# steveschwarcz/Cuda-Path-Tracer-SS

Measured on AMD Instinct MI355X. Metric: Mrays/sec at 1920x1080, 8 bounces, 2072 spp run (BASELINE configs[2] asks 2000 spp; a rate metric); ray = one live ray processed in one bounce, higher is better.
Workload: dtype f32; 1 GPU; configs[2]: 1920x1080 'mixed' preset (22 spheres, 16 triangles, Lambert/Phong/Cook-Torrance/glass/mirror), 8 bounces, 2072 spp = 74 steps x 1 pass(es) x 28 sample lanes per pixel; samples_per_pass=28, frame_lanes=1, lanes_free_run=True, seed=24301

## Files before the change

### cuda-path-tracer-ss_amd/csrc/ptss_api.hip

```cpp
#include <stdio.h>
#include <stdlib.h>
#include <string.h>

#include <new>
#include <string>
#include <vector>

#include "ptss.h"
#include "ptss_device.h"
#include <algorithm>
#include <array>
#include <cmath>
#include "ptquant.h"
#include "ptdenoise.h"
#include "ptmesh.h"
#include "pttri.h"

using namespace ptv;

#if PTSS_DIAG
namespace ptss { hipError_t readDiagCounters(unsigned long long* out8); }
#endif
namespace {

// ... 473 lines not shown
int validateScene(const ptss_scene_desc& s) {
    if ((s.numSpheres && !s.spheres) || (s.numTriangles && !s.triangles) || (s.numMaterials && !s.materials) ||
        (s.numPointLights && !s.pointLights) || (s.numAreaLights && !s.areaLights))
        return fail(PTSS_EINVAL, "scene: null array with non-zero count");
    for (size_t i = 0; i < s.numSpheres; ++i)
        if (s.spheres[i].materialIdx < 0 || (size_t)s.spheres[i].materialIdx >= s.numMaterials)
            return fail(PTSS_EINVAL, "scene: sphere materialIdx out of range");
    for (size_t i = 0; i < s.numTriangles; ++i)
        if (s.triangles[i].materialIdx < 0 || (size_t)s.triangles[i].materialIdx >= s.numMaterials)
            return fail(PTSS_EINVAL, "scene: triangle materialIdx out of range");
    for (size_t i = 0; i < s.numAreaLights; ++i)
        if (s.areaLights[i].triangleIdx < 0 || (size_t)s.areaLights[i].triangleIdx + 1 >= s.numTriangles)
            return fail(PTSS_EINVAL, "scene: area light needs triangles [triangleIdx, triangleIdx+1]");
    return PTSS_OK;
}

int localRows(const ptss_render_config& cfg) {
    int rows = 0;
    for (int y = 0; y < cfg.height; ++y)
        if ((y / cfg.bandRows) % cfg.tileWorld == cfg.tileRank) ++rows;
    return rows;
}

int createCheck(hipError_t e, const char* what) { return e == hipSuccess ? PTSS_OK : fail(e == hipErrorOutOfMemory ? PTSS_ENOMEM : PTSS_EHIP, what, e); }
#define ALLOC_TRY(expr) RC_TRY(createCheck((expr), #expr))
template <class T>
hipError_t mallocZeroed(T** p, size_t bytes) {
    const hipError_t e = hipMalloc(p, bytes);
    return e == hipSuccess ? hipMemset(*p, 0, bytes) : e;
}

int allocLane(Lane& ln, const uint32_t (&shardCount0)[ptss::kShards], bool ownStream) {
    const size_t poolBytes = (size_t)ptss::kRayPlanes * ln.regionCap * ptss::kShards * sizeof(float);
    for (float*& pool : ln.dPool) ALLOC_TRY(hipMalloc(&pool, poolBytes));
    for (uint32_t*& counts : ln.dCounts) ALLOC_TRY(mallocZeroed(&counts, ptss::kCountWords * sizeof(uint32_t)));
    ALLOC_TRY(mallocZeroed(&ln.dLastCounts, ptss::kCountWords * sizeof(uint32_t)));
    for (int s = 0; s < ptss::kShards; ++s)
        ALLOC_TRY(hipMemcpy(ln.dCounts[0] + ptss::countIndex(0, s), &shardCount0[s], sizeof(uint32_t), hipMemcpyHostToDevice));
    ALLOC_TRY(hipMalloc(&ln.dShardCount0, sizeof(shardCount0)));
    ALLOC_TRY(hipMemcpy(ln.dShardCount0, shardCount0, sizeof(shardCount0), hipMemcpyHostToDevice));
    ALLOC_TRY(mallocZeroed(&ln.dDone, (ptss::kCountWords + ptss::kCountStride) * sizeof(uint32_t)));
    if (ownStream) {
        ALLOC_TRY(hipStreamCreateWithFlags(&ln.stream, hipStreamNonBlocking));
        for (hipEvent_t& ev : ln.evDone) ALLOC_TRY(hipEventCreateWithFlags(&ev, hipEventDisableTiming));
    }
    ALLOC_TRY(hipHostMalloc(&ln.hCounts, 4 * ptss::kCountWords * sizeof(uint32_t), hipHostMallocDefault));
    for (hipEvent_t& ev : ln.hintEvent) ALLOC_TRY(hipEventCreateWithFlags(&ev, hipEventDisableTiming));
    return PTSS_OK;
}
#undef ALLOC_TRY

void releaseLane(Lane& ln) {
    for (hipEvent_t ev : ln.hintEvent)
        if (ev) (void)hipEventDestroy(ev);
    if (ln.hCounts) (void)hipHostFree(ln.hCounts);
    (void)hipFree(ln.dDone);
    for (hipEvent_t ev : ln.evDone)
        if (ev) (void)hipEventDestroy(ev);
    if (ln.stream) (void)hipStreamDestroy(ln.stream);
    for (float* pool : ln.dPool) (void)hipFree(pool);
    for (uint32_t* counts : ln.dCounts) (void)hipFree(counts);
    (void)hipFree(ln.dShardCount0);
    (void)hipFree(ln.dLastCounts);
}

ptss::FrameBuffers frameBuffers(const ptss_context* c, int laneIdx, ptss_uchar4* pixels, int sample) {
    const Lane& ln = c->lanes[(size_t)laneIdx];
    ptss::FrameBuffers fb{};
    fb.pool[0] = ln.dPool[0];
    fb.pool[1] = ln.dPool[1];
    fb.rngHome = c->dRngHome;
    fb.counts = ln.dCounts[c->countParity];
    fb.countsNext = ln.dCounts[1 - c->countParity];
    fb.shardCount0 = ln.dShardCount0;
    fb.lastCounts = ln.dLastCounts;
    fb.totalRayBounces = c->dTotal + laneIdx;
    fb.guardTimeouts = reinterpret_cast<uint32_t*>(c->dTotal + ptss::kMaxLanes + 8);
    fb.accum = c->dAccum;
    fb.fsum = c->dFsum;
    fb.staged = c->dStaged ? c->dStaged + (c->stagedTwice ? (size_t)(c->frameIndex & 1u) * c->capacity * c->samples : 0) : nullptr;
    fb.quantTable = reinterpret_cast<const float*>(c->image().dBlob + c->image().layout.offQuant);
    fb.pixels = pixels;
    fb.regionCap = ln.regionCap;
    fb.numPixels = c->numPixels;
    fb.plane = c->capacity;
    fb.samples = c->samples;
    fb.firstTiles = c->samples * (c->capacity / ptss::kBlock);
    fb.minLive = c->tile.world > 1 ? 0u : ptss::kMinLiveRays;
    fb.inverseTicks = 1.f / (float)((int)c->samples * (sample + 1));
    fb.defaultColor[0] = c->defaultColor[0];
    fb.defaultColor[1] = c->defaultColor[1];
    fb.defaultColor[2] = c->defaultColor[2];
    fb.laneIndex = (uint32_t)laneIdx;
    fb.laneCount = (uint32_t)c->lanes.size();
    fb.frameRays = c->numPixels * c->samples;
    fb.numPeers = fb.laneCount - 1;
    fb.myDone = ln.dDone;
    fb.myFrameDone = ln.dDone + ptss::kCountWords;
    fb.frameSeq = c->frameIndex;
    fb.joinsFrame = (laneIdx + 1 == (int)c->lanes.size()) ? 1u : 0u;
    uint32_t p = 0;
    for (size_t k = 0; k < c->lanes.size(); ++k) {
        if ((int)k == laneIdx) continue;
        fb.peerCounts[p] = c->lanes[k].dCounts[c->countParity];
        fb.peerDone[p] = c->lanes[k].dDone;
        fb.peerFrameDone[p] = c->lanes[k].dDone + ptss::kCountWords;
        ++p;
    }
    return fb;
}

void drainKernelEvents(ptss_context* c, bool wait) {
    size_t k = 0;
    for (size_t i = 0; i < c->evBusy.size(); ++i) {
        EventPair p = c->evBusy[i];
        hipError_t q = wait ? hipEventSynchronize(p.b) : hipEventQuery(p.b);
        if (q == hipSuccess) {
            float start = 0, ms = 0;
            if (hipEventElapsedTime(&start, c->evEpoch, p.a) == hipSuccess && hipEventElapsedTime(&ms, p.a, p.b) == hipSuccess)
            {
                if (c->kernelSpans.size() >= (1u << 20)) c->kernelSpans.clear();
                c->kernelSpans.emplace_back((double)start, (double)start + (double)ms);
            }
            c->evFree.push_back(p);
        } else {
            c->evBusy[k++] = p;
        }
    }
    c->evBusy.resize(k);
    (void)hipGetLastError();
}

int checkLaneTimeouts(ptss_context* c) {
    if (c->lanes.size() < 2 && !c->images[0].oneLaunch && !c->images[1].oneLaunch) return PTSS_OK;
    uint32_t v = 0;
    HIP_TRY(hipMemcpy(&v, c->dTotal + ptss::kMaxLanes + 8, sizeof(v), hipMemcpyDeviceToHost));
    if (v != c->timeoutsSeen) {
        c->timeoutsSeen = v;
        return fail(PTSS_ETIMEOUT, "a bounded wait on the device expired (a frame lane for a peer lane, or a workgroup of the one-launch "
                                   "frame kernel for its shard): the frame was not traced as specified");
    }
    return PTSS_OK;
}

void selectImage(ptss_context* c) {
    if (!c->images[1].dBlob) return;
    const int want = cameraInRange(c->camera) ? 0 : 1;
    if (want != c->active) {
        c->active = want;
        c->cameraDirty = true;
    }
}

ptss::EyeParams eyeParams(const ptss_context* c) {
    return {c->camera, -2 * ptm::tan(c->camera.fieldOfView * 0.5f), (float)c->tile.height / (float)c->tile.width, 1.0f / c->tile.width,
            1.0f / c->tile.height};
}

void harvestHints(ptss_context* c) {
    for (Lane& ln : c->lanes)
        for (int q = 0; q < 4; ++q) {
            if (!ln.hintPending[q] || hipEventQuery(ln.hintEvent[q]) != hipSuccess) continue;
            const uint32_t* src = ln.hCounts + (size_t)q * ptss::kCountWords;
            for (int b = 0; b <= ptss::kMaxBounces; ++b) {
                uint32_t mx = 0;
                for (int s = 0; s < ptss::kShards; ++s) mx = std::max(mx, src[ptss::countIndex(b, s)]);
                ln.hint[b] = mx;
            }
            ln.haveHint = true;
            ln.hintPending[q] = false;
        }
    (void)hipGetLastError();
}

int forkLanes(ptss_context* c, bool forkNeeded) {
    if (c->lanes.size() > 1 && (forkNeeded || c->frameIndex == 0 || !c->cfg.lanesFreeRun)) {
        HIP_TRY(hipEventRecord(c->evFork, c->stream));
        for (Lane& ln : c->lanes) HIP_TRY(hipStreamWaitEvent(ln.stream, c->evFork, 0));
    }
    if (c->stagedTwice && c->frameIndex >= 2)
        for (Lane& ln : c->lanes) HIP_TRY(hipStreamWaitEvent(ln.stream, c->evDisplay[c->frameIndex & 1u], 0));
    return PTSS_OK;
}

template <class Launch>
int timedLaunch(ptss_context* c, hipStream_t s, Launch launch) {
    if (!c->cfg.timeKernels) return launch();
    EventPair ev{nullptr, nullptr};
    if (c->evFree.empty() && c->evBusy.size() >= 4096) drainKernelEvents(c, true);
    if (c->evFree.empty()) {
        HIP_TRY(hipEventCreate(&ev.a));
        HIP_TRY(hipEventCreate(&ev.b));
    } else {
        ev = c->evFree.back();
        c->evFree.pop_back();
    }
    HIP_TRY(hipEventRecord(ev.a, s));
    RC_TRY(launch());
    HIP_TRY(hipEventRecord(ev.b, s));
    c->evBusy.push_back(ev);
    return PTSS_OK;
}

int traceOneLaunch(ptss_context* c, const ptss::FrameBuffers& fb, int numIterations, bool bounded, const ptss::EyeParams& eye) {
    const SceneImage& im = c->image();
    return timedLaunch(c, c->stream, [&] {
        HIP_TRY(ptss::launchFrame(c->stream, fb, im.dBlob, im.layout, numIterations, bounded, c->lanes[0].maxBlocks, c->tile, eye,
                                          &c->launchedKernels));
        return PTSS_OK;
    });
}

int traceBounces(ptss_context* c, ptss::FrameBuffers* fbs, int numIterations, bool bounded, const ptss::EyeParams& eye) {
    const SceneImage& im = c->image();
    const int K = (int)c->lanes.size();
    for (int i = 0; i < numIterations; ++i)
        for (int k = 0; k < K; ++k) {
            Lane& ln = c->lanes[(size_t)k];
            const hipStream_t ls = K > 1 ? ln.stream : c->stream;
            int blocks = ln.maxBlocks;
            if (i > 0 && ln.haveHint) {
                const unsigned long long tilesPerShard = ((unsigned long long)ln.hint[i] * 65 / 64 + ptss::kBlock) / ptss::kBlock + 1;
                const unsigned long long want = tilesPerShard * ptss::kShards;
                if (want < (unsigned long long)blocks) blocks = (int)want;
            }
            if (c->gridCap > 0 && c->gridCap * ptss::kShards < blocks) blocks = c->gridCap * ptss::kShards;
            if (i > 0)
                for (int j = 0, p = 0; j < K; ++j)
                    if (j != k) fbs[k].peerTarget[p++] = c->lanes[(size_t)j].doneTarget[i - 1];
            RC_TRY(timedLaunch(c, ls, [&] {
                HIP_TRY(ptss::launchBounce(ls, fbs[k], im.dBlob, im.layout, i, i == numIterations - 1, im.inLds, bounded, blocks, c->tile, eye,
                                               &c->launchedKernels));
                return PTSS_OK;
            }));
            ln.doneTarget[i] += (uint32_t)blocks;
        }
    return PTSS_OK;
}

int flushAndJoin(ptss_context* c, const ptss::FrameBuffers* fbs, int numIterations) {
    const int K = (int)c->lanes.size();
    for (int k = 0; k < K; ++k) {
        Lane& ln = c->lanes[(size_t)k];
        const hipStream_t ls = K > 1 ? ln.stream : c->stream;
        ptss::FlushTargets targets{};
        for (int j = 0, p = 0; j < K; ++j)
            if (j != k) {
                for (int b = 0; b <= ptss::kMaxBounces; ++b) targets.target[p][b] = c->lanes[(size_t)j].doneTarget[b];
                ++p;
            }
        HIP_TRY(ptss::launchFlush(ls, fbs[k], numIterations, targets));
        if (!ln.haveHint || (c->frameIndex & 7u) == 0) {
            const int q = (int)((c->frameIndex >> 3) & 3u);
            if (!ln.hintPending[q]) {
                HIP_TRY(hipMemcpyAsync(ln.hCounts + (size_t)q * ptss::kCountWords, ln.dLastCounts, ptss::kCountWords * sizeof(uint32_t),
                                       hipMemcpyDeviceToHost, ls));
                HIP_TRY(hipEventRecord(ln.hintEvent[q], ls));
                ln.hintPending[q] = true;
            }
        }
        if (K > 1 && k == K - 1) {
            HIP_TRY(hipEventRecord(ln.evDone[c->frameIndex & 1u], ls));
            HIP_TRY(hipStreamWaitEvent(c->stream, ln.evDone[c->frameIndex & 1u], 0));
        }
    }
    return PTSS_OK;
}

}

extern "C" {

int ptss_version(void) { return PTSS_VERSION; }

const char* ptss_error_string(int code) {
    switch (code) {
        case PTSS_OK: return "ok";
        case PTSS_EINVAL: return "invalid argument";
        case PTSS_EHIP: return "HIP runtime error";
        case PTSS_ENODEVICE: return "no usable HIP device";
        case PTSS_ENOMEM: return "out of memory";
        case PTSS_ERANGE: return "buffer too small or index out of range";
        case PTSS_ETIMEOUT: return "a frame lane timed out waiting for a peer lane";
        default: return "unknown error";
    }
}

const char* ptss_last_error_detail(void) { return g_detail.c_str(); }

int ptss_default_config(ptss_render_config* cfg) {
    if (!cfg) return fail(PTSS_EINVAL, "cfg is null");
    memset(cfg, 0, sizeof(*cfg));
    cfg->structSize = (unsigned int)sizeof(*cfg);
    cfg->width = 512;
    cfg->height = 512;
    cfg->seed = 0x5EEDull;
    cfg->maxIterations = 15;
    cfg->device = 0;
    cfg->tileRank = 0;
    cfg->tileWorld = 1;
    cfg->bandRows = 8;
    cfg->syncEachFrame = 1;
    cfg->floatAccumulator = 0;
    cfg->timeKernels = 0;
    cfg->samplesPerPass = 1;
    cfg->everySphereLoop = 0;
    cfg->frameLanes = 0;
    cfg->lanesFreeRun = 0;
    cfg->oneLaunchFrames = 0;
    return PTSS_OK;
}

int ptss_create(const ptss_scene_desc* scene, const ptss_render_config* cfg, ptss_context** out) {
    if (!scene || !cfg || !out) return fail(PTSS_EINVAL, "null argument");
    if (cfg->structSize != (unsigned int)sizeof(ptss_render_config))
        return fail(PTSS_EINVAL, "cfg->structSize is not this library's sizeof(ptss_render_config): the caller was built against another "
                                 "ptss.h (compare ptss_version() with PTSS_VERSION) or did not start from ptss_default_config");
    if (cfg->width <= 0 || cfg->height <= 0 || (long long)cfg->width * cfg->height > (1ll << 31) - 256)
        return fail(PTSS_EINVAL, "bad frame size");
    if (cfg->maxIterations == 0 || cfg->maxIterations > (unsigned)ptss::kMaxBounces)
        return fail(PTSS_EINVAL, "maxIterations must be in [1, 64]");
    if (cfg->tileWorld <= 0 || cfg->tileRank < 0 || cfg->tileRank >= cfg->tileWorld || cfg->bandRows <= 0)
        return fail(PTSS_EINVAL, "bad tile spec");
    const int spp = cfg->samplesPerPass == 0 ? 1 : cfg->samplesPerPass;
    if (spp < 1 || spp > 64) return fail(PTSS_EINVAL, "samplesPerPass must be in [1, 64]");
    if ((long long)cfg->width * cfg->height >= (1ll << 26)) return fail(PTSS_EINVAL, "frame too large (>= 2^26 pixels)");
    {
        const long long rows = localRows(*cfg);
        const unsigned long long rays = ((unsigned long long)cfg->width * rows + 255ull) / 256ull * 256ull * (unsigned long long)spp;
        if ((rays + (unsigned long long)ptss::kShards * ptss::kBlock) * ptss::kRayPlanes >= (1ull << 32))
            return fail(PTSS_EINVAL, "too many rays per pass: width x local rows x samplesPerPass must stay below ~226 million");
    }
    int rc = validateScene(*scene);
    if (rc != PTSS_OK) return rc;

    int ndev = 0;
    hipError_t e = hipGetDeviceCount(&ndev);
    if (e != hipSuccess || ndev <= 0) {
        (void)hipGetLastError();
        return fail(PTSS_ENODEVICE, "hipGetDeviceCount found no device (libptss has no CPU path)", e);
    }
    if (cfg->device < 0 || cfg->device >= ndev) return fail(PTSS_ENODEVICE, "device ordinal out of range");
    HIP_TRY(hipSetDevice(cfg->device));

    ptss_context* c = new (std::nothrow) ptss_context();
    if (!c) return fail(PTSS_ENOMEM, "context");
    c->cfg = *cfg;
    c->maxIterations = cfg->maxIterations;
    c->samples = (uint32_t)spp;
    c->defaultColor[0] = scene->defaultColor.x;
    c->defaultColor[1] = scene->defaultColor.y;
    c->defaultColor[2] = scene->defaultColor.z;
    c->camera.rotation = q4(1, 0, 0, 0);
    c->camera.position = v3(0, 0, 0);
    c->camera.zNear = -0.1f;
    c->camera.zFar = -100.0f;
    c->camera.fieldOfView = ptm::kPi / 2.0f;

    c->tile = ptss::TileMap{cfg->width, cfg->height, localRows(*cfg), cfg->tileRank, cfg->tileWorld, cfg->bandRows};
    c->numPixels = (uint32_t)cfg->width * (uint32_t)c->tile.localRows;
    const uint32_t gran = ptss::kBlock > 256 ? (uint32_t)ptss::kBlock : 256u;
    c->capacity = ((c->numPixels + gran - 1) / gran) * gran;
    if (c->capacity == 0) c->capacity = gran;
    int numLanes = cfg->frameLanes;
    if (numLanes < 0 || numLanes > ptss::kMaxLanes) return (delete c, fail(PTSS_EINVAL, "frameLanes must be in [0, 4]"));
    {
        const unsigned long long rays = (unsigned long long)c->numPixels * c->samples;
        if (numLanes == 0) numLanes = (cfg->lanesFreeRun && rays >= (3ull << 17) && rays <= (1ull << 24)) ? 2 : 1;
    }
    c->lanes.resize((size_t)numLanes);
    uint32_t shardCount0[ptss::kMaxLanes][ptss::kShards] = {{0}};
    {
        const uint32_t tilesPerPlane = c->capacity / ptss::kBlock;
        const uint32_t tiles = tilesPerPlane * c->samples;
        const uint32_t rounds = (tiles + ptss::kShards - 1) / ptss::kShards;
        for (int k = 0; k < numLanes; ++k) {
            const uint32_t laneRounds = (rounds + (uint32_t)numLanes - 1 - (uint32_t)k) / (uint32_t)numLanes;
            c->lanes[(size_t)k].regionCap = (laneRounds ? laneRounds : 1) * ptss::kBlock;
            c->lanes[(size_t)k].maxBlocks = (int)(c->lanes[(size_t)k].regionCap / ptss::kBlock) * ptss::kShards;
        }
        for (uint32_t t = 0; t < tiles; ++t) {
            const uint32_t first = (t % tilesPerPlane) * ptss::kBlock;
            uint32_t cnt = 0;
            if (first < c->numPixels) cnt = c->numPixels - first < (uint32_t)ptss::kBlock ? c->numPixels - first : (uint32_t)ptss::kBlock;
            shardCount0[(t / ptss::kShards) % (uint32_t)numLanes][t % ptss::kShards] += cnt;
        }
    }

    const bool wantAccel = accelEligible(*scene) && !cfg->everySphereLoop;
    const bool wantMesh = !wantAccel && meshEligible(*scene) && !cfg->everySphereLoop;
    const int numImages = wantAccel ? 2 : 1;
    std::vector<float4> blob[2];
    for (int i = 0; i < numImages; ++i) {
        SceneImage& im = c->images[i];
        packScene(*scene, im.layout, blob[i], wantAccel && i == 0, wantMesh);
        im.inLds = ptss::bounceLdsBytes(im.layout, true) <= 64 * 1024;
    }

#define CREATE_TRY(expr) do { if (int _rc = createCheck((expr), #expr)) return (ptss_destroy(c), _rc); } while (0)

    for (int i = 0; i < numImages; ++i) {
        CREATE_TRY(hipMalloc(&c->images[i].dBlob, blob[i].size() * sizeof(float4)));
        CREATE_TRY(hipMemcpy(c->images[i].dBlob, blob[i].data(), blob[i].size() * sizeof(float4), hipMemcpyHostToDevice));
    }
    CREATE_TRY(hipMalloc(&c->dRngHome, (size_t)ptss::kHomeWords * c->capacity * c->samples * sizeof(uint32_t)));
    for (int k = 0; k < numLanes; ++k)
        if (int laneRc = allocLane(c->lanes[(size_t)k], shardCount0[k], numLanes > 1)) return (ptss_destroy(c), laneRc);
    if (numLanes > 1) CREATE_TRY(hipEventCreateWithFlags(&c->evFork, hipEventDisableTiming));
    CREATE_TRY(mallocZeroed(&c->dTotal, kTotalWords * sizeof(unsigned long long)));
    CREATE_TRY(mallocZeroed(&c->dAccumOwned, (size_t)3 * c->capacity * sizeof(uint32_t)));
    c->dAccum = c->dAccumOwned;
    if (cfg->floatAccumulator) CREATE_TRY(mallocZeroed(&c->dFsum, (size_t)3 * c->capacity * c->samples * sizeof(float)));
    if (c->samples > 1) {
        c->stagedTwice = numLanes > 1 && cfg->lanesFreeRun != 0;
        const size_t words = (size_t)c->capacity * c->samples * (c->stagedTwice ? 2 : 1);
        CREATE_TRY(mallocZeroed(&c->dStaged, words * sizeof(uint32_t)));
        if (c->stagedTwice)
            for (int q = 0; q < 2; ++q) CREATE_TRY(hipEventCreateWithFlags(&c->evDisplay[q], hipEventDisableTiming));
    }
    CREATE_TRY(hipEventCreate(&c->evStart));
    CREATE_TRY(hipEventCreate(&c->evStop));
    CREATE_TRY(hipEventCreate(&c->evEpoch));

    {
        std::vector<uint32_t> table(ptrng::kJumpTableWords);
        ptrng::build_subsequence_table(table.data());
        uint32_t* dTable = nullptr;
        CREATE_TRY(hipMalloc(&dTable, table.size() * sizeof(uint32_t)));
        hipError_t e1 = hipMemcpy(dTable, table.data(), table.size() * sizeof(uint32_t), hipMemcpyHostToDevice);
        hipError_t e2 = e1;
        if (e1 == hipSuccess && c->numPixels > 0)
            e2 = ptss::launchRngInit(nullptr, c->dRngHome, c->capacity, c->samples, c->tile, cfg->seed, dTable);
        hipError_t e3 = e2 == hipSuccess ? hipEventRecord(c->evEpoch, nullptr) : e2;
        if (e3 == hipSuccess) e3 = hipDeviceSynchronize();
        (void)hipFree(dTable);
        CREATE_TRY(e3);
    }

    {
        hipDeviceProp_t prop;
        CREATE_TRY(hipGetDeviceProperties(&prop, cfg->device));
        const SceneImage& primary = c->images[0];
        const int perCU = ptss::bounceOccupancyBlocksPerCU(primary.layout, primary.inLds, primary.layout.sphereBounded != 0);
        c->gridCap = prop.multiProcessorCount * (perCU > 0 ? perCU : 4) * 16 / ptss::kShards;
        auto qualifies = [&](const SceneImage& im) {
            if (cfg->oneLaunchFrames <= 0 || numLanes != 1 || !im.inLds) return false;
            if (ptss::meshImage(im.layout)) return false;
            int perCU = ptss::frameOccupancyBlocksPerCU(im.layout, false);
            if (im.layout.sphereBounded) perCU = std::min(perCU, ptss::frameOccupancyBlocksPerCU(im.layout, true));
            const int resident = perCU - 1;
            return resident >= 1 && c->lanes[0].maxBlocks <= prop.multiProcessorCount * resident;
        };
        for (int i = 0; i < numImages; ++i) c->images[i].oneLaunch = qualifies(c->images[i]);
#ifdef PTSS_TUNING_KNOBS
        if (const char* e = getenv("PTSS_SCENE_PATH")) {
            if (!strcmp(e, "scalar"))
                for (SceneImage& im : c->images) im.inLds = false;
        }
        if (const char* e = getenv("PTSS_GRID_CAP")) c->gridCap = atoi(e);
#endif
    }
#undef CREATE_TRY

    *out = c;
    return PTSS_OK;
}

int ptss_destroy(ptss_context* c) {
    if (!c) return PTSS_OK;
    (void)hipSetDevice(c->cfg.device);
    (void)hipDeviceSynchronize();
    drainKernelEvents(c, true);
    for (EventPair& p : c->evFree) {
        (void)hipEventDestroy(p.a);
        (void)hipEventDestroy(p.b);
    }
    for (Lane& ln : c->lanes) releaseLane(ln);
    for (hipEvent_t ev : {c->evFork, c->evDisplay[0], c->evDisplay[1], c->evStart, c->evStop, c->evEpoch})
        if (ev) (void)hipEventDestroy(ev);
    for (SceneImage& im : c->images) (void)hipFree(im.dBlob);
    (void)hipFree(c->dRngHome);
    (void)hipFree(c->dTotal);
    (void)hipFree(c->dAccumOwned);
    (void)hipFree(c->dFsum);
    (void)hipFree(c->dStaged);
    for (float4* plane : c->dDenoise) (void)hipFree(plane);
    delete c;
    return PTSS_OK;
}

int ptss_generate_frame(ptss_context* c, ptss_uchar4* pixels, int ticks) {
    if (!c) return fail(PTSS_EINVAL, "ctx is null");
    hipStream_t st = c->stream;
    HIP_TRY(hipSetDevice(c->cfg.device));
    c->lastTicks = ticks;
    if (c->numPixels == 0) {
        if (c->resetTicksThisFrame) c->lastResetTick = ticks;
        c->resetTicksThisFrame = false;
        c->lastMs = 0.0f;
        return PTSS_OK;
    }

    selectImage(c);
    bool forkNeeded = false;
    if (c->resetTicksThisFrame) {
        forkNeeded = true;
        c->lastResetTick = ticks;
        HIP_TRY(ptss::launchClear(st, frameBuffers(c, 0, pixels, 0)));
        c->resetTicksThisFrame = false;
    }
    const int sample = ticks - c->lastResetTick;
    const int K = (int)c->lanes.size();
    ptss::FrameBuffers fbs[ptss::kMaxLanes];
    for (int k = 0; k < K; ++k) fbs[k] = frameBuffers(c, k, pixels, sample);

    if (c->cfg.syncEachFrame) HIP_TRY(hipEventRecord(c->evStart, st));

    const int numIterations = c->usePathTracer ? (int)c->maxIterations : 1;
    const ptss::EyeParams eye = eyeParams(c);
    if (c->cameraDirty) {
        forkNeeded = true;
        HIP_TRY(ptss::launchPrimaryPrep(st, c->image().dBlob, c->image().layout, c->camera.position));
        c->cameraDirty = false;
    }
    harvestHints(c);
    RC_TRY(forkLanes(c, forkNeeded));
    if (c->cfg.timeKernels) drainKernelEvents(c, false);
    const bool bounded = c->image().layout.sphereBounded != 0 && cameraInRange(c->camera);
    RC_TRY(c->image().oneLaunch && K == 1 ? traceOneLaunch(c, fbs[0], numIterations, bounded, eye) : traceBounces(c, fbs, numIterations, bounded, eye));
    RC_TRY(flushAndJoin(c, fbs, numIterations));
    if (c->samples > 1) {
        HIP_TRY(ptss::launchDisplay(st, fbs[0]));
        if (c->stagedTwice) HIP_TRY(hipEventRecord(c->evDisplay[c->frameIndex & 1u], st));
    }
    c->countParity ^= 1;
    c->frameIndex++;

    if (c->cfg.syncEachFrame) {
        HIP_TRY(hipEventRecord(c->evStop, st));
        HIP_TRY(hipEventSynchronize(c->evStop));
        HIP_TRY(hipEventElapsedTime(&c->lastMs, c->evStart, c->evStop));
        return c->lanes.size() > 1 ? checkLaneTimeouts(c) : PTSS_OK;
    }
    return PTSS_OK;
}

int ptss_set_camera(ptss_context* c, const ptss_camera* camera) {
    if (!c || !camera) return fail(PTSS_EINVAL, "null argument");
    c->camera = *camera;
    c->cameraDirty = true;
    c->resetTicksThisFrame = true;
    return PTSS_OK;
}

int ptss_get_camera(const ptss_context* c, ptss_camera* out) {
    if (!c || !out) return fail(PTSS_EINVAL, "null argument");
    *out = c->camera;
    return PTSS_OK;
}

int ptss_request_reset(ptss_context* c) {
    if (!c) return fail(PTSS_EINVAL, "ctx is null");
    c->resetTicksThisFrame = true;
    return PTSS_OK;
}

int ptss_set_mode(ptss_context* c, int usePathTracer) {
    if (!c) return fail(PTSS_EINVAL, "ctx is null");
    c->usePathTracer = usePathTracer != 0;
    c->resetTicksThisFrame = true;
    return PTSS_OK;
}

int ptss_set_max_iterations(ptss_context* c, unsigned int maxIterations) {
    if (!c || maxIterations == 0 || maxIterations > (unsigned)ptss::kMaxBounces)
        return fail(PTSS_EINVAL, "maxIterations must be in [1, 64]");
    c->maxIterations = maxIterations;
    return PTSS_OK;
}

int ptss_set_stream(ptss_context* c, void* hipStream) {
    if (!c) return fail(PTSS_EINVAL, "ctx is null");
    c->stream = (hipStream_t)hipStream;
    return PTSS_OK;
}

int ptss_bind_accumulator(ptss_context* c, uint32_t* dev) {
    if (!c) return fail(PTSS_EINVAL, "ctx is null");
    c->dAccum = dev ? dev : c->dAccumOwned;
    return PTSS_OK;
}

int ptss_accumulator_devptr(ptss_context* c, uint32_t** out) {
    if (!c || !out) return fail(PTSS_EINVAL, "null argument");
    *out = c->dAccum;
    return PTSS_OK;
}

int ptss_float_accumulator_devptr(ptss_context* c, float** out) {
    if (!c || !out) return fail(PTSS_EINVAL, "null argument");
    *out = c->dFsum;
    return PTSS_OK;
}

int ptss_alloc_pixels(ptss_context* c, ptss_uchar4** out) {
    if (!c || !out) return fail(PTSS_EINVAL, "null argument");
    HIP_TRY(hipSetDevice(c->cfg.device));
    HIP_TRY(hipMalloc(out, (size_t)c->capacity * sizeof(ptss_uchar4)));
    HIP_TRY(hipMemset(*out, 0, (size_t)c->capacity * sizeof(ptss_uchar4)));
    return PTSS_OK;
}

int ptss_free_pixels(ptss_context* c, ptss_uchar4* dev) {
    if (!c) return fail(PTSS_EINVAL, "ctx is null");
    HIP_TRY(hipFree(dev));
    return PTSS_OK;
}

int ptss_local_pixels(const ptss_context* c, size_t* out) {
    if (!c || !out) return fail(PTSS_EINVAL, "null argument");
    *out = c->numPixels;
    return PTSS_OK;
}

int ptss_local_rows(const ptss_context* c, int* rows, int cap, int* count) {
    if (!c || !count) return fail(PTSS_EINVAL, "null argument");
    int n = 0;
    for (int y = 0; y < c->tile.height; ++y) {
        if ((y / c->tile.bandRows) % c->tile.world != c->tile.rank) continue;
        if (rows) {
            if (n >= cap) return fail(PTSS_ERANGE, "rows[] too small");
            rows[n] = y;
        }
        ++n;
    }
    *count = n;
    return PTSS_OK;
}

int ptss_synchronize(ptss_context* c) {
    if (!c) return fail(PTSS_EINVAL, "ctx is null");
    HIP_TRY(hipStreamSynchronize(c->stream));
    return checkLaneTimeouts(c);
}

int ptss_read_accumulator(ptss_context* c, uint32_t* host, size_t count) {
    if (!c || !host) return fail(PTSS_EINVAL, "null argument");
    if (count != (size_t)3 * c->numPixels) return fail(PTSS_ERANGE, "count must be 3 * local pixels");
    HIP_TRY(hipStreamSynchronize(c->stream));
    HIP_TRY(hipMemcpy(host, c->dAccum, count * sizeof(uint32_t), hipMemcpyDeviceToHost));
    return checkLaneTimeouts(c);
}

int ptss_read_float_accumulator(ptss_context* c, float* host, size_t count) {
    if (!c || !host) return fail(PTSS_EINVAL, "null argument");
    if (!c->dFsum) return fail(PTSS_EINVAL, "context was created without floatAccumulator");
    if (count != (size_t)3 * c->numPixels) return fail(PTSS_ERANGE, "count must be 3 * local pixels");
    HIP_TRY(hipStreamSynchronize(c->stream));
    if (c->samples == 1) {
        HIP_TRY(hipMemcpy(host, c->dFsum, count * sizeof(float), hipMemcpyDeviceToHost));
    } else {
        std::vector<float> lane(count);
        for (size_t k = 0; k < count; ++k) host[k] = 0.0f;
        for (uint32_t l = 0; l < c->samples; ++l) {
            HIP_TRY(hipMemcpy(lane.data(), c->dFsum + (size_t)3 * l * c->capacity, count * sizeof(float), hipMemcpyDeviceToHost));
            for (size_t k = 0; k < count; ++k) host[k] = host[k] + lane[k];
        }
    }
    return checkLaneTimeouts(c);
}

int ptss_read_pixels(ptss_context* c, const ptss_uchar4* dev, ptss_uchar4* host, size_t count) {
    if (!c || !dev || !host) return fail(PTSS_EINVAL, "null argument");
    if (count > c->numPixels) return fail(PTSS_ERANGE, "count exceeds local pixels");
    HIP_TRY(hipStreamSynchronize(c->stream));
    HIP_TRY(hipMemcpy(host, dev, count * sizeof(ptss_uchar4), hipMemcpyDeviceToHost));
    return checkLaneTimeouts(c);
}

int ptss_read_rng_state(ptss_context* c, size_t local_pixel, uint32_t* out6) { return ptss_read_rng_state_lane(c, local_pixel, 0, out6); }

int ptss_read_rng_state_lane(ptss_context* c, size_t local_pixel, unsigned int lane, uint32_t* out6) {
    if (!c || !out6) return fail(PTSS_EINVAL, "null argument");
    if (local_pixel >= c->numPixels || lane >= c->samples) return fail(PTSS_ERANGE, "pixel or lane out of range");
    HIP_TRY(hipStreamSynchronize(c->stream));
    HIP_TRY(hipMemcpy(out6, c->dRngHome + (size_t)ptss::kHomeWords * ((size_t)lane * c->capacity + local_pixel), 6 * sizeof(uint32_t),
                      hipMemcpyDeviceToHost));
    return PTSS_OK;
}

int ptss_last_pass_ms(ptss_context* c, float* out) {
    if (!c || !out) return fail(PTSS_EINVAL, "null argument");
    *out = c->lastMs;
    return PTSS_OK;
}

int ptss_samples_since_reset(const ptss_context* c, int* out) {
    if (!c || !out) return fail(PTSS_EINVAL, "null argument");
    *out = c->resetTicksThisFrame ? 0 : (c->lastTicks - c->lastResetTick + 1) * (int)c->samples;
    return PTSS_OK;
}

int ptss_live_counts(ptss_context* c, uint32_t* out, int cap, int* n) {
    if (!c || !out || !n) return fail(PTSS_EINVAL, "null argument");
    const int numIterations = c->usePathTracer ? (int)c->maxIterations : 1;
    if (cap < numIterations) return fail(PTSS_ERANGE, "out[] too small");
    std::vector<uint32_t> raw(ptss::kCountWords), sum(ptss::kCountWords, 0u);
    HIP_TRY(hipStreamSynchronize(c->stream));
    for (const Lane& ln : c->lanes) {
        HIP_TRY(hipMemcpy(raw.data(), ln.dLastCounts, raw.size() * sizeof(uint32_t), hipMemcpyDeviceToHost));
        for (size_t k = 0; k < raw.size(); ++k) sum[k] += raw[k];
    }
    bool stopped = false;
    for (int i = 0; i < numIterations; ++i) {
        uint32_t total = 0;
        for (int s = 0; s < ptss::kShards; ++s) total += sum[ptss::countIndex(i, s)];
        if (total <= (c->tile.world > 1 ? 0u : ptss::kMinLiveRays)) stopped = true;
        out[i] = stopped ? 0u : total;
    }
    *n = numIterations;
    return checkLaneTimeouts(c);
}

int ptss_total_ray_bounces(ptss_context* c, unsigned long long* out) {
    if (!c || !out) return fail(PTSS_EINVAL, "null argument");
    HIP_TRY(hipStreamSynchronize(c->stream));
    unsigned long long perLane[ptss::kMaxLanes];
    HIP_TRY(hipMemcpy(perLane, c->dTotal, sizeof(perLane), hipMemcpyDeviceToHost));
    *out = 0;
    for (size_t k = 0; k < c->lanes.size(); ++k) *out += perLane[k];
    return checkLaneTimeouts(c);
}

int ptss_guard_timeouts(ptss_context* c, unsigned int* out) {
    if (!c || !out) return fail(PTSS_EINVAL, "null argument");
    HIP_TRY(hipStreamSynchronize(c->stream));
    uint32_t v = 0;
    HIP_TRY(hipMemcpy(&v, c->dTotal + ptss::kMaxLanes + 8, sizeof(v), hipMemcpyDeviceToHost));
    *out = v;
    return PTSS_OK;
}

int ptss_one_launch_frames(const ptss_context* c, int* out) {
    if (!c || !out) return fail(PTSS_EINVAL, "null argument");
    *out = (c->image().oneLaunch && c->lanes.size() == 1) ? 1 : 0;
    return PTSS_OK;
}

int ptss_frame_lanes(const ptss_context* c, int* out) {
    if (!c || !out) return fail(PTSS_EINVAL, "null argument");
    *out = (int)c->lanes.size();
    return PTSS_OK;
}

int ptss_launched_kernels(const ptss_context* c, unsigned long long* out) {
    if (!c || !out) return fail(PTSS_EINVAL, "null argument");
    *out = c->launchedKernels;
    return PTSS_OK;
}

static int rayQuery(ptss_context* c, bool any, const ptss_ray_query* rays, void* out, size_t n, void* hipStream) {
    if (!c) return fail(PTSS_EINVAL, "ctx is null");
    if (n == 0) return PTSS_OK;
    if (!rays || !out) return fail(PTSS_EINVAL, "null buffer with n > 0");
    if (n >= (size_t(1) << 31)) return fail(PTSS_ERANGE, "n must be below 2^31");
    if (((uintptr_t)rays | (uintptr_t)out) & (any ? 3u : 15u) || (uintptr_t)rays & 15u)
        return fail(PTSS_EINVAL, "rays and hits must be 16-byte aligned, verdicts 4-byte aligned");
    const SceneImage& im = c->images[0];
    if (!im.dBlob) return fail(PTSS_EINVAL, "context has no scene image");
    HIP_TRY(hipSetDevice(c->cfg.device));
    hipStream_t st = hipStream ? static_cast<hipStream_t>(hipStream) : c->stream;
    HIP_TRY(ptss::launchQuery(st, any, im.dBlob, im.layout, im.inLds, rays, out, (uint32_t)n, c->gridCap * ptss::kShards,
                              &c->launchedKernels));
    return PTSS_OK;
}

int ptss_intersect(ptss_context* c, const ptss_ray_query* dev_rays, ptss_ray_hit* dev_hits, size_t n, void* hipStream) {
    return rayQuery(c, false, dev_rays, dev_hits, n, hipStream);
}

int ptss_occluded(ptss_context* c, const ptss_ray_query* dev_rays, uint32_t* dev_occluded, size_t n, void* hipStream) {
    return rayQuery(c, true, dev_rays, dev_occluded, n, hipStream);
}

int ptss_render_features(ptss_context* c, ptss_pixel_feature* dev_features, void* hipStream) {
    if (!c) return fail(PTSS_EINVAL, "ctx is null");
    if (!dev_features) return fail(PTSS_EINVAL, "dev_features is null");
    if ((uintptr_t)dev_features & 15u) return fail(PTSS_EINVAL, "dev_features must be 16-byte aligned");
    if (c->numPixels == 0) return PTSS_OK;
    const SceneImage& im = c->images[0];
    if (!im.dBlob) return fail(PTSS_EINVAL, "context has no scene image");
    HIP_TRY(hipSetDevice(c->cfg.device));
    hipStream_t st = hipStream ? static_cast<hipStream_t>(hipStream) : c->stream;
    const ptss_vec3 defaultColor{c->defaultColor[0], c->defaultColor[1], c->defaultColor[2]};
    HIP_TRY(ptss::launchFeatures(st, im.dBlob, im.layout, im.inLds, c->tile, eyeParams(c), defaultColor, dev_features, c->numPixels,
                                 c->gridCap * ptss::kShards, &c->launchedKernels));
    return PTSS_OK;
}

int ptss_default_denoise_params(ptss_denoise_params* p) {
    if (!p) return fail(PTSS_EINVAL, "params is null");
    p->structSize = (unsigned int)sizeof(*p);
    p->levels = 5;
    p->sigmaColor = 64.0f;
    p->sigmaNormal = 0.1f;
    p->sigmaDepth = 4.0f;
    return PTSS_OK;
}

int ptss_denoise(ptss_context* c, const ptss_pixel_feature* dev_features, const ptss_denoise_params* params, ptss_uchar4* dev_out,
                 void* hipStream) {
    if (!c) return fail(PTSS_EINVAL, "ctx is null");
    if (!dev_features || !params || !dev_out) return fail(PTSS_EINVAL, "null argument");
    if (params->structSize != (unsigned int)sizeof(ptss_denoise_params))
        return fail(PTSS_EINVAL, "params->structSize is not this library's sizeof(ptss_denoise_params): start from ptss_default_denoise_params");
    if (params->levels < 0 || params->levels > PTSS_DENOISE_MAX_LEVELS) return fail(PTSS_EINVAL, "levels must be in [0, 6]");
    if (!(params->sigmaColor > 0.0f) || !(params->sigmaNormal > 0.0f) || !(params->sigmaDepth >= 0.0f))
        return fail(PTSS_EINVAL, "sigmaColor and sigmaNormal must be positive, sigmaDepth not negative");
    if (((uintptr_t)dev_features & 15u) || ((uintptr_t)dev_out & 3u)) return fail(PTSS_EINVAL, "dev_features must be 16-byte aligned, dev_out 4-byte aligned");
    if (c->tile.world > 1)
        return fail(PTSS_EINVAL, "ptss_denoise needs the whole frame: this context is a pixel-band shard (tileWorld > 1), whose bands of rows "
                                 "have no neighbours to filter with");
    HIP_TRY(hipSetDevice(c->cfg.device));
    hipStream_t st = hipStream ? static_cast<hipStream_t>(hipStream) : c->stream;
    const int levels = params->levels;
    if (levels >= 2)
        for (float4*& plane : c->dDenoise)
            if (!plane) {
                const hipError_t e = hipMalloc(&plane, (size_t)c->numPixels * sizeof(float4));
                if (e != hipSuccess) return fail(e == hipErrorOutOfMemory ? PTSS_ENOMEM : PTSS_EHIP, "ptss_denoise: colour planes", e);
            }
    const float inverseTicks = 1.f / (float)((int)c->samples * (c->lastTicks - c->lastResetTick + 1));
    const int width = c->tile.width, height = c->tile.height;
    c->denoiseLastPlane = levels >= 2 ? (levels - 2) & 1 : -1;
    c->denoiseLastLevel = levels - 2;
    c->denoiseStream = st;
    for (int i = 0; i < (levels > 0 ? levels : 1); ++i) {
        const bool first = i == 0, last = i + 1 >= levels;
        const void* src = first ? static_cast<const void*>(c->dAccum) : c->dDenoise[(i - 1) & 1];
        void* dst = last ? static_cast<void*>(dev_out) : c->dDenoise[i & 1];
        HIP_TRY(ptss::launchDenoise(st, first, last, src, dst, dev_features, width, height, ptdn::levelOf(*params, i), inverseTicks,
                                    &c->launchedKernels));
    }
    return PTSS_OK;
}

int ptss_read_denoise_plane(ptss_context* c, float* host_float3, size_t count, int* level) {
    if (!c || !host_float3) return fail(PTSS_EINVAL, "null argument");
    if (c->denoiseLastPlane < 0) return fail(PTSS_EINVAL, "no colour plane: the latest ptss_denoise of this context ran fewer than two levels");
    if (count != (size_t)3 * c->numPixels) return fail(PTSS_ERANGE, "count must be 3 * local pixels");
    HIP_TRY(hipSetDevice(c->cfg.device));
    HIP_TRY(hipStreamSynchronize(c->denoiseStream));
    std::vector<float4> plane(c->numPixels);
    HIP_TRY(hipMemcpy(plane.data(), c->dDenoise[c->denoiseLastPlane], plane.size() * sizeof(float4), hipMemcpyDeviceToHost));
    for (size_t p = 0; p < plane.size(); ++p) {
        host_float3[3 * p] = plane[p].x;
        host_float3[3 * p + 1] = plane[p].y;
        host_float3[3 * p + 2] = plane[p].z;
    }
    if (level) *level = c->denoiseLastLevel;
    return PTSS_OK;
}

int ptss_triangle_leaves(const ptss_context* c, int* out) {
    if (!c || !out) return fail(PTSS_EINVAL, "null argument");
    const ptss::SceneLayout& L = c->image().layout;
    *out = ptss::meshImage(L) ? L.mesh.numLeaves : 0;
    return PTSS_OK;
}

int ptss_debug_counters(ptss_context* c, unsigned long long* out8) {
    if (!c || !out8) return fail(PTSS_EINVAL, "null argument");
    HIP_TRY(hipStreamSynchronize(c->stream));
#if PTSS_DIAG
    HIP_TRY(ptss::readDiagCounters(out8));
#else
    for (int k = 0; k < 8; ++k) out8[k] = 0ull;
#endif
    return PTSS_OK;
}

int ptss_bounce_kernel_time(ptss_context* c, double* total_ms, unsigned long long* launches) {
    if (!c || !total_ms || !launches) return fail(PTSS_EINVAL, "null argument");
    HIP_TRY(hipStreamSynchronize(c->stream));
    for (const Lane& ln : c->lanes)
        if (ln.stream) HIP_TRY(hipStreamSynchronize(ln.stream));
    drainKernelEvents(c, true);
    std::sort(c->kernelSpans.begin(), c->kernelSpans.end());
    double busy = 0.0, curA = 0.0, curB = -1.0;
    for (const auto& sp : c->kernelSpans) {
        if (curB < curA || sp.first > curB) {
            if (curB >= curA) busy += curB - curA;
            curA = sp.first;
            curB = sp.second;
        } else if (sp.second > curB) {
            curB = sp.second;
        }
    }
    if (curB >= curA) busy += curB - curA;
    *total_ms = busy;
    *launches = c->kernelSpans.size();
    c->kernelSpans.clear();
    HIP_TRY(hipEventRecord(c->evEpoch, c->stream));
    HIP_TRY(hipEventSynchronize(c->evEpoch));
    return checkLaneTimeouts(c);
}

}
```

### cuda-path-tracer-ss_amd/csrc/ptss_device.h

```cpp
#pragma once
#include <hip/hip_runtime.h>
#include <stdint.h>

#include "ptmath.h"
#include "ptss_types.h"
#include "xorwow.h"

namespace ptdn { struct Level; }

namespace ptss {

enum RayPlane : int {
    kOx = 0, kOy, kOz,
    kDx, kDy, kDz,
    kL0x, kL0y, kL0z,
    kTx, kTy, kTz,
    kPix,
    kR0, kR1, kR2, kR3, kR4,
    kRd,
    kRayPlanes
};
constexpr int kHomeWords = 8;
constexpr int kMaxBounces = 64;
#ifndef PTSS_BLOCK
#define PTSS_BLOCK 256
#endif
#ifndef PTSS_SHARDS
#define PTSS_SHARDS 16
#endif
#ifndef PTSS_CHUNK
#define PTSS_CHUNK 16
#endif
#ifndef PTSS_MINWAVES
#define PTSS_MINWAVES 7
#endif
#ifndef PTSS_MINWAVES_BOUNDED
#define PTSS_MINWAVES_BOUNDED 6
#endif
#ifndef PTSS_MINWAVES_FIRST
#define PTSS_MINWAVES_FIRST 6
#endif
#ifndef PTSS_ABLATE
#define PTSS_ABLATE 0
#endif
#ifndef PTSS_DIAG
#define PTSS_DIAG 0
#endif
constexpr int kBlock = PTSS_BLOCK;
constexpr int kChunkSpheres = PTSS_CHUNK;
static_assert((kChunkSpheres & (kChunkSpheres - 1)) == 0, "chunk size must be a power of two");
constexpr int kShards = PTSS_SHARDS;
constexpr int kCountStride = 32;
constexpr int kCountWords = (kMaxBounces + 1) * kShards * kCountStride;
__host__ __device__ inline int countIndex(int bounce, int shard) { return (bounce * kShards + shard) * kCountStride; }
constexpr int kWaves = kBlock / 64;
constexpr uint32_t kMinLiveRays = 128;

struct SceneLayout {
    int numSpheres, numTriangles, numMaterials, numPointLights, numAreaLights;
    int offSphere;
    int offSphereMat;
    int offTri;
    int offTriNormal;
    int offTriVert;
    int offMaterial;
    int offPointLight;
    int offAreaLight;
    int accelSpheres;
    int numChunks;
    int offChunk;
    int offSphereOrig;
    int offSpherePos;
    int offQuant;
    int offPrimSphere;
    int offPrimTri;
    int offPrimChunk;
    int totalVec4;
    int ldsVec4;
    int neeSkipSafe;
    int sphereBounded;
    int neePairs;
    int triDetBounded;
    int triClassed;
    union {
        uint32_t triClassPack[5];
        struct {
            int numLeaves, numGroups;
            int offGroup;
            int offLeaf;
            int reserved;
        } mesh;
    };
    int offTriPos;
};

constexpr int kMeshLeaf = 16;
__host__ __device__ inline bool meshImage(const SceneLayout& L) { return !L.triClassed && L.mesh.numLeaves > 0; }

struct TileMap {
    int width, height;
    int localRows;
    int rank, world, bandRows;
};

struct EyeParams {
    ptss_camera camera;
    float s;
    float aspect;
    float invW, invH;
};

constexpr int kMaxLanes = 4;

struct FrameBuffers {
    float* pool[2];
    uint32_t* rngHome;
    uint32_t* counts;
    uint32_t* countsNext;
    const uint32_t* shardCount0;
    uint32_t* lastCounts;
    unsigned long long* totalRayBounces;
    uint32_t* accum;
    float* fsum;
    const float* quantTable;
    uint32_t* staged;
    ptss_uchar4* pixels;
    uint32_t regionCap;
    uint32_t numPixels;
    uint32_t plane;
    uint32_t samples;
    uint32_t firstTiles;
    uint32_t minLive;
    float inverseTicks;
    float defaultColor[3];
    uint32_t laneIndex, laneCount;
    uint32_t frameRays;
    uint32_t numPeers;
    const uint32_t* peerCounts[kMaxLanes - 1];
    const uint32_t* peerDone[kMaxLanes - 1];
    uint32_t peerTarget[kMaxLanes - 1];
    uint32_t* myDone;
    uint32_t* myFrameDone;
    const uint32_t* peerFrameDone[kMaxLanes - 1];
    uint32_t frameSeq;
    uint32_t joinsFrame;
    uint32_t* guardTimeouts;
};

hipError_t launchRngInit(hipStream_t st, uint32_t* rngHome, uint32_t plane, uint32_t samples, TileMap tile, uint64_t seed,
                         const uint32_t* jumpTable);
hipError_t launchDisplay(hipStream_t st, const FrameBuffers& fb);
hipError_t launchClear(hipStream_t st, const FrameBuffers& fb);
hipError_t launchPrimaryPrep(hipStream_t st, float4* sceneBlob, const SceneLayout& layout, ptss_vec3 origin);
hipError_t launchBounce(hipStream_t st, const FrameBuffers& fb, const float4* sceneBlob, SceneLayout layout, int bounce,
                        bool isLast, bool sceneInLds, bool bounded, int gridBlocks, TileMap tile, EyeParams eye, unsigned long long* launched);
size_t bounceLdsBytes(const SceneLayout& layout, bool sceneInLds);
hipError_t launchFrame(hipStream_t st, const FrameBuffers& fb, const float4* sceneBlob, SceneLayout layout, int numBounces, bool bounded, int gridBlocks,
                       TileMap tile, EyeParams eye, unsigned long long* launched);
int frameOccupancyBlocksPerCU(const SceneLayout& layout, bool bounded);
struct FlushTargets {
    uint32_t target[kMaxLanes - 1][kMaxBounces + 1];
};
hipError_t launchFlush(hipStream_t st, const FrameBuffers& fb, int numBounces, const FlushTargets& targets);
int bounceOccupancyBlocksPerCU(const SceneLayout& layout, bool sceneInLds, bool bounded);
hipError_t launchQuery(hipStream_t st, bool any, const float4* sceneBlob, SceneLayout layout, bool sceneInLds, const void* rays, void* out,
                       uint32_t n, int maxBlocks, unsigned long long* launched);
hipError_t launchFeatures(hipStream_t st, const float4* sceneBlob, SceneLayout layout, bool sceneInLds, TileMap tile, EyeParams eye,
                          ptss_vec3 defaultColor, void* out, uint32_t n, int maxBlocks, unsigned long long* launched);
hipError_t launchDenoise(hipStream_t st, bool first, bool last, const void* src, void* dst, const void* features, int width, int height,
                         const ptdn::Level& level, float inverseTicks, unsigned long long* launched);

}
```

### cuda-path-tracer-ss_amd/csrc/ptss_kernels.hip

```cpp
#include "ptss_device.h"
#include "ptquant.h"
#include "pttri.h"

#include <array>
#include <utility>

using namespace ptv;

namespace ptss {
namespace {

__device__ __forceinline__ float asF(uint32_t u) { return __builtin_bit_cast(float, u); }
__device__ __forceinline__ uint32_t asU(float f) { return __builtin_bit_cast(uint32_t, f); }
__device__ __forceinline__ vec3 xyz(float4 v) { return vec3{v.x, v.y, v.z}; }
__device__ __forceinline__ bool waveAny(bool p) { return __builtin_amdgcn_ballot_w64(p) != 0ull; }
__device__ __forceinline__ bool waveAll(bool p) { return __builtin_amdgcn_ballot_w64(p) == __builtin_amdgcn_ballot_w64(true); }
__device__ __forceinline__ void waveLdsFence() { __builtin_amdgcn_fence(__ATOMIC_ACQ_REL, "wavefront"); }

struct PixelCoord {
    int x, gy;
    uint32_t globalIndex;
};

__device__ __forceinline__ PixelCoord locate(const TileMap& t, uint32_t local) {
    const int lx = (int)(local % (uint32_t)t.width);
    const int ly = (int)(local / (uint32_t)t.width);
    const int band = ly / t.bandRows, within = ly % t.bandRows;
    PixelCoord p;
    p.x = lx;
    p.gy = (band * t.world + t.rank) * t.bandRows + within;
    p.globalIndex = (uint32_t)p.gy * (uint32_t)t.width + (uint32_t)lx;
    return p;
}

constexpr uint32_t kLaneShift = 26;
constexpr uint32_t kPixMask = (1u << kLaneShift) - 1u;
__device__ __forceinline__ uint32_t pixOf(uint32_t packed) { return packed & kPixMask; }
__device__ __forceinline__ uint32_t laneOf(uint32_t packed) { return packed >> kLaneShift; }

struct RayRegs {
    vec3 o, d, L0, T;
    uint32_t pix;
    ptrng::State rng;
    bool active;
};

__device__ __forceinline__ const float* tileBlock(const float* __restrict__ region, uint32_t firstSlot ) {
    return region + (size_t)(firstSlot / kBlock) * (kRayPlanes * kBlock);
}
__device__ __forceinline__ uint32_t slotWord(uint32_t slot) {
    return (slot / kBlock) * (uint32_t)(kRayPlanes * kBlock) + (slot % kBlock);
}

template <bool kCoherent = false>
__device__ __forceinline__ float ldPlane(const float* __restrict__ block, uint32_t laneBytes, int plane) {
    const float* p = reinterpret_cast<const float*>(reinterpret_cast<const char*>(block) + (size_t)laneBytes + (size_t)plane * (kBlock * sizeof(float)));
    if constexpr (kCoherent) return __hip_atomic_load(p, __ATOMIC_RELAXED, __HIP_MEMORY_SCOPE_AGENT);
    else return *p;
}
template <bool kCoherent = false>
__device__ __forceinline__ void stPlane(float* __restrict__ region, uint32_t wordBytes, int plane, float v) {
    float* p = reinterpret_cast<float*>(reinterpret_cast<char*>(region) + (size_t)wordBytes + (size_t)plane * (kBlock * sizeof(float)));
    if constexpr (kCoherent) __hip_atomic_store(p, v, __ATOMIC_RELAXED, __HIP_MEMORY_SCOPE_AGENT);
    else *p = v;
}

template <bool kCoherent = false>
__device__ __forceinline__ void loadRayGeometry(const float* __restrict__ block, uint32_t w, RayRegs& r) {
    const uint32_t b = w * 4u;
    r.o = vec3{ldPlane<kCoherent>(block, b, kOx), ldPlane<kCoherent>(block, b, kOy), ldPlane<kCoherent>(block, b, kOz)};
    r.d = vec3{ldPlane<kCoherent>(block, b, kDx), ldPlane<kCoherent>(block, b, kDy), ldPlane<kCoherent>(block, b, kDz)};
    r.active = true;
}
template <bool kCoherent = false>
__device__ __forceinline__ void loadRayRng(const float* __restrict__ block, uint32_t w, RayRegs& r) {
    const uint32_t b = w * 4u;
    r.rng.v[0] = asU(ldPlane<kCoherent>(block, b, kR0));
    r.rng.v[1] = asU(ldPlane<kCoherent>(block, b, kR1));
    r.rng.v[2] = asU(ldPlane<kCoherent>(block, b, kR2));
    r.rng.v[3] = asU(ldPlane<kCoherent>(block, b, kR3));
    r.rng.v[4] = asU(ldPlane<kCoherent>(block, b, kR4));
    r.rng.d = asU(ldPlane<kCoherent>(block, b, kRd));
}
template <bool kCoherent = false>
__device__ __forceinline__ void loadRayRadiance(const float* __restrict__ block, uint32_t w, RayRegs& r) {
    const uint32_t b = w * 4u;
    r.L0 = vec3{ldPlane<kCoherent>(block, b, kL0x), ldPlane<kCoherent>(block, b, kL0y), ldPlane<kCoherent>(block, b, kL0z)};
    r.T = vec3{ldPlane<kCoherent>(block, b, kTx), ldPlane<kCoherent>(block, b, kTy), ldPlane<kCoherent>(block, b, kTz)};
    r.pix = asU(ldPlane<kCoherent>(block, b, kPix));
}
template <bool kCoherent = false>
__device__ __forceinline__ void loadRay(const float* __restrict__ block, uint32_t w, RayRegs& r) {
    loadRayGeometry<kCoherent>(block, w, r);
    loadRayRng<kCoherent>(block, w, r);
    loadRayRadiance<kCoherent>(block, w, r);
}

template <bool kCoherent = false>
__device__ __forceinline__ void storeRay(float* __restrict__ region, uint32_t slot, const RayRegs& r) {
    const uint32_t b = slotWord(slot) * 4u;
    stPlane<kCoherent>(region, b, kOx, r.o.x);   stPlane<kCoherent>(region, b, kOy, r.o.y);   stPlane<kCoherent>(region, b, kOz, r.o.z);
    stPlane<kCoherent>(region, b, kDx, r.d.x);   stPlane<kCoherent>(region, b, kDy, r.d.y);   stPlane<kCoherent>(region, b, kDz, r.d.z);
    stPlane<kCoherent>(region, b, kL0x, r.L0.x); stPlane<kCoherent>(region, b, kL0y, r.L0.y); stPlane<kCoherent>(region, b, kL0z, r.L0.z);
    stPlane<kCoherent>(region, b, kTx, r.T.x);   stPlane<kCoherent>(region, b, kTy, r.T.y);   stPlane<kCoherent>(region, b, kTz, r.T.z);
    stPlane<kCoherent>(region, b, kPix, asF(r.pix));
    stPlane<kCoherent>(region, b, kR0, asF(r.rng.v[0]));
    stPlane<kCoherent>(region, b, kR1, asF(r.rng.v[1]));
    stPlane<kCoherent>(region, b, kR2, asF(r.rng.v[2]));
    stPlane<kCoherent>(region, b, kR3, asF(r.rng.v[3]));
    stPlane<kCoherent>(region, b, kR4, asF(r.rng.v[4]));
    stPlane<kCoherent>(region, b, kRd, asF(r.rng.d));
}

__device__ __forceinline__ bool sphereTest(float4 sp, vec3 o, vec3 d, float limit, float& t) {
    const vec3 v = o - xyz(sp);
    const float b = dot(d, v) * 2;
    const float c = dot(v, v) - sp.w;
    float disc = (b * b) - 4 * c;
    if (disc < 0) return false;
    disc = ptm::sqrt(disc);
    float t0 = (-b + disc) * 0.5f;
    float t1 = (-b - disc) * 0.5f;
    if (t0 < 0 && t1 < 0) return false;
    if (t0 > t1) {
        const float tmp = t0;
        t0 = t1;
        t1 = tmp;
    }
    const float cand = (t0 < 0) ? t1 : t0;
    if (cand > limit) return false;
    t = cand;
    return true;
}

struct TriHit {
    bool hit;
    unsigned long long hitMask;
    float dist, w0, w1, w2;
};

struct TriRows {
    float4 a, b, c;
};
__device__ __forceinline__ float4 loadRow16(const float4* p) { return *p; }
__device__ __forceinline__ TriRows loadTri(const float4* tr) { return TriRows{loadRow16(tr), loadRow16(tr + 1), loadRow16(tr + 2)}; }
__device__ __forceinline__ TriRows loadTriEdges(const float4* tr) { return TriRows{float4{0, 0, 0, 0}, loadRow16(tr + 1), loadRow16(tr + 2)}; }

__device__ __forceinline__ float triRcp(float det) { return ptm::rcp_if_above_1em7(det); }

__device__ __forceinline__ unsigned long long maskOf(bool directCompare) { return __builtin_amdgcn_ballot_w64(directCompare); }

__device__ __forceinline__ TriHit triangleTest(const TriRows& tr, vec3 o, vec3 d, float limit, unsigned long long liveMask) {
    const vec3 v0 = xyz(tr.a), e1 = xyz(tr.b), e2 = xyz(tr.c);
    const vec3 q = cross(d, e2);
    const float det = dot(e1, q);
// ... 56 lines not shown
        const bool hit = __builtin_amdgcn_inverse_ballot_w64(hitMask);
        best.dist = hit ? h.dist : best.dist;
        best.key = hit ? key : best.key;
        best.w1 = hit ? b1 : best.w1;
        best.w2 = hit ? b2 : best.w2;
    }
}
struct ClassBounds {
    uint32_t w[5];
};
__device__ __forceinline__ ClassBounds classBounds(const SceneLayout& L) {
    return ClassBounds{{L.triClassPack[0], L.triClassPack[1], L.triClassPack[2], L.triClassPack[3], L.triClassPack[4]}};
}
template <int kCode>
__device__ __forceinline__ int classBegin(ClassBounds& b) {
    asm volatile("" : "+s"(b.w[kCode / 4]));
    return (int)((b.w[kCode / 4] >> (8 * (kCode % 4))) & 255u);
}
#define PTSS_FOR_TRIANGLES_BY_CLASS(L, BODY)                                                                        \
    do {                                                                                                            \
        ClassBounds _cb = classBounds(L);                                                                           \
        PTSS_TRI_CLASS_LOOP(_cb, 0, 0, BODY) PTSS_TRI_CLASS_LOOP(_cb, 0, 1, BODY) PTSS_TRI_CLASS_LOOP(_cb, 0, 2, BODY) PTSS_TRI_CLASS_LOOP(_cb, 0, 3, BODY) \
        PTSS_TRI_CLASS_LOOP(_cb, 1, 0, BODY) PTSS_TRI_CLASS_LOOP(_cb, 1, 2, BODY) PTSS_TRI_CLASS_LOOP(_cb, 1, 3, BODY)      \
        PTSS_TRI_CLASS_LOOP(_cb, 2, 0, BODY) PTSS_TRI_CLASS_LOOP(_cb, 2, 1, BODY) PTSS_TRI_CLASS_LOOP(_cb, 2, 3, BODY)      \
        PTSS_TRI_CLASS_LOOP(_cb, 3, 0, BODY) PTSS_TRI_CLASS_LOOP(_cb, 3, 1, BODY) PTSS_TRI_CLASS_LOOP(_cb, 3, 2, BODY)      \
    } while (0)
#define PTSS_TRI_CLASS_LOOP(cb, c1, c2, BODY) \
    for (int t = classBegin<(c1) * 4 + (c2)>(cb), tEnd = classBegin<(c1) * 4 + (c2) + 1>(cb); t < tEnd; ++t) { BODY(c1, c2, t) }

template <int kC1, int kC2>
__device__ __forceinline__ void triangleClassedAny(const float4* rows, vec3 o, vec3 d, float limit, unsigned long long& need, unsigned long long& blocked) {
    const pttri::Head h = pttri::head<kC1, kC2, false>(xyz(loadRow16(rows)), xyz(loadRow16(rows + 1)), xyz(loadRow16(rows + 2)), v3(0, 0, 0), v3(0, 0, 0), 0.0f, o, d);
    const unsigned long long passMask = need & maskOf(!(ptm::abs(h.det) <= 1e-7f)) & maskOf(!(h.dist <= 0.0f)) & maskOf(!(h.dist > limit));
    if (passMask != 0ull) {
        float b0, b1, b2;
        pttri::weights<kC1, kC2>(h, d, b0, b1, b2);
        const unsigned long long hitMask = passMask & maskOf(!(__builtin_fminf(__builtin_fminf(b0, b1), b2) < 0));
        blocked |= hitMask;
        need &= ~hitMask;
    }
}
template <int kC1, int kC2>
__device__ __forceinline__ void triangleClassedPair(const float4* rows, vec3 o, vec3 dA, float limitA, vec3 dB, float limitB, unsigned long long& needA,
                                                    unsigned long long& needB, unsigned long long& blockedA, unsigned long long& blockedB) {
    const vec3 e1 = xyz(loadRow16(rows + 1)), e2 = xyz(loadRow16(rows + 2));
    const pttri::OriginPart p = pttri::originPart<kC1, kC2>(xyz(loadRow16(rows)), e1, e2, o);
    if (needA != 0ull) {
        const pttri::Head h = pttri::headFrom<kC1, kC2>(p, e1, e2, dA);
        const unsigned long long pass = needA & maskOf(!(ptm::abs(h.det) <= 1e-7f)) & maskOf(!(h.dist <= 0.0f)) & maskOf(!(h.dist > limitA));
        if (pass != 0ull) {
            float b0, b1, b2;
            pttri::weights<kC1, kC2>(h, dA, b0, b1, b2);
            const unsigned long long hit = pass & maskOf(!(__builtin_fminf(__builtin_fminf(b0, b1), b2) < 0));
            blockedA |= hit;
            needA &= ~hit;
        }
    }
    if (needB != 0ull) {
        const pttri::Head h = pttri::headFrom<kC1, kC2>(p, e1, e2, dB);
        const unsigned long long pass = needB & maskOf(!(ptm::abs(h.det) <= 1e-7f)) & maskOf(!(h.dist <= 0.0f)) & maskOf(!(h.dist > limitB));
        if (pass != 0ull) {
            float b0, b1, b2;
            pttri::weights<kC1, kC2>(h, dB, b0, b1, b2);
            const unsigned long long hit = pass & maskOf(!(__builtin_fminf(__builtin_fminf(b0, b1), b2) < 0));
            blockedB |= hit;
            needB &= ~hit;
        }
    }
}
__device__ __forceinline__ bool classedQueryOk(vec3 o, vec3 d) { return waveAll(dot(d, d) < 0x1p30f) && waveAll(dot(o, o) < 0x1p100f); }

__device__ __forceinline__ bool sphereTestPrimary(float4 pv, vec3 d, float limit, float& t) {
    const float b = dot(d, xyz(pv)) * 2;
    float disc = (b * b) - 4 * pv.w;
    if (disc < 0) return false;
    disc = ptm::sqrt(disc);
    float t0 = (-b + disc) * 0.5f;
    float t1 = (-b - disc) * 0.5f;
    if (t0 < 0 && t1 < 0) return false;
    if (t0 > t1) {
        const float tmp = t0;
        t0 = t1;
        t1 = tmp;
    }
    const float cand = (t0 < 0) ? t1 : t0;
    if (cand > limit) return false;
    t = cand;
    return true;
}

__device__ __forceinline__ TriHit triangleTestPrimary(const TriRows& tr, float4 ps , float4 pr ,
                                                      vec3 d, float limit, unsigned long long liveMask) {
    const vec3 e1 = xyz(tr.b), e2 = xyz(tr.c);
    const vec3 q = cross(d, e2);
    const float det = dot(e1, q);
    const float inverseDet = triRcp(det);
    const float dist = ps.w * inverseDet;
    const unsigned long long passMask = liveMask & maskOf(!(ptm::abs(det) <= 1e-7f)) & maskOf(!(dist <= 0.0f)) & maskOf(!(dist > limit));
    TriHit h;
    h.hit = false;
    h.hitMask = 0ull;
    h.dist = dist;
    h.w0 = h.w1 = h.w2 = 0;
    if (passMask != 0ull) {
        const float b1 = dot(xyz(ps), q) * inverseDet;
        const float b2 = dot(d, xyz(pr)) * inverseDet;
        const float b0 = 1.0f - (b1 + b2);
        h.hitMask = passMask & maskOf(!(b0 < 0)) & maskOf(!(b1 < 0)) & maskOf(!(b2 < 0));
        h.hit = __builtin_amdgcn_inverse_ballot_w64(h.hitMask);
        h.w0 = b0;
        h.w1 = b1;
        h.w2 = b2;
    }
    return h;
}

__device__ __forceinline__ void shiftInMayHit(uint32_t& rev, float bb, float c4) {
    asm("v_cmp_nlt_f32 vcc, %1, %2\n\tv_addc_co_u32 %0, vcc, %0, %0, vcc" : "+v"(rev) : "v"(bb), "v"(c4) : "vcc");
}
template <bool kCull>
__device__ __forceinline__ float aheadFactor(float h) {
    if constexpr (kCull) {
        const float hk = h * 0x1p-18f;
        float m;
        asm("v_min_f32 %0, %1, %2" : "=v"(m) : "v"(hk), "v"(h));
        return m;
    } else {
        return h;
    }
}
template <bool kBounded, bool kCull = false>
__device__ __forceinline__ void shiftInSphere(uint32_t& rev, float4 sp, vec3 o, vec3 d) {
    const vec3 v = o - xyz(sp);
    if constexpr (kBounded) {
        const float h = dot(d, v);
        const float c = dot(v, v) - sp.w;
        shiftInMayHit(rev, h * aheadFactor<kCull>(h), c);
    } else {
        const float b = dot(d, v) * 2;
        const float c = dot(v, v) - sp.w;
        shiftInMayHit(rev, b * b, 4 * c);
    }
}
template <bool kBounded>
__device__ __forceinline__ void shiftInSpherePrimary(uint32_t& rev, float4 pv, vec3 d) {
    if constexpr (kBounded) {
        const float h = dot(d, xyz(pv));
        shiftInMayHit(rev, h * h, pv.w);
    } else {
        const float b = dot(d, xyz(pv)) * 2;
        shiftInMayHit(rev, b * b, 4 * pv.w);
    }
}
template <bool kPrimary, bool kBounded>
__device__ __forceinline__ uint32_t sphereCandidates(const float4* rows, int cnt, vec3 o, vec3 d) {
    const int trips = (cnt + 3) >> 2;
    uint32_t rev = 0;
    for (int g = 0; g < trips; ++g) {
        const float4 r0 = rows[4 * g], r1 = rows[4 * g + 1], r2 = rows[4 * g + 2], r3 = rows[4 * g + 3];
        if constexpr (kPrimary) {
            shiftInSpherePrimary<kBounded>(rev, r0, d);
            shiftInSpherePrimary<kBounded>(rev, r1, d);
            shiftInSpherePrimary<kBounded>(rev, r2, d);
            shiftInSpherePrimary<kBounded>(rev, r3, d);
        } else {
            shiftInSphere<kBounded, true>(rev, r0, o, d);
            shiftInSphere<kBounded, true>(rev, r1, o, d);
            shiftInSphere<kBounded, true>(rev, r2, o, d);
            shiftInSphere<kBounded, true>(rev, r3, o, d);
        }
    }
    return __builtin_bitreverse32(rev) >> (32 - 4 * trips);
}
template <bool kBounded>
__device__ __forceinline__ uint32_t sphereCandidatesPairs(const float4* rows, int cnt, vec3 o, vec3 d) {
    const int trips = (cnt + 1) >> 1;
    uint32_t rev = 0;
    for (int g = 0; g < trips; ++g) {
        const float4 r0 = rows[2 * g], r1 = rows[2 * g + 1];
        shiftInSphere<kBounded>(rev, r0, o, d);
        shiftInSphere<kBounded>(rev, r1, o, d);
    }
    return __builtin_bitreverse32(rev) >> (32 - 2 * trips);
}
template <bool kBounded>
__device__ __forceinline__ uint32_t sphereCandidatesStridedPairs(const float4* first, int stride, int cnt, vec3 o, vec3 d) {
    const int trips = (cnt + 1) >> 1;
    uint32_t rev = 0;
    for (int g = 0; g < trips; ++g) {
        const float4* p = first + 2 * g * stride;
        const float4 r0 = p[0], r1 = p[stride];
        shiftInSphere<kBounded>(rev, r0, o, d);
        shiftInSphere<kBounded>(rev, r1, o, d);
    }
    return __builtin_bitreverse32(rev) >> (32 - 2 * trips);
}
__device__ __forceinline__ uint32_t lowBits(int cnt) { return (cnt >= 32) ? 0xffffffffu : ((1u << cnt) - 1u); }
__device__ __forceinline__ uint32_t lowBitsClamped(int cnt) { return (cnt <= 0) ? 0u : lowBits(cnt); }

struct Hit {
    float distance;
    int kind, idx;
    float w0, w1, w2;
};

constexpr int kQueueCapConst = 2 * 64;
constexpr float kAccelMu = 5e-3f + 5e-3f * 5e-3f;
constexpr float kAccelDirEps = 1e-5f;
constexpr float kAccelQ = 0.25f * (1.0f + 2e-5f) / (1.0f - kAccelMu) * (1.0f + 1e-6f);

__device__ __forceinline__ void shiftInChunk(uint32_t& rev, float4 b, vec3 o, vec3 d) {
    const vec3 v = o - xyz(b);
    const float dv = dot(d, v);
    const float vv = dot(v, v);
    const float t = dv - ptm::abs(dv);
    const unsigned long long may = ~maskOf(ptm::fma(-kAccelQ, t * t, vv) > b.w);
    asm("v_addc_co_u32 %0, vcc, %0, %0, %1" : "+v"(rev) : "s"(may) : "vcc");
}
__device__ __forceinline__ void shiftInChunkPrimary(uint32_t& rev, float4 pv, vec3 d) {
    const float dv = dot(d, xyz(pv));
    const float t = dv - ptm::abs(dv);
    const unsigned long long may = ~maskOf(ptm::fma(-kAccelQ, t * t, pv.w) > 0.0f);
    asm("v_addc_co_u32 %0, vcc, %0, %0, %1" : "+v"(rev) : "s"(may) : "vcc");
}
template <bool kPrimary>
__device__ __forceinline__ uint32_t chunkMask(const float4* bounds, int cnt, vec3 o, vec3 d, bool unitDir) {
    const int trips = (cnt + 3) >> 2;
    uint32_t rev = 0;
    for (int g = 0; g < trips; ++g) {
        const float4 b0 = bounds[4 * g], b1 = bounds[4 * g + 1], b2 = bounds[4 * g + 2], b3 = bounds[4 * g + 3];
        if constexpr (kPrimary) {
            shiftInChunkPrimary(rev, b0, d);
            shiftInChunkPrimary(rev, b1, d);
            shiftInChunkPrimary(rev, b2, d);
            shiftInChunkPrimary(rev, b3, d);
        } else {
            shiftInChunk(rev, b0, o, d);
            shiftInChunk(rev, b1, o, d);
            shiftInChunk(rev, b2, o, d);
            shiftInChunk(rev, b3, o, d);
        }
    }
    const uint32_t all = (cnt >= 32) ? 0xffffffffu : ((1u << cnt) - 1u);
    return unitDir ? ((__builtin_bitreverse32(rev) >> (32 - 4 * trips)) & all) : all;
}

#include "ptss_diag.h"
#include "ptmesh.h"

typedef __attribute__((address_space(3))) const float4 LdsRow;
__device__ __forceinline__ uint32_t chunkCandidates(const float4* spheres , int base, int chunk, vec3 o, vec3 d) {
    static_assert(kChunkSpheres * sizeof(float4) <= 256, "a chunk's rows must not straddle the 256-byte window the XOR walks");
    uint32_t rev = 0;
    const int twist = chunk & (kChunkSpheres - 1);
#if __HIP_DEVICE_COMPILE__
    if (__builtin_amdgcn_is_shared(spheres)) {
        const uint32_t first = (uint32_t)(uintptr_t)(LdsRow*)spheres;
        if ((first & 255u) == 0u) {
            uint32_t x = (first + (uint32_t)base * (uint32_t)sizeof(float4)) ^ ((uint32_t)twist << 4);
            asm volatile("" : "+v"(x));
#pragma unroll
            for (int i = 0; i < kChunkSpheres; ++i) shiftInSphere<true, true>(rev, *(LdsRow*)(uintptr_t)(x ^ ((uint32_t)i << 4)), o, d);
            return rev;
        }
    }
#endif
#pragma unroll 4
    for (int i = 0; i < kChunkSpheres; ++i) shiftInSphere<true, true>(rev, spheres[base + (i ^ twist)], o, d);
    return rev;
}
__device__ __forceinline__ int chunkSlot(int bit, int chunk) { return ((kChunkSpheres - 1 - bit) ^ chunk) & (kChunkSpheres - 1); }

struct ChunkBits {
    uint32_t w[4];
};
template <bool kPrimary = false>
__device__ __forceinline__ ChunkBits chunkBits128(const float4* sc, const SceneLayout& L, int g0, vec3 o, vec3 d, bool unitDir, bool live) {
    ChunkBits b;
#pragma unroll
    for (int q = 0; q < 4; ++q) {
        const int g = g0 + 32 * q;
        const int left = L.numChunks - g;
        b.w[q] = (left > 0) ? chunkMask<kPrimary>(sc + (kPrimary ? L.offPrimChunk : L.offChunk) + g, left < 32 ? left : 32, o, d, unitDir) : 0u;
        if (!live) b.w[q] = 0u;
    }
    return b;
}
__device__ __forceinline__ bool anyChunk(const ChunkBits& b) { return (b.w[0] | b.w[1] | b.w[2] | b.w[3]) != 0u; }
__device__ __forceinline__ int popChunk(ChunkBits& b) {
    const int q = b.w[0] ? 0 : (b.w[1] ? 1 : (b.w[2] ? 2 : 3));
    const uint32_t word = q == 0 ? b.w[0] : (q == 1 ? b.w[1] : (q == 2 ? b.w[2] : b.w[3]));
    const int k = __builtin_ctz(word);
    const uint32_t rest = word & (word - 1u);
    b.w[0] = q == 0 ? rest : b.w[0];
    b.w[1] = q == 1 ? rest : b.w[1];
    b.w[2] = q == 2 ? rest : b.w[2];
    b.w[3] = q == 3 ? rest : b.w[3];
    return 32 * q + k;
}


__device__ __forceinline__ bool anySphereChunked(const float4* sc, const SceneLayout& L, vec3 lo, vec3 w_i, float distance, bool live) {
    const bool unitDir = ptm::abs(dot(w_i, w_i) - 1.0f) <= kAccelDirEps;
    bool occluded = false;
    for (int g0 = 0; g0 < L.numChunks; g0 += 128) {
        ChunkBits chunks = chunkBits128(sc, L, g0, lo, w_i, unitDir, live && !occluded);
        while (anyChunk(chunks)) {
            const int chunk = g0 + popChunk(chunks);
            const int base = chunk * kChunkSpheres;
            uint32_t mask = chunkCandidates(sc + L.offSphere, base, chunk, lo, w_i);
            while (mask != 0) {
// ... 181 lines not shown
            incl += (lane >= off) ? below : 0u;
        }
        startTab[lane] = incl - cnt;
        const uint32_t total = (uint32_t)__shfl((int)incl, 63);
        waveLdsFence();
        for (uint32_t q0 = 0; q0 < total; q0 += 64) {
            const uint32_t q = q0 + lane;
            const bool valid = q < total;
            uint32_t a = 0, b = 64;
#pragma unroll
            for (int step = 0; step < 6; ++step) {
                const uint32_t mid = (a + b) >> 1;
                const bool right = startTab[mid] <= q;
                a = right ? mid : a;
                b = right ? b : mid;
            }
            const uint32_t owner = valid ? a : lane;
            uint32_t r = valid ? q - startTab[owner] : 0u;
            uint32_t word = 0, wordIdx = 0;
            bool found = false;
#pragma unroll
            for (int w = 0; w < 4; ++w) {
                const uint32_t bits = (w == 0 ? bits0 : (w == 1 ? bits1 : (w == 2 ? bits2 : bits3)))[owner];
                const uint32_t pc = (uint32_t)__builtin_popcount(bits);
                const bool here = !found && r < pc;
                word = here ? bits : word;
                wordIdx = here ? (uint32_t)w : wordIdx;
                found = found || here;
                r -= (!found) ? pc : 0u;
            }
            const bool work = valid && found && blocked[owner] == 0u;
            const int chunk = g0 + (int)(32u * wordIdx + nthSetBit(word, r));
            const int base = (work ? chunk : 0) * kChunkSpheres;
            const vec3 so = v3(seg[0 * kQueueCapConst + owner], seg[1 * kQueueCapConst + owner], seg[2 * kQueueCapConst + owner]);
            const vec3 sd = v3(seg[3 * kQueueCapConst + owner], seg[4 * kQueueCapConst + owner], seg[5 * kQueueCapConst + owner]);
            const float reach = seg[6 * kQueueCapConst + owner];
            uint32_t mask = chunkCandidates(sc + L.offSphere, base, chunk, so, sd);
            if (!work) mask = 0;
            while (mask != 0) {
                const int j = chunkSlot(__builtin_ctz(mask), chunk);
                mask &= mask - 1;
                float t;
                if (sphereTest(sc[L.offSphere + base + j], so, sd, reach, t)) {
                    blocked[owner] = 1u;
                    mask = 0;
                }
            }
        }
        waveLdsFence();
        occluded = blocked[lane] != 0u;
        waveLdsFence();
    }
    return occluded;
}

__device__ __forceinline__ bool meshQueryOk(vec3 o, vec3 d, bool live) {
    return waveAll(!live || (ptm::abs(dot(d, d) - 1.0f) <= ptmesh::kMeshDirEps && dot(o, o) < 0x1p80f));
}
__device__ __forceinline__ bool meshMay(const float4* b, vec3 o, vec3 d) {
    const float4 r0 = loadRow16(b), r1 = loadRow16(b + 1), r2 = loadRow16(b + 2);
    return ptmesh::mayTouch(xyz(r0), r0.w, xyz(r1), r1.w, r2.x, r2.y, r2.z, r2.w, o, d, 1.0f);
}
__device__ __forceinline__ uint32_t meshGroupMask(const float4* groups, int cnt, vec3 o, vec3 d) {
    const int trips = (cnt + 3) >> 2;
    uint32_t rev = 0;
    for (int g = 0; g < trips; ++g) {
#pragma unroll
        for (int k = 0; k < 4; ++k) {
            const unsigned long long may = maskOf(meshMay(groups + 3 * (4 * g + k), o, d));
            asm("v_addc_co_u32 %0, vcc, %0, %0, %1" : "+v"(rev) : "s"(may) : "vcc");
        }
    }
    return (__builtin_bitreverse32(rev) >> (32 - 4 * trips)) & lowBits(cnt);
}
__device__ __forceinline__ uint32_t meshLeafMask(const float4* leaves, int g, int numLeaves, vec3 o, vec3 d) {
    const int first = g * kMeshLeaf;
    const int cnt = numLeaves - first < kMeshLeaf ? numLeaves - first : kMeshLeaf;
    uint32_t m = 0;
    for (int j = 0; j < cnt; ++j) m |= meshMay(leaves + 3 * (first + j), o, d) ? (1u << j) : 0u;
    return m;
}
__device__ __forceinline__ const float4* meshLeaves(const float4* sc, const float4* cold, const SceneLayout& L) {
    return (L.mesh.offLeaf < L.ldsVec4 ? sc : cold) + L.mesh.offLeaf;
}
template <bool kPrimary>
__device__ __forceinline__ void closestTrianglesMesh(const float4* sc, const float4* cold, const SceneLayout& L, vec3 o, vec3 d, bool live,
                                                     TriBest& best) {
    const float4* leaves = meshLeaves(sc, cold, L);
    for (int g0 = 0; g0 < L.mesh.numGroups; g0 += 32) {
        const int left = L.mesh.numGroups - g0;
        uint32_t groups = meshGroupMask(sc + L.mesh.offGroup + 3 * g0, left < 32 ? left : 32, o, d);
        if (!live) groups = 0u;
        while (groups != 0u) {
            const int g = g0 + __builtin_ctz(groups);
            groups &= groups - 1u;
            uint32_t leafBits = meshLeafMask(leaves, g, L.mesh.numLeaves, o, d);
            while (leafBits != 0u) {
                const int t0 = (g * kMeshLeaf + __builtin_ctz(leafBits)) * kMeshLeaf;
                leafBits &= leafBits - 1u;
                const int t1 = L.numTriangles - t0 < kMeshLeaf ? L.numTriangles : t0 + kMeshLeaf;
                for (int t = t0; t < t1; ++t)
                    triangleClassed<kPrimary, 0, 0, true>(cold + L.offTri + 3 * t, cold + L.offPrimTri + 2 * t, 0u, o, d, ~0ull, best);
            }
        }
    }
}
__device__ __forceinline__ bool anyTrianglesMesh(const float4* sc, const float4* cold, const SceneLayout& L, vec3 o, vec3 d, float limit, bool live) {
    if (!meshQueryOk(o, d, live)) {
        unsigned long long need = maskOf(live), blocked = 0ull;
        for (int i = 0; i < L.numTriangles; ++i) {
            if (need == 0ull) break;
            const TriHit th = triangleTest(loadTri(cold + L.offTri + 3 * i), o, d, limit, need);
            blocked |= th.hitMask;
            need &= ~th.hitMask;
        }
        return __builtin_amdgcn_inverse_ballot_w64(blocked);
    }
    const float4* leaves = meshLeaves(sc, cold, L);
    bool blocked = false;
    for (int g0 = 0; g0 < L.mesh.numGroups; g0 += 32) {
        if (!waveAny(live && !blocked)) break;
        const int left = L.mesh.numGroups - g0;
        uint32_t groups = meshGroupMask(sc + L.mesh.offGroup + 3 * g0, left < 32 ? left : 32, o, d);
        if (!live || blocked) groups = 0u;
        while (groups != 0u) {
            const int g = g0 + __builtin_ctz(groups);
            groups &= groups - 1u;
            uint32_t leafBits = meshLeafMask(leaves, g, L.mesh.numLeaves, o, d);
            while (leafBits != 0u) {
                const int t0 = (g * kMeshLeaf + __builtin_ctz(leafBits)) * kMeshLeaf;
                leafBits &= leafBits - 1u;
                const int t1 = L.numTriangles - t0 < kMeshLeaf ? L.numTriangles : t0 + kMeshLeaf;
                for (int t = t0; t < t1; ++t) {
                    const float4* r = cold + L.offTri + 3 * t;
                    const pttri::Head hh = pttri::head<0, 0, false>(xyz(loadRow16(r)), xyz(loadRow16(r + 1)), xyz(loadRow16(r + 2)), v3(0, 0, 0),
                                                                    v3(0, 0, 0), 0.0f, o, d);
                    if (pttri::passesHead(hh, limit)) {
                        float b0, b1, b2;
                        pttri::weights<0, 0>(hh, d, b0, b1, b2);
                        if (pttri::passesWeights(b0, b1, b2)) {
                            blocked = true;
                            break;
                        }
                    }
                }
                if (blocked) leafBits = 0u;
            }
            if (blocked) groups = 0u;
        }
    }
    return blocked;
}

template <bool kPrimary, bool kAccel, bool kBounded, bool kMesh = false>
__device__ __forceinline__ Hit closestHit(const float4* sc, const float4* cold, const SceneLayout& L, vec3 o, vec3 d, bool live, uint32_t* ws) {
    Hit h;
    h.distance = ptm::inf();
    h.kind = 0;
    h.idx = 0;
    h.w0 = h.w1 = h.w2 = 0;
    if constexpr (kAccel) closestSpheresRegrouped<kPrimary>(sc, cold, L, o, d, live, h, ws);
    for (int base = 0; base < (kAccel ? 0 : L.numSpheres); base += 32) {
        const int cnt = (L.numSpheres - base < 32) ? (L.numSpheres - base) : 32;
        uint32_t mask = sphereCandidates<kPrimary, kBounded>(sc + (kPrimary ? L.offPrimSphere : L.offSphere) + base, cnt, o, d);
        mask &= live ? lowBits(cnt) : 0u;
        PTSS_DIAG_CANDIDATES(mask, live, 0);
        while (mask != 0) {
            const int j = __builtin_ctz(mask);
            mask &= mask - 1;
            float t;
            const bool acc = kPrimary ? sphereTestPrimary(sc[L.offPrimSphere + base + j], d, h.distance, t)
                                      : sphereTest(sc[L.offSphere + base + j], o, d, h.distance, t);
            if (acc) {
                h.distance = t;
                h.kind = 1;
                h.idx = base + j;
            }
        }
    }
    const unsigned long long liveMask = maskOf(live);
    if constexpr (kMesh) {
        if (meshQueryOk(o, d, live)) {
            TriBest best{h.distance, kNoTriangle, 0.0f, 0.0f};
            closestTrianglesMesh<kPrimary>(sc, cold, L, o, d, live, best);
            if (best.key != kNoTriangle) {
                h.distance = best.dist;
                h.kind = 2;
                h.idx = reinterpret_cast<const int*>(cold + L.offTriPos)[0xfffffffeu - best.key];
                h.w1 = best.w1;
                h.w2 = best.w2;
                h.w0 = 1.0f - (best.w1 + best.w2);
            }
            return h;
        }
    } else if (L.triClassed) {
        if (classedQueryOk(o, d)) {
            TriBest best{h.distance, kNoTriangle, 0.0f, 0.0f};
#define PTSS_CLOSEST_BODY(c1, c2, t) \
    triangleClassed<kPrimary, c1, c2, true>(sc + L.offTri + 3 * t, sc + L.offPrimTri + 2 * t, 0u, o, d, liveMask, best);
            PTSS_FOR_TRIANGLES_BY_CLASS(L, PTSS_CLOSEST_BODY);
#undef PTSS_CLOSEST_BODY
            if (waveAny(best.key != kNoTriangle)) {
                const int* posOf = reinterpret_cast<const int*>(sc + L.offTriPos);
                int pos = 0;
                if (best.key != kNoTriangle) pos = posOf[0xfffffffeu - best.key];
                const bool zeroWeight = best.key != kNoTriangle && (best.w1 == 0.0f || best.w2 == 0.0f);
                if (waveAny(zeroWeight)) {
                    if (zeroWeight) {
                        const float4* rows = sc + L.offTri + 3 * pos;
                        const float4* prim = sc + L.offPrimTri + 2 * pos;
                        const pttri::Head g = pttri::head<0, 0, kPrimary>(xyz(rows[0]), xyz(rows[1]), xyz(rows[2]), xyz(prim[0]), xyz(prim[1]), prim[0].w, o, d);
                        float b0;
                        pttri::weights<0, 0>(g, d, b0, best.w1, best.w2);
                    }
                }
                if (best.key != kNoTriangle) {
                    h.distance = best.dist;
                    h.kind = 2;
                    h.idx = pos;
                    h.w1 = best.w1;
                    h.w2 = best.w2;
                    h.w0 = 1.0f - (best.w1 + best.w2);
                }
            }
            return h;
        }
    } else if (L.triDetBounded && waveAll(dot(d, d) < 0x1p30f)) {
        TriBest best{h.distance, kNoTriangle, 0.0f, 0.0f};
        for (int i = 0; i < L.numTriangles; ++i)
            triangleClassed<kPrimary, 0, 0, false>(sc + L.offTri + 3 * i, sc + L.offPrimTri + 2 * i, (uint32_t)i, o, d, liveMask, best);
        if (best.key != kNoTriangle) {
            h.distance = best.dist;
            h.kind = 2;
            h.idx = (int)best.key;
            h.w1 = best.w1;
            h.w2 = best.w2;
            h.w0 = 1.0f - (best.w1 + best.w2);
        }
        return h;
    }
    const float4* td = kMesh ? cold : sc;
    const int* posOfOriginal = reinterpret_cast<const int*>(td + L.offTriPos);
    for (int k = 0; k < L.numTriangles; ++k) {
        const int i = (kMesh || L.triClassed) ? posOfOriginal[k] : k;
        const TriRows tcur = kPrimary ? loadTriEdges(td + L.offTri + 3 * i) : loadTri(td + L.offTri + 3 * i);
        const TriHit th = kPrimary ? triangleTestPrimary(tcur, td[L.offPrimTri + 2 * i], loadRow16(td + L.offPrimTri + 2 * i + 1), d,
                                                         h.distance, liveMask)
                                   : triangleTest(tcur, o, d, h.distance, liveMask);
        if (th.hit) {
            h.distance = th.dist;
            h.kind = 2;
            h.idx = i;
            h.w0 = th.w0;
            h.w1 = th.w1;
            h.w2 = th.w2;
        }
    }
    return h;
}

__device__ __forceinline__ void anyTriangleLoop(const float4* sc, const SceneLayout& L, vec3 lo, vec3 w_i, float distance, unsigned long long& need,
                                                unsigned long long& blocked) {
    if (L.triClassed && classedQueryOk(lo, w_i)) {
#define PTSS_ANY_BODY(c1, c2, t)   \
    if (need == 0ull) break;      \
    triangleClassedAny<c1, c2>(sc + L.offTri + 3 * t, lo, w_i, distance, need, blocked);
        PTSS_FOR_TRIANGLES_BY_CLASS(L, PTSS_ANY_BODY);
#undef PTSS_ANY_BODY
        return;
    }
    for (int i = 0; i < L.numTriangles; ++i) {
        if (need == 0ull) break;
        const TriRows tcur = loadTri(sc + L.offTri + 3 * i);
        const TriHit th = triangleTest(tcur, lo, w_i, distance, need);
        blocked |= th.hitMask;
        need &= ~th.hitMask;
    }
}

__device__ __forceinline__ bool anyTriangles(const float4* sc, const SceneLayout& L, vec3 lo, vec3 w_i, float distance, bool live) {
    unsigned long long need = maskOf(live), blocked = 0ull;
    anyTriangleLoop(sc, L, lo, w_i, distance, need, blocked);
    return __builtin_amdgcn_inverse_ballot_w64(blocked);
}

template <bool kAccel, bool kBounded, bool kMesh = false>
__device__ __forceinline__ bool anyHit(const float4* sc, const SceneLayout& L, vec3 lo, vec3 w_i, float distance,
                                       bool live, const float4* cold = nullptr) {
    bool occluded = false;
    if constexpr (kAccel) occluded = anySphereChunked(sc, L, lo, w_i, distance, live);
    for (int base = 0; base < (kAccel ? 0 : L.numSpheres); base += 32) {
        const int cnt = (L.numSpheres - base < 32) ? (L.numSpheres - base) : 32;
        uint32_t mask = sphereCandidatesPairs<kBounded>(sc + L.offSphere + base, cnt, lo, w_i);
        mask &= (live && !occluded) ? lowBits(cnt) : 0u;
        PTSS_DIAG_CANDIDATES(mask, live, 4);
        while (mask != 0) {
            const int j = __builtin_ctz(mask);
            mask &= mask - 1;
            float t;
            if (sphereTest(sc[L.offSphere + base + j], lo, w_i, distance, t)) {
                occluded = true;
                mask = 0;
            }
        }
    }
    if constexpr (kMesh) return anyTrianglesMesh(sc, cold, L, lo, w_i, distance, live && !occluded) || occluded;
    unsigned long long need = maskOf(live) & ~maskOf(occluded);
    unsigned long long blocked = 0ull;
    anyTriangleLoop(sc, L, lo, w_i, distance, need, blocked);
    return occluded || __builtin_amdgcn_inverse_ballot_w64(blocked);
}

template <bool kBounded>
__device__ __forceinline__ bool anyHitSplit(const float4* sc, const SceneLayout& L, vec3 lo, vec3 w_i, float distance,
                                            bool live, int shift, int sub) {
    bool occluded = false;
    const int g = 1 << shift;
    const int sphereSteps = (L.numSpheres + g - 1) >> shift;
    for (int base = 0; base < sphereSteps; base += 32) {
        const int cnt = (sphereSteps - base < 32) ? (sphereSteps - base) : 32;
        uint32_t mask = sphereCandidatesStridedPairs<kBounded>(sc + L.offSphere + (base << shift) + sub, g, cnt, lo, w_i);
        mask &= (live && !occluded) ? lowBitsClamped(((L.numSpheres - sub + g - 1) >> shift) - base) : 0u;
        while (mask != 0) {
            const int j = __builtin_ctz(mask);
            mask &= mask - 1;
            float t;
            if (sphereTest(sc[L.offSphere + ((base + j) << shift) + sub], lo, w_i, distance, t)) {
                occluded = true;
                mask = 0;
            }
        }
    }
    const int triSteps = (L.numTriangles + g - 1) >> shift;
    unsigned long long need = maskOf(live) & ~maskOf(occluded);
    unsigned long long blocked = 0ull;
    for (int k = 0; k < triSteps; ++k) {
        if (need == 0ull) break;
        const int idx = (k << shift) + sub;
        const bool in = idx < L.numTriangles;
        const TriRows tcur = loadTri(sc + L.offTri + 3 * (in ? idx : 0));
        const TriHit th = triangleTest(tcur, lo, w_i, distance, need & maskOf(in));
        blocked |= th.hitMask;
        need &= ~th.hitMask;
    }
    return occluded || __builtin_amdgcn_inverse_ballot_w64(blocked);
}

template <bool kBounded, bool kSplit>
__device__ __forceinline__ void pairAnyHit(const float4* sc, const SceneLayout& L, vec3 lo, vec3 wA, float dA, bool liveA, vec3 wB, float dB,
                                           bool liveB, int shift, int sub, bool& occA, bool& occB) {
    occA = false;
    occB = false;
    const int g = kSplit ? (1 << shift) : 1;
    const int sphereSteps = kSplit ? ((L.numSpheres + g - 1) >> shift) : L.numSpheres;
// ... 266 lines not shown
    uint32_t x, y, z;
};

__device__ __forceinline__ void finishPath(const FrameBuffers& fb, const RayRegs& r, const float* quantT) {
    const uint32_t p = pixOf(r.pix), lane = laneOf(r.pix);
    const uint32_t stream = lane * fb.plane + p;
    const uint32_t qx = quantizeSample(r.L0.x, quantT), qy = quantizeSample(r.L0.y, quantT), qz = quantizeSample(r.L0.z, quantT);
    if (fb.samples == 1) {
        U3* acc = reinterpret_cast<U3*>(fb.accum) + p;
        U3 t = *acc;
        t.x += qx;
        t.y += qy;
        t.z += qz;
        *acc = t;
        if (fb.pixels) {
            const uint32_t px = (uint32_t)(unsigned char)(t.x * fb.inverseTicks + 0.5f) |
                                ((uint32_t)(unsigned char)(t.y * fb.inverseTicks + 0.5f) << 8) |
                                ((uint32_t)(unsigned char)(t.z * fb.inverseTicks + 0.5f) << 16) | (255u << 24);
            reinterpret_cast<uint32_t*>(fb.pixels)[p] = px;
        }
    } else {
        fb.staged[stream] = qx | (qy << 8) | (qz << 16);
    }
    if (fb.fsum) {
        float* fs = fb.fsum + 3u * stream;
        fs[0] += r.L0.x;
        fs[1] += r.L0.y;
        fs[2] += r.L0.z;
    }
    storeHome(fb.rngHome, stream, r.rng);
}

constexpr unsigned long long kPeerWaitTicks = 200000000ull;
__device__ __forceinline__ bool peerWaitExpired(unsigned long long& since) {
    const unsigned long long now = wall_clock64();
    if (since == 0ull) {
        since = now | 1ull;
        return false;
    }
    return now > since && now - since > kPeerWaitTicks;
}

__device__ __forceinline__ uint32_t frameLiveCount(const FrameBuffers& fb, int bounce, uint32_t own, const uint32_t* target) {
    uint32_t total = own;
    for (uint32_t p = 0; p < fb.numPeers; ++p) {
        unsigned long long since = 0ull;
        for (;;) {
            uint32_t ended = 0;
            for (int s = 0; s < kShards; ++s)
                ended += __hip_atomic_load(fb.peerDone[p] + countIndex(bounce - 1, s), __ATOMIC_ACQUIRE, __HIP_MEMORY_SCOPE_AGENT);
            if ((int32_t)(ended - target[p]) >= 0) break;
            __builtin_amdgcn_s_sleep(64);
            if (peerWaitExpired(since)) {
                if (threadIdx.x == 0) atomicAdd(fb.guardTimeouts, 1u);
                break;
            }
        }
        for (int s = 0; s < kShards; ++s)
            total += __hip_atomic_load(fb.peerCounts[p] + countIndex(bounce, s), __ATOMIC_RELAXED, __HIP_MEMORY_SCOPE_AGENT);
    }
    return total;
}

constexpr int kNeeLights = 2;
constexpr int kQueueCap = kNeeLights * 64;
static_assert(kQueueCap == kQueueCapConst, "anySpheresHybrid's plane stride");
constexpr int kWaveLdsWords = 8 * kQueueCap + kNeeLights * 64 / 4;
constexpr int kBlockScratchVec4 = 4;
constexpr int kBlockLdsVec4 = kBlockScratchVec4 + (kWaves * kWaveLdsWords + 3) / 4;

}

__global__ void rngInitKernel(uint32_t* __restrict__ rngHome, uint32_t plane, uint32_t samples, TileMap tile, uint64_t seed,
                              const uint32_t* __restrict__ jumpTable) {
    const uint32_t i = blockIdx.x * blockDim.x + threadIdx.x;
    const uint32_t n = (uint32_t)tile.width * (uint32_t)tile.localRows;
    const uint32_t lane = i / plane, p = i - lane * plane;
    if (lane >= samples || p >= n) return;
    const PixelCoord pc = locate(tile, p);
    ptrng::State s = ptrng::seeded(seed);
    ptrng::skip_subsequences(s, pc.globalIndex * samples + lane, jumpTable);
    storeHome(rngHome, i, s);
}

__global__ void clearKernel(FrameBuffers fb) {
    const uint32_t i = blockIdx.x * blockDim.x + threadIdx.x;
    if (i >= fb.numPixels) return;
    fb.accum[3 * i] = 0;
    fb.accum[3 * i + 1] = 0;
    fb.accum[3 * i + 2] = 0;
    if (fb.fsum)
        for (uint32_t l = 0; l < fb.samples; ++l) {
            float* fs = fb.fsum + 3u * (l * fb.plane + i);
            fs[0] = 0;
            fs[1] = 0;
            fs[2] = 0;
        }
    if (fb.pixels) fb.pixels[i] = ptss_uchar4{0, 0, 0, 0};
}

__global__ void displayKernel(FrameBuffers fb) {
    const uint32_t p = blockIdx.x * blockDim.x + threadIdx.x;
    if (p >= fb.numPixels) return;
    U3 t = reinterpret_cast<const U3*>(fb.accum)[p];
    uint32_t l = 0;
    for (; l + 8 <= fb.samples; l += 8) {
        uint32_t q[8];
#pragma unroll
        for (int k = 0; k < 8; ++k) q[k] = fb.staged[(l + k) * fb.plane + p];
#pragma unroll
        for (int k = 0; k < 8; ++k) {
            t.x += q[k] & 255u;
            t.y += (q[k] >> 8) & 255u;
            t.z += (q[k] >> 16) & 255u;
        }
    }
    for (; l < fb.samples; ++l) {
        const uint32_t q = fb.staged[l * fb.plane + p];
        t.x += q & 255u;
        t.y += (q >> 8) & 255u;
        t.z += (q >> 16) & 255u;
    }
    reinterpret_cast<U3*>(fb.accum)[p] = t;
    if (fb.pixels) {
        const uint32_t px = (uint32_t)(unsigned char)(t.x * fb.inverseTicks + 0.5f) |
                            ((uint32_t)(unsigned char)(t.y * fb.inverseTicks + 0.5f) << 8) |
                            ((uint32_t)(unsigned char)(t.z * fb.inverseTicks + 0.5f) << 16) | (255u << 24);
        reinterpret_cast<uint32_t*>(fb.pixels)[p] = px;
    }
}

__global__ void primaryPrepKernel(float4* __restrict__ blob, SceneLayout L, vec3 origin) {
    const int i = blockIdx.x * blockDim.x + threadIdx.x;
    if (i < L.numSpheres && !L.accelSpheres) {
        const float4 sp = blob[L.offSphere + i];
        const vec3 v = origin - xyz(sp);
        blob[L.offPrimSphere + i] = float4{v.x, v.y, v.z, dot(v, v) - sp.w};
    }
    if (L.accelSpheres && i < L.numChunks) {
        const float4 b = blob[L.offChunk + i];
        const vec3 v = origin - xyz(b);
        const float x = dot(v, v) - b.w;
        blob[L.offPrimChunk + i] = float4{v.x, v.y, v.z, x - ptm::abs(x) * 2.4e-7f};
    }
    if (i < L.numTriangles) {
        const vec3 v0 = xyz(blob[L.offTri + 3 * i]), e1 = xyz(blob[L.offTri + 3 * i + 1]), e2 = xyz(blob[L.offTri + 3 * i + 2]);
        const vec3 s = origin - v0;
        const vec3 r = cross(s, e1);
        blob[L.offPrimTri + 2 * i] = float4{s.x, s.y, s.z, dot(e2, r)};
        blob[L.offPrimTri + 2 * i + 1] = float4{r.x, r.y, r.z, 0.0f};
    }
}

struct TileEnv {
    const float4* sc;
    const float4* sceneBlob;
    const float* quantT;
    const float* in;
    float* out;
    float* wq;
    uint32_t* wqOwner;
    unsigned char* wqAnswer;
    uint32_t shard, lane, n;
    int numLights, bounce;
};

template <bool kLast, bool kFirst, bool kAccel, bool kBounded, bool kPairs, bool kCoherentIo, bool kMesh = false>
__device__ __forceinline__ void bounceTile(const FrameBuffers& fb, const SceneLayout& L, const TileMap& tile, const EyeParams& eye, const TileEnv& env,
                                           uint32_t base) {
    const float4* sc = env.sc;
    const float4* sceneBlob = env.sceneBlob;
    const float* quantT = env.quantT;
    const float* __restrict__ in = env.in;
    float* __restrict__ out = env.out;
    float* wq = env.wq;
    uint32_t* wqOwner = env.wqOwner;
    unsigned char* wqAnswer = env.wqAnswer;
    const uint32_t shard = env.shard, lane = env.lane, n = env.n;
    const int numLights = env.numLights, bounce = env.bounce;
    {
        const uint32_t i = base + threadIdx.x;
        uint32_t firstPixel = 0, firstLane = 0;
        bool valid = i < n;
        if constexpr (kFirst) {
            const uint32_t start = (((base / kBlock) * fb.laneCount + fb.laneIndex) * kShards + shard) * kBlock;
            firstLane = start / fb.plane;
            firstPixel = start - firstLane * fb.plane + threadIdx.x;
            valid = firstPixel < fb.numPixels;
        }

        RayRegs ray;
        ray.o = ray.d = ray.L0 = ray.T = v3(0, 0, 0);
        ray.pix = 0;
        ray.active = false;
        if constexpr (kFirst) {
            if (valid) {
                const uint32_t pixel = firstPixel;
                const PixelCoord pc = locate(tile, pixel);
                loadHome(fb.rngHome, firstLane * fb.plane + pixel, ray.rng);
                const float jitteredX = pc.x + ptrng::uniform(ray.rng);
                const float jitteredY = pc.gy + ptrng::uniform(ray.rng);
                const vec3 start = v3(((jitteredX * eye.invW) - 0.5f) * eye.s,
                                      1 * ((jitteredY * eye.invH) - 0.5f) * eye.s * eye.aspect, 1.0f) *
                                   eye.camera.zNear;
                ray.o = eye.camera.position;
                ray.d = normalize(rotate(eye.camera.rotation, start));
                ray.L0 = v3(0, 0, 0);
                ray.T = v3(1, 1, 1);
                ray.pix = pixel | (firstLane << kLaneShift);
                ray.active = true;
            }
        } else {
            if (valid) loadRayGeometry<kCoherentIo>(tileBlock(in, base), threadIdx.x, ray);
        }
#if PTSS_ABLATE & 2
        Hit h;
        h.kind = 2; h.idx = (int)(pixOf(ray.pix) % (uint32_t)L.numTriangles); h.distance = 1.0f + ray.d.x;
        h.w0 = 0.3f; h.w1 = 0.3f; h.w2 = 0.4f;
#else
        const Hit h = closestHit<kFirst, kAccel, kBounded, kMesh>(sc, sceneBlob, L, ray.o, ray.d, valid, reinterpret_cast<uint32_t*>(wq));
#endif
        const bool hit = valid && h.kind != 0;
        if constexpr (!kFirst) {
            if (valid) loadRayRng<kCoherentIo>(tileBlock(in, base), threadIdx.x, ray);
        }
        const float4* td = kMesh ? sceneBlob : sc;
        vec3 point = v3(0, 0, 0), normal = v3(0, 0, 0);
        float cosI = 0;
        int materialIdx = 0;
        if (hit) {
            point = ray.o + ray.d * h.distance;
            if (h.kind == 1) {
                normal = normalize(point - xyz(loadRow16(sc + L.offSphere + h.idx)));
                materialIdx = reinterpret_cast<const int*>((kAccel ? sceneBlob : sc) + L.offSphereMat)[h.idx];
            } else {
                const float4* nn = td + L.offTriNormal + 3 * h.idx;
                normal = (xyz(loadRow16(nn)) * h.w0 + xyz(loadRow16(nn + 1)) * h.w1) + xyz(loadRow16(nn + 2)) * h.w2;
                materialIdx = (int)asU(td[L.offTri + 3 * h.idx].w);
            }
            cosI = dot(-ray.d, normal);
        }
        const bool inside = cosI <= 0.0f;
        const bool lit = hit && !inside && !(PTSS_ABLATE & 1);
        const float4* mat = sc + L.offMaterial + 5 * materialIdx;

        vec3 radiance = v3(0, 0, 0);
        for (int l0 = 0; l0 < numLights; l0 += kNeeLights) {
            uint32_t queued = 0;
            bool need[kNeeLights];
            float cosL[kNeeLights], distance2[kNeeLights];
            [[maybe_unused]] vec3 pairW[kNeeLights];
            [[maybe_unused]] float pairReach[kNeeLights];
#pragma unroll
            for (int k = 0; k < kNeeLights; ++k) {
                need[k] = false;
                cosL[k] = 0;
                distance2[k] = 0;
                pairW[k] = v3(0, 0, 0);
                pairReach[k] = 0;
                const int li = l0 + k;
                if (li >= numLights) continue;
                vec3 lo = v3(0, 0, 0), w_i = v3(0, 0, 0);
                float distance = 0;
                if (lit) {
                    vec3 lightPoint;
                    if (li < L.numPointLights) {
                        lightPoint = xyz(loadRow16(sc + L.offPointLight + 2 * li));
                    } else {
                        const float4 light = sc[L.offAreaLight + 2 * (li - L.numPointLights)];
                        const float u1 = ptrng::uniform(ray.rng);
                        const float u2 = ptrng::uniform(ray.rng);
                        const float u3 = ptrng::uniform(ray.rng);
                        const float inverseTotal = ptm::rcp(u1 + u2 + u3);
                        const float weight0 = u1 * inverseTotal, weight1 = u2 * inverseTotal, weight2 = u3 * inverseTotal;
                        const int tri = (ptrng::uniform(ray.rng) > .5f) ? (int)asU(light.w) : (int)asU(sc[L.offAreaLight + 2 * (li - L.numPointLights) + 1].x);
                        const vec3 a = xyz(loadRow16(td + L.offTri + 3 * tri));
                        const vec3 b = xyz(loadRow16(td + L.offTriVert + 2 * tri));
                        const vec3 c = xyz(loadRow16(td + L.offTriVert + 2 * tri + 1));
                        lightPoint = (a * weight0 + b * weight1) + c * weight2;
                    }
                    const vec3 offset = lightPoint - point;
                    distance2[k] = dot(offset, offset);
                    distance = ptm::sqrt(distance2[k]);
                    w_i = offset / distance;
                    cosL[k] = ptm::max(0.0f, dot(normal, w_i));
                    const bool zeroTerm = L.neeSkipSafe && (distance2[k] > 0.0f) && (distance2[k] < ptm::inf()) &&
                                          (cosL[k] == 0.0f || mat[0].w == 0.0f);
                    need[k] = !zeroTerm;
                    lo = point + (ptm::kRayBump * normal);
                    distance -= 2 * ptm::kRayBump;
                }
                if constexpr (kPairs) {
                    pairW[k] = w_i;
                    pairReach[k] = distance;
                    continue;
                }
                const unsigned long long m = __ballot(need[k]);
                if (need[k]) {
                    const uint32_t slot = queued + __popcll(m & ((1ull << lane) - 1ull));
                    wq[0 * kQueueCap + slot] = lo.x;
                    wq[1 * kQueueCap + slot] = lo.y;
                    wq[2 * kQueueCap + slot] = lo.z;
                    wq[3 * kQueueCap + slot] = w_i.x;
                    wq[4 * kQueueCap + slot] = w_i.y;
                    wq[5 * kQueueCap + slot] = w_i.z;
                    wq[6 * kQueueCap + slot] = distance;
                    wqOwner[slot] = lane | ((uint32_t)k << 8);
                    wqAnswer[k * 64 + lane] = 0;
                }
                queued += (uint32_t)__popcll(m);
            }
            PTSS_DIAG_PAIRS(need[0], need[1], lit);
            waveLdsFence();
            PTSS_DIAG_QUEUE(queued);
            if constexpr (kPairs) {
                constexpr int kPairCap = 64;
                const bool needAny = need[0] || need[1];
                const unsigned long long m = __ballot(needAny);
                const uint32_t pairs = (uint32_t)__popcll(m);
                uint32_t* pairOwner = reinterpret_cast<uint32_t*>(wq + 11 * kPairCap);
                if (needAny) {
                    const uint32_t slot = __popcll(m & ((1ull << lane) - 1ull));
                    const vec3 lo = point + (ptm::kRayBump * normal);
                    wq[0 * kPairCap + slot] = lo.x;
                    wq[1 * kPairCap + slot] = lo.y;
                    wq[2 * kPairCap + slot] = lo.z;
                    wq[3 * kPairCap + slot] = pairW[0].x;
                    wq[4 * kPairCap + slot] = pairW[0].y;
                    wq[5 * kPairCap + slot] = pairW[0].z;
                    wq[6 * kPairCap + slot] = pairReach[0];
                    wq[7 * kPairCap + slot] = pairW[1].x;
                    wq[8 * kPairCap + slot] = pairW[1].y;
                    wq[9 * kPairCap + slot] = pairW[1].z;
                    wq[10 * kPairCap + slot] = pairReach[1];
                    pairOwner[slot] = lane | ((need[0] ? 1u : 0u) << 8) | ((need[1] ? 1u : 0u) << 9);
                    wqAnswer[0 * 64 + lane] = 0;
                    wqAnswer[1 * 64 + lane] = 0;
                }
                waveLdsFence();
                for (uint32_t e0 = 0; e0 < pairs;) {
                    const uint32_t rem = pairs - e0;
                    const uint32_t units = (rem + 7u) >> 3;
                    const int chunkLog = (units >= 7u) ? 6 : (units >= 4u ? 5 : (units >= 2u ? 4 : 3));
                    const int shift = 6 - chunkLog;
                    const uint32_t mine = lane >> shift;
                    const uint32_t sub = lane & ((1u << shift) - 1u);
                    const bool have = mine < rem;
                    const uint32_t es = have ? e0 + mine : 0u;
                    const vec3 lo = v3(wq[0 * kPairCap + es], wq[1 * kPairCap + es], wq[2 * kPairCap + es]);
                    const vec3 wA = v3(wq[3 * kPairCap + es], wq[4 * kPairCap + es], wq[5 * kPairCap + es]);
                    const float dA = wq[6 * kPairCap + es];
                    const vec3 wB = v3(wq[7 * kPairCap + es], wq[8 * kPairCap + es], wq[9 * kPairCap + es]);
                    const float dB = wq[10 * kPairCap + es];
                    const uint32_t ow = pairOwner[es];
                    const bool liveA = have && ((ow >> 8) & 1u) != 0u, liveB = have && ((ow >> 9) & 1u) != 0u;
                    bool occA, occB;
                    if (shift == 0) pairAnyHit<kBounded, false>(sc, L, lo, wA, dA, liveA, wB, dB, liveB, 0, 0, occA, occB);
                    else pairAnyHit<kBounded, true>(sc, L, lo, wA, dA, liveA, wB, dB, liveB, shift, (int)sub, occA, occB);
                    const unsigned long long verdictsA = __ballot(occA), verdictsB = __ballot(occB);
                    const unsigned long long group = ((1ull << (1u << shift)) - 1ull) << (mine << shift);
                    if (have && sub == 0u) {
                        if ((verdictsA & group) != 0ull) wqAnswer[0 * 64 + (ow & 63u)] = 1;
                        if ((verdictsB & group) != 0ull) wqAnswer[1 * 64 + (ow & 63u)] = 1;
                    }
                    e0 += 1u << chunkLog;
                }
            } else {
            for (uint32_t e0 = 0; e0 < queued;) {
                const uint32_t rem = queued - e0;
                const uint32_t units = (rem + 7u) >> 3;
                const int chunkLog = (units >= 7u || kAccel || kMesh) ? 6 : (units >= 4u ? 5 : (units >= 2u ? 4 : 3));
                const int shift = 6 - chunkLog;
                const uint32_t mine = lane >> shift;
// ... 383 lines not shown
        closestTrianglesMesh<false>(sc, sceneBlob, L, o, d, live, best);
        if (best.key != kNoTriangle) {
            dist = best.dist;
            kind = 2;
            prim = (int)(0xfffffffeu - best.key);
            pos = triPos[prim];
            w1 = best.w1;
            w2 = best.w2;
            w0 = 1.0f - (w1 + w2);
        }
    } else {
        for (int k = 0; k < L.numTriangles; ++k) {
            const int p = triStoredElsewhere ? triPos[k] : k;
            const TriHit th = triangleTest(loadTri(td + L.offTri + 3 * p), o, d, dist, liveMask);
            if (th.hit) {
                dist = th.dist;
                kind = 2;
                prim = k;
                pos = p;
                w0 = th.w0;
                w1 = th.w1;
                w2 = th.w2;
            }
        }
    }
    vec3 point = v3(0, 0, 0), normal = v3(0, 0, 0);
    int materialIdx = -1;
    if (kind != 0) {
        point = o + d * dist;
        if (kind == 1) {
            normal = normalize(point - xyz(loadRow16(sc + L.offSphere + pos)));
            materialIdx = reinterpret_cast<const int*>(sceneBlob + L.offSphereMat)[pos];
        } else {
            const float4* nn = td + L.offTriNormal + 3 * pos;
            normal = (xyz(loadRow16(nn)) * w0 + xyz(loadRow16(nn + 1)) * w1) + xyz(loadRow16(nn + 2)) * w2;
            materialIdx = (int)asU(td[L.offTri + 3 * pos].w);
        }
    } else {
        w1 = w2 = 0.0f;
    }
    if (kind == 1) w1 = w2 = 0.0f;
    return QueryHit{point, normal, dist, materialIdx, kind, prim, w1, w2};
}

template <bool kAny, bool kSceneInLds>
__global__ __launch_bounds__(kBlock) void queryKernel(const float4* __restrict__ sceneBlob, SceneLayout L, const float4* __restrict__ rays,
                                                       float4* __restrict__ out, uint32_t n) {
    extern __shared__ __attribute__((aligned(256))) float4 lds[];
    const float4* sc;
    if constexpr (kSceneInLds) {
        for (int k = threadIdx.x; k < L.ldsVec4; k += kBlock) lds[k] = sceneBlob[k];
        __syncthreads();
        sc = lds;
    } else {
        sc = sceneBlob;
    }
    const bool mesh = meshImage(L);
    for (uint32_t base = blockIdx.x * kBlock; base < n; base += gridDim.x * kBlock) {
        const uint32_t i = base + threadIdx.x;
        const bool live = i < n;
        float4 r0 = float4{0, 0, 0, 0}, r1 = float4{0, 0, 0, 0};
        if (live) {
            r0 = rays[2 * (size_t)i];
            r1 = rays[2 * (size_t)i + 1];
        }
        const vec3 o = xyz(r0), d = xyz(r1);
        const float tmax = r0.w;
        if constexpr (kAny) {
            bool blocked;
            if (L.accelSpheres) {
                SceneLayout Ls = L;
                Ls.numSpheres = L.numChunks * kChunkSpheres;
                blocked = anyHit<false, false, false>(sc, Ls, o, d, tmax, live);
            } else if (mesh) {
                blocked = anyHit<false, false, true>(sc, L, o, d, tmax, live, sceneBlob);
            } else {
                blocked = anyHit<false, false, false>(sc, L, o, d, tmax, live);
            }
            if (live) reinterpret_cast<uint32_t*>(out)[i] = blocked ? 1u : 0u;
        } else {
            const QueryHit q = closestQuery(sc, sceneBlob, L, o, d, tmax, live);
            if (live) {
                float4* h = out + 3 * (size_t)i;
                h[0] = float4{q.point.x, q.point.y, q.point.z, q.dist};
                h[1] = float4{q.normal.x, q.normal.y, q.normal.z, asF((uint32_t)q.materialIdx)};
                h[2] = float4{asF((uint32_t)q.kind), asF((uint32_t)q.prim), q.w1, q.w2};
            }
        }
    }
}

template <bool kSceneInLds>
__global__ __launch_bounds__(kBlock) void featureKernel(const float4* __restrict__ sceneBlob, SceneLayout L, TileMap tile, EyeParams eye,
                                                         vec3 defaultColor, float4* __restrict__ out, uint32_t n) {
    extern __shared__ __attribute__((aligned(256))) float4 lds[];
    const float4* sc;
    if constexpr (kSceneInLds) {
        for (int k = threadIdx.x; k < L.ldsVec4; k += kBlock) lds[k] = sceneBlob[k];
        __syncthreads();
        sc = lds;
    } else {
        sc = sceneBlob;
    }
    for (uint32_t base = blockIdx.x * kBlock; base < n; base += gridDim.x * kBlock) {
        const uint32_t i = base + threadIdx.x;
        const bool live = i < n;
        vec3 d = v3(0, 0, 0);
        if (live) {
            const PixelCoord pc = locate(tile, i);
            const float jitteredX = pc.x + 0.5f;
            const float jitteredY = pc.gy + 0.5f;
            const vec3 start = v3(((jitteredX * eye.invW) - 0.5f) * eye.s,
                                  1 * ((jitteredY * eye.invH) - 0.5f) * eye.s * eye.aspect, 1.0f) *
                               eye.camera.zNear;
            d = normalize(rotate(eye.camera.rotation, start));
        }
        const QueryHit q = closestQuery(sc, sceneBlob, L, eye.camera.position, d, ptm::inf(), live);
        if (live) {
            vec3 albedo = defaultColor;
            if (q.kind != 0) albedo = xyz(loadRow16(sc + L.offMaterial + 5 * q.materialIdx));
            float4* f = out + 2 * (size_t)i;
            f[0] = float4{q.normal.x, q.normal.y, q.normal.z, q.dist};
            f[1] = float4{albedo.x, albedo.y, albedo.z, asF((uint32_t)q.materialIdx)};
        }
    }
}

static inline unsigned blocksFor(uint32_t n, unsigned block) { return (n + block - 1) / block; }

hipError_t launchRngInit(hipStream_t st, uint32_t* rngHome, uint32_t plane, uint32_t samples, TileMap tile, uint64_t seed,
                         const uint32_t* jumpTable) {
    hipLaunchKernelGGL(rngInitKernel, dim3(blocksFor(plane * samples, 256)), dim3(256), 0, st, rngHome, plane, samples, tile, seed,
                       jumpTable);
    return hipGetLastError();
}

hipError_t launchDisplay(hipStream_t st, const FrameBuffers& fb) {
    hipLaunchKernelGGL(displayKernel, dim3(blocksFor(fb.numPixels, 256)), dim3(256), 0, st, fb);
    return hipGetLastError();
}

hipError_t launchClear(hipStream_t st, const FrameBuffers& fb) {
    hipLaunchKernelGGL(clearKernel, dim3(blocksFor(fb.numPixels, 256)), dim3(256), 0, st, fb);
    return hipGetLastError();
}

hipError_t launchPrimaryPrep(hipStream_t st, float4* sceneBlob, const SceneLayout& layout, ptss_vec3 origin) {
    const int n = layout.numSpheres > layout.numTriangles ? layout.numSpheres : layout.numTriangles;
    if (n <= 0) return hipSuccess;
    hipLaunchKernelGGL(primaryPrepKernel, dim3(blocksFor((uint32_t)n, 64)), dim3(64), 0, st, sceneBlob, layout, origin);
    return hipGetLastError();
}

#if PTSS_DIAG
hipError_t readDiagCounters(unsigned long long* out8) { return hipMemcpyFromSymbol(out8, HIP_SYMBOL(g_diag), 64); }
#endif
size_t bounceLdsBytes(const SceneLayout& layout, bool sceneInLds) {
    return ((sceneInLds ? (size_t)layout.ldsVec4 : 0) + kBlockLdsVec4) * sizeof(float4);
}

enum SceneVariant : int { kVariantAccel, kVariantBoundedPairs, kVariantBounded, kVariantPlain, kVariantMesh, kNumVariants };
constexpr int kNumFrameVariants = kVariantMesh;
constexpr bool kVariantArgs[kNumVariants][4] = {{true, false, false, false}, {false, true, true, false}, {false, true, false, false},
                                                {false, false, false, false}, {false, false, false, true}};

static SceneVariant sceneVariant(const SceneLayout& layout, bool bounded) {
    if (meshImage(layout)) return kVariantMesh;
    if (layout.accelSpheres) return kVariantAccel;
    if (bounded && layout.neePairs) return kVariantBoundedPairs;
    return bounded ? kVariantBounded : kVariantPlain;
}

using KernelFn = void (*)(FrameBuffers, const float4*, SceneLayout, int, TileMap, EyeParams);

template <size_t... I>
constexpr std::array<KernelFn, sizeof...(I)> bounceTable(std::index_sequence<I...>) {
    return {{bounceKernel<(I & 4) != 0, (I & 2) != 0, (I & 1) != 0, kVariantArgs[I / 8][0], kVariantArgs[I / 8][1], kVariantArgs[I / 8][2],
                          kVariantArgs[I / 8][3]>...}};
}
template <size_t... V>
constexpr std::array<KernelFn, sizeof...(V)> frameTable(std::index_sequence<V...>) {
    return {{frameKernel<kVariantArgs[V][0], kVariantArgs[V][1], kVariantArgs[V][2]>...}};
}
static int bounceIndex(SceneVariant v, bool last, bool sceneInLds, bool first) { return v * 8 + last * 4 + sceneInLds * 2 + first; }
static KernelFn bounceKernelFor(int index) {
    static constexpr auto table = bounceTable(std::make_index_sequence<kNumVariants * 8>{});
    return table[index];
}
static KernelFn frameKernelFor(SceneVariant v) {
    static constexpr auto table = frameTable(std::make_index_sequence<kNumFrameVariants>{});
    return v < kNumFrameVariants ? table[v] : nullptr;
}
static int blocksPerCU(KernelFn k, size_t lds) {
    int a = 0;
    return hipOccupancyMaxActiveBlocksPerMultiprocessor(&a, k, kBlock, lds) == hipSuccess ? a : 0;
}

hipError_t launchBounce(hipStream_t st, const FrameBuffers& fb, const float4* sceneBlob, SceneLayout layout, int bounce,
                        bool isLast, bool sceneInLds, bool bounded, int gridBlocks, TileMap tile, EyeParams eye, unsigned long long* launched) {
    const int index = bounceIndex(sceneVariant(layout, bounded), isLast, sceneInLds, bounce == 0);
    hipLaunchKernelGGL(bounceKernelFor(index), dim3(gridBlocks), dim3(kBlock), bounceLdsBytes(layout, sceneInLds), st, fb, sceneBlob, layout, bounce,
                       tile, eye);
    const hipError_t e = hipGetLastError();
    if (e == hipSuccess) *launched |= 1ull << (index < kVariantMesh * 8 ? index : index + 8);
    return e;
}

hipError_t launchFrame(hipStream_t st, const FrameBuffers& fb, const float4* sceneBlob, SceneLayout layout, int numBounces, bool bounded, int gridBlocks,
                       TileMap tile, EyeParams eye, unsigned long long* launched) {
    const SceneVariant v = sceneVariant(layout, bounded);
    if (!frameKernelFor(v)) return hipErrorInvalidValue;
    hipLaunchKernelGGL(frameKernelFor(v), dim3(gridBlocks), dim3(kBlock), bounceLdsBytes(layout, true), st, fb, sceneBlob, layout, numBounces, tile, eye);
    const hipError_t e = hipGetLastError();
    if (e == hipSuccess) *launched |= 1ull << (kVariantMesh * 8 + v);
    return e;
}
int frameOccupancyBlocksPerCU(const SceneLayout& layout, bool bounded) {
    const KernelFn k = frameKernelFor(sceneVariant(layout, bounded));
    return k ? blocksPerCU(k, bounceLdsBytes(layout, true)) : 0;
}

hipError_t launchQuery(hipStream_t st, bool any, const float4* sceneBlob, SceneLayout layout, bool sceneInLds, const void* rays, void* out,
                       uint32_t n, int maxBlocks, unsigned long long* launched) {
    using QueryFn = void (*)(const float4*, SceneLayout, const float4*, float4*, uint32_t);
    static constexpr QueryFn table[4] = {queryKernel<false, false>, queryKernel<false, true>, queryKernel<true, false>, queryKernel<true, true>};
    const int index = (any ? 2 : 0) + (sceneInLds ? 1 : 0);
    unsigned blocks = blocksFor(n, kBlock);
    if (maxBlocks > 0 && blocks > (unsigned)maxBlocks) blocks = (unsigned)maxBlocks;
    const size_t lds = sceneInLds ? (size_t)layout.ldsVec4 * sizeof(float4) : 0;
    hipLaunchKernelGGL(table[index], dim3(blocks), dim3(kBlock), lds, st, sceneBlob, layout, static_cast<const float4*>(rays),
                       static_cast<float4*>(out), n);
    const hipError_t e = hipGetLastError();
    if (e == hipSuccess) *launched |= 1ull << (48 + index);
    return e;
}

hipError_t launchFeatures(hipStream_t st, const float4* sceneBlob, SceneLayout layout, bool sceneInLds, TileMap tile, EyeParams eye,
                          ptss_vec3 defaultColor, void* out, uint32_t n, int maxBlocks, unsigned long long* launched) {
    unsigned blocks = blocksFor(n, kBlock);
    if (maxBlocks > 0 && blocks > (unsigned)maxBlocks) blocks = (unsigned)maxBlocks;
    const size_t lds = sceneInLds ? (size_t)layout.ldsVec4 * sizeof(float4) : 0;
    hipLaunchKernelGGL(sceneInLds ? featureKernel<true> : featureKernel<false>, dim3(blocks), dim3(kBlock), lds, st, sceneBlob, layout, tile, eye,
                       defaultColor, static_cast<float4*>(out), n);
    const hipError_t e = hipGetLastError();
    if (e == hipSuccess) *launched |= 1ull << (52 + (sceneInLds ? 1 : 0));
    return e;
}

hipError_t launchFlush(hipStream_t st, const FrameBuffers& fb, int numBounces, const FlushTargets& targets) {
    hipLaunchKernelGGL(flushKernel, dim3(1), dim3(kMinLiveRays), 0, st, fb, numBounces, targets);
    return hipGetLastError();
}

int bounceOccupancyBlocksPerCU(const SceneLayout& layout, bool sceneInLds, bool bounded) {
    return blocksPerCU(bounceKernelFor(bounceIndex(sceneVariant(layout, bounded), false, sceneInLds, false)), bounceLdsBytes(layout, sceneInLds));
}

}
```

### cuda-path-tracer-ss_amd/host/host_capi.cpp

```cpp
#include "ptss_host.h"

#include <cstdio>
#include <cstring>
#include <new>
#include <vector>

#include "HostOps.h"
#include "Scene.h"
#include "ptdenoise.h"
#include "ptquant.h"
#include "ptmesh.h"
#include "pttri.h"
#include "xorwow.h"

struct ptss_scene {
    Scene scene;
};

namespace {
using namespace ptv;
template <int kC1, int kC2>
void triangleForm(const float* t, const float* o3, const float* d3, float limit, bool primary, float* out) {
    const vec3 v0 = v3(t[0], t[1], t[2]), e1 = v3(t[3], t[4], t[5]), e2 = v3(t[6], t[7], t[8]);
    const vec3 o = v3(o3[0], o3[1], o3[2]), d = v3(d3[0], d3[1], d3[2]);
    pttri::Head h;
    if (primary) {
        const vec3 s = o - v0, r = cross(s, e1);
        h = pttri::head<kC1, kC2, true>(v0, e1, e2, s, r, dot(e2, r), o, d);
    } else {
        h = pttri::head<kC1, kC2, false>(v0, e1, e2, v3(0, 0, 0), v3(0, 0, 0), 0.0f, o, d);
    }
    float b0 = 0, b1 = 0, b2 = 0;
    const bool pass = pttri::passesHead(h, limit);
    if (pass) pttri::weights<kC1, kC2>(h, d, b0, b1, b2);
    out[0] = (pass && pttri::passesWeights(b0, b1, b2)) ? 1.0f : 0.0f;
    out[1] = h.dist;
    out[2] = b0;
    out[3] = b1;
    out[4] = b2;
    out[5] = h.det;
}
}

extern "C" {

int ptss_scene_create(const char* preset, ptss_scene** out) {
    if (!preset || !out) return PTSS_HOST_EINVAL;
    ptss_scene* s = new (std::nothrow) ptss_scene();
    if (!s) return PTSS_HOST_EINVAL;
    if (!s->scene.buildPreset(preset)) {
        delete s;
        return PTSS_HOST_EINVAL;
    }
    *out = s;
    return PTSS_HOST_OK;
}

void ptss_scene_destroy(ptss_scene* s) { delete s; }

int ptss_scene_describe(const ptss_scene* s, ptss_scene_desc* out) {
    if (!s || !out) return PTSS_HOST_EINVAL;
    *out = s->scene.desc();
    return PTSS_HOST_OK;
}

int ptss_scene_add_obj(ptss_scene* s, const char* path, const float* m, int materialIdx, size_t* added) {
    if (!s || !path || materialIdx < 0 || (size_t)materialIdx >= s->scene.materialsVec.size()) return PTSS_HOST_EINVAL;
    mat4 t = mat4::identity();
    if (m)
        for (int r = 0; r < 4; ++r)
            for (int c = 0; c < 4; ++c) t.c[c][r] = m[4 * r + c];
    const long n = s->scene.addObjModel(path, t, materialIdx);
    if (n < 0) return n == -2 ? PTSS_HOST_EIO : PTSS_HOST_EINVAL;
    if (added) *added = (size_t)n;
    return PTSS_HOST_OK;
}

int ptss_camera_default(ptss_camera* out) {
    if (!out) return PTSS_HOST_EINVAL;
    *out = Camera();
    return PTSS_HOST_OK;
}

int ptss_camera_ray(const ptss_camera* cam, int width, int height, int x, int y, float jx, float jy, ptss_ray_query* out) {
    if (!cam || !out || width <= 0 || height <= 0) return PTSS_HOST_EINVAL;
    *out = cameraRay(*cam, width, height, x, y, jx, jy);
    return PTSS_HOST_OK;
}

int ptss_camera_move(ptss_camera* cam, unsigned char key, int* moved) {
    if (!cam) return PTSS_HOST_EINVAL;
    Camera c;
    static_cast<ptss_camera&>(c) = *cam;
    const bool m = moveCamera(c, key);
    *cam = c;
    if (moved) *moved = m ? 1 : 0;
    return PTSS_HOST_OK;
}

int ptss_write_tga(const char* filename, const ptss_uchar4* rgba, int width, int height) {
    if (!filename || !rgba || width <= 0 || height <= 0) return PTSS_HOST_EINVAL;
    return writeTga(filename, rgba, width, height) ? PTSS_HOST_OK : PTSS_HOST_EIO;
}

int ptss_tile_rows(int height, int band_rows, int rank, int world, int* rows, int cap) {
    if (height < 0 || band_rows <= 0 || world <= 0 || rank < 0 || rank >= world) return PTSS_HOST_EINVAL;
    int n = 0;
    for (int y = 0; y < height; ++y) {
        if ((y / band_rows) % world != rank) continue;
        if (rows && n < cap) rows[n] = y;
        ++n;
    }
    return n;
}

int ptss_probe_math(int op, const float* x, const float* y, float* out, size_t n) {
    if (!x || !out) return PTSS_HOST_EINVAL;
    for (size_t i = 0; i < n; ++i) {
        float s, c;
        switch (op) {
            case 0: ptm::sincos(x[i], s, c); out[i] = s; break;
            case 1: ptm::sincos(x[i], s, c); out[i] = c; break;
            case 2: out[i] = ptm::tan(x[i]); break;
            case 3: out[i] = ptm::atan(x[i]); break;
            case 4: out[i] = ptm::log(x[i]); break;
            case 5: out[i] = ptm::exp(x[i]); break;
            case 6: if (!y) return PTSS_HOST_EINVAL; out[i] = ptm::pow(x[i], y[i]); break;
            case 7: out[i] = ptm::sqrt(x[i]); break;
            default: return PTSS_HOST_EINVAL;
        }
    }
    return PTSS_HOST_OK;
}

int ptss_probe_triangle_forms(const float* tri9, const float* o3, const float* d3, const float* limit, int primary, size_t n, int* cls,
                              float* general6, float* classed6) {
    if (!tri9 || !o3 || !d3 || !limit || !cls || !general6 || !classed6) return PTSS_HOST_EINVAL;
    for (size_t i = 0; i < n; ++i) {
        const float* t = tri9 + 9 * i;
        const int c = pttri::triangleClass(v3(t[3], t[4], t[5]), v3(t[6], t[7], t[8]));
        cls[i] = c;
        triangleForm<0, 0>(t, o3 + 3 * i, d3 + 3 * i, limit[i], primary != 0, general6 + 6 * i);
        float* out = classed6 + 6 * i;
        switch (c) {
#define PTSS_TRI_CASE(c1, c2) \
    case (c1) * 4 + (c2): triangleForm<c1, c2>(t, o3 + 3 * i, d3 + 3 * i, limit[i], primary != 0, out); break;
            PTSS_TRI_CASE(0, 1) PTSS_TRI_CASE(0, 2) PTSS_TRI_CASE(0, 3)
            PTSS_TRI_CASE(1, 0) PTSS_TRI_CASE(1, 2) PTSS_TRI_CASE(1, 3)
            PTSS_TRI_CASE(2, 0) PTSS_TRI_CASE(2, 1) PTSS_TRI_CASE(2, 3)
            PTSS_TRI_CASE(3, 0) PTSS_TRI_CASE(3, 1) PTSS_TRI_CASE(3, 2)
#undef PTSS_TRI_CASE
            default: triangleForm<0, 0>(t, o3 + 3 * i, d3 + 3 * i, limit[i], primary != 0, out); break;
        }
    }
    return PTSS_HOST_OK;
}

int ptss_probe_quantize(const float* x, unsigned int* out, size_t n) {
    if (!x || !out) return PTSS_HOST_EINVAL;
    for (size_t i = 0; i < n; ++i) out[i] = ptq::quantize_literal(x[i]);
    return PTSS_HOST_OK;
}

int ptss_probe_quant_table(float* out257) {
    if (!out257) return PTSS_HOST_EINVAL;
    float T[ptq::kTableFloats];
    if (!ptq::build_thresholds(T)) return PTSS_HOST_EINVAL;
    for (int k = 0; k <= 256; ++k) out257[k] = T[k];
    return PTSS_HOST_OK;
}

static const uint32_t* jumpTable() {
    static std::vector<uint32_t> table;
    if (table.empty()) {
        table.resize(ptrng::kJumpTableWords);
        ptrng::build_subsequence_table(table.data());
    }
    return table.data();
}

int ptss_probe_mesh_bound(const float* tri9, size_t ntri, const float* o3, const float* d3, size_t n, float margin, int* out, float* bound12) {
    if (!tri9 || ntri == 0 || ntri > (1u << 20) || (n && (!o3 || !d3 || !out))) return PTSS_HOST_EINVAL;
    float b[12];
    ptmesh::buildBound(tri9, (int)ntri, b);
    if (bound12)
        for (int k = 0; k < 12; ++k) bound12[k] = b[k];
    for (size_t i = 0; i < n; ++i) {
        const vec3 o = v3(o3[3 * i], o3[3 * i + 1], o3[3 * i + 2]), d = v3(d3[3 * i], d3[3 * i + 1], d3[3 * i + 2]);
        out[i] = ptmesh::mayTouch(v3(b[0], b[1], b[2]), b[3], v3(b[4], b[5], b[6]), b[7], b[8], b[9], b[10], b[11], o, d, margin) ? 1 : 0;
    }
    return PTSS_HOST_OK;
}

int ptss_probe_denoise(const uint32_t* accum, float inverseTicks, const ptss_pixel_feature* features, int width, int height,
                       const ptss_denoise_params* params, unsigned char* out_rgba, float* out_float) {
    if (!accum || !features || !params || width <= 0 || height <= 0) return PTSS_HOST_EINVAL;
    if (params->structSize != (unsigned int)sizeof(ptss_denoise_params) || params->levels < 0 || params->levels > PTSS_DENOISE_MAX_LEVELS)
        return PTSS_HOST_EINVAL;
    if (!(params->sigmaColor > 0.0f) || !(params->sigmaNormal > 0.0f) || !(params->sigmaDepth >= 0.0f)) return PTSS_HOST_EINVAL;
    const size_t n = (size_t)width * (size_t)height;
    std::vector<vec3> plane[2];
    plane[0].resize(n);
    for (size_t p = 0; p < n; ++p) plane[0][p] = ptdn::displayValue(accum[3 * p], accum[3 * p + 1], accum[3 * p + 2], inverseTicks);
    auto featureAt = [&](int q) { return ptdn::Feature{features[q].normal, features[q].depth, features[q].materialIdx}; };
    auto depthAt = [&](int q) { return features[q].depth; };
    int cur = 0;
    for (int i = 0; i < params->levels; ++i) {
        const ptdn::Level lv = ptdn::levelOf(*params, i);
        const std::vector<vec3>& src = plane[cur];
        std::vector<vec3>& dst = plane[1 - cur];
        dst.resize(n);
        auto colourAt = [&](int q) { return src[(size_t)q]; };
        for (int y = 0; y < height; ++y)
            for (int x = 0; x < width; ++x) dst[(size_t)y * width + x] = ptdn::filterPixel(x, y, width, height, lv, colourAt, featureAt, depthAt);
        cur = 1 - cur;
    }
    for (size_t p = 0; p < n; ++p) {
        const vec3 v = plane[cur][p];
        if (out_float) { out_float[3 * p] = v.x; out_float[3 * p + 1] = v.y; out_float[3 * p + 2] = v.z; }
        if (out_rgba) { out_rgba[4 * p] = ptdn::toByte(v.x); out_rgba[4 * p + 1] = ptdn::toByte(v.y); out_rgba[4 * p + 2] = ptdn::toByte(v.z); out_rgba[4 * p + 3] = 255; }
    }
    return PTSS_HOST_OK;
}

int ptss_probe_rng_init(unsigned long long seed, unsigned int subsequence, unsigned int* out6) {
    if (!out6) return PTSS_HOST_EINVAL;
    ptrng::State s = ptrng::seeded(seed);
    ptrng::skip_subsequences(s, subsequence, jumpTable());
    for (int i = 0; i < 5; ++i) out6[i] = s.v[i];
    out6[5] = s.d;
    return PTSS_HOST_OK;
}

int ptss_probe_rng_draw(unsigned int* state6, unsigned int* raw, float* uni, size_t n) {
    if (!state6) return PTSS_HOST_EINVAL;
    ptrng::State s;
    for (int i = 0; i < 5; ++i) s.v[i] = state6[i];
    s.d = state6[5];
    for (size_t i = 0; i < n; ++i) {
        ptrng::State before = s;
        const uint32_t r = ptrng::next(s);
        if (raw) raw[i] = r;
        if (uni) uni[i] = ptrng::uniform(before);
    }
    for (int i = 0; i < 5; ++i) state6[i] = s.v[i];
    state6[5] = s.d;
    return PTSS_HOST_OK;
}

int ptss_probe_rng_jump_table(unsigned int* out, size_t words) {
    if (!out || words != (size_t)ptrng::kJumpTableWords) return PTSS_HOST_EINVAL;
    std::memcpy(out, jumpTable(), words * sizeof(uint32_t));
    return PTSS_HOST_OK;
}

}
```

### cuda-path-tracer-ss_amd/ptss.py

```python
import ctypes as C
import os

import numpy as np

from ptss_types import (AreaLight, Camera, DenoiseParams, Material, PixelFeature, PointLight, RayHit, RayQuery, SceneDesc, Sphere,
                        Triangle, UChar4, Vec3, struct_to_dict)

_HERE = os.path.dirname(os.path.abspath(__file__))
LIBDIR = os.path.join(_HERE, "lib")
HOST_LIB = os.path.join(LIBDIR, "libptss_host.so")
DEVICE_LIB = os.path.join(LIBDIR, os.environ.get("PTSS_LIBNAME", "libptss.so"))

_u32p = C.POINTER(C.c_uint32)
_f32p = C.POINTER(C.c_float)


class PtssError(RuntimeError):
    pass


class RenderConfig(C.Structure):
    _fields_ = [("structSize", C.c_uint), ("width", C.c_int), ("height", C.c_int), ("seed", C.c_ulonglong), ("maxIterations", C.c_uint),
                ("device", C.c_int), ("tileRank", C.c_int), ("tileWorld", C.c_int), ("bandRows", C.c_int),
                ("syncEachFrame", C.c_int), ("floatAccumulator", C.c_int), ("timeKernels", C.c_int),
                ("samplesPerPass", C.c_int), ("everySphereLoop", C.c_int), ("frameLanes", C.c_int),
                ("lanesFreeRun", C.c_int), ("oneLaunchFrames", C.c_int)]


KERNEL_VARIANTS = ("accel", "bounded+pairs", "bounded", "plain")


def all_kernels():
    out = {("frame", v) for v in KERNEL_VARIANTS}
    for v in KERNEL_VARIANTS:
        out |= {("bounce", v, last, lds, first) for last in (False, True) for lds in (False, True) for first in (False, True)}
    return out


def mesh_kernels():
    return {("bounce", "mesh", last, lds, first) for last in (False, True) for lds in (False, True) for first in (False, True)}


def query_kernels():
    return {("query", kind, lds) for kind in ("closest", "any") for lds in (False, True)}


def feature_kernels():
    return {("features", lds) for lds in (False, True)}


_host = None
_dev = None
_hip = None


def _hip_lib():
    global _hip
    if _hip is None:
        device_lib()
        L = C.CDLL("libamdhip64.so.7", mode=C.RTLD_GLOBAL)
        L.hipMalloc.argtypes = [C.POINTER(C.c_void_p), C.c_size_t]
        L.hipFree.argtypes = [C.c_void_p]
        L.hipMemcpy.argtypes = [C.c_void_p, C.c_void_p, C.c_size_t, C.c_int]
        L.hipSetDevice.argtypes = [C.c_int]
        L.hipDeviceSynchronize.argtypes = []
        _hip = L
    return _hip


def _hip_check(rc, what):
    if rc != 0:
        raise PtssError(f"{what} failed (hipError {rc})")


def host_lib():
    global _host
    if _host is None:
        if not os.path.exists(HOST_LIB):
            raise PtssError(f"{HOST_LIB} missing: run `python __graft_entry__.py build` first")
        L = C.CDLL(HOST_LIB)
        L.ptss_scene_create.argtypes = [C.c_char_p, C.POINTER(C.c_void_p)]
        L.ptss_scene_destroy.argtypes = [C.c_void_p]
        L.ptss_scene_destroy.restype = None
        L.ptss_scene_describe.argtypes = [C.c_void_p, C.POINTER(SceneDesc)]
        L.ptss_camera_default.argtypes = [C.POINTER(Camera)]
        L.ptss_camera_move.argtypes = [C.POINTER(Camera), C.c_ubyte, C.POINTER(C.c_int)]
        L.ptss_write_tga.argtypes = [C.c_char_p, C.c_void_p, C.c_int, C.c_int]
        L.ptss_tile_rows.argtypes = [C.c_int, C.c_int, C.c_int, C.c_int, C.POINTER(C.c_int), C.c_int]
        L.ptss_probe_math.argtypes = [C.c_int, _f32p, _f32p, _f32p, C.c_size_t]
        L.ptss_probe_quantize.argtypes = [_f32p, C.POINTER(C.c_uint), C.c_size_t]
        L.ptss_probe_triangle_forms.argtypes = [_f32p, _f32p, _f32p, _f32p, C.c_int, C.c_size_t, C.POINTER(C.c_int), _f32p, _f32p]
        L.ptss_probe_quant_table.argtypes = [_f32p]
        L.ptss_probe_rng_init.argtypes = [C.c_ulonglong, C.c_uint, _u32p]
        L.ptss_scene_add_obj.argtypes = [C.c_void_p, C.c_char_p, _f32p, C.c_int, C.POINTER(C.c_size_t)]
        L.ptss_probe_mesh_bound.argtypes = [_f32p, C.c_size_t, _f32p, _f32p, C.c_size_t, C.c_float, C.POINTER(C.c_int), _f32p]
        L.ptss_probe_rng_draw.argtypes = [_u32p, _u32p, _f32p, C.c_size_t]
        L.ptss_probe_rng_jump_table.argtypes = [_u32p, C.c_size_t]
        L.ptss_camera_ray.argtypes = [C.POINTER(Camera), C.c_int, C.c_int, C.c_int, C.c_int, C.c_float, C.c_float, C.POINTER(RayQuery)]
        L.ptss_probe_denoise.argtypes = [_u32p, C.c_float, C.c_void_p, C.c_int, C.c_int, C.POINTER(DenoiseParams), C.c_void_p, _f32p]
        _host = L
    return _host


def _torch_first():
    import sys
    torch = sys.modules.get("torch")
    if torch is None:
        return
    try:
        if torch.cuda.is_available() and not torch.cuda.is_initialized():
            torch.cuda.init()
    except Exception as e:
        raise PtssError("torch is imported but torch.cuda could not be initialised before libptss.so's HIP runtime "
                        f"(INTEGRATION.md §5, two HIP runtimes in one process): {e}")


def device_lib():
    global _dev
    _torch_first()
    if _dev is None:
        if not os.path.exists(DEVICE_LIB):
            raise PtssError(f"{DEVICE_LIB} missing: the HIP extension was not built (no CPU fallback exists)")
        L = C.CDLL(DEVICE_LIB)
        vp = C.c_void_p
        L.ptss_default_config.argtypes = [C.POINTER(RenderConfig)]
        L.ptss_create.argtypes = [C.POINTER(SceneDesc), C.POINTER(RenderConfig), C.POINTER(vp)]
        L.ptss_destroy.argtypes = [vp]
        L.ptss_generate_frame.argtypes = [vp, vp, C.c_int]
        L.ptss_set_camera.argtypes = [vp, C.POINTER(Camera)]
        L.ptss_get_camera.argtypes = [vp, C.POINTER(Camera)]
        L.ptss_request_reset.argtypes = [vp]
        L.ptss_set_mode.argtypes = [vp, C.c_int]
        L.ptss_set_max_iterations.argtypes = [vp, C.c_uint]
        L.ptss_set_stream.argtypes = [vp, vp]
        L.ptss_bind_accumulator.argtypes = [vp, vp]
        L.ptss_accumulator_devptr.argtypes = [vp, C.POINTER(vp)]
        L.ptss_float_accumulator_devptr.argtypes = [vp, C.POINTER(vp)]
        L.ptss_alloc_pixels.argtypes = [vp, C.POINTER(vp)]
        L.ptss_free_pixels.argtypes = [vp, vp]
        L.ptss_local_pixels.argtypes = [vp, C.POINTER(C.c_size_t)]
        L.ptss_local_rows.argtypes = [vp, C.POINTER(C.c_int), C.c_int, C.POINTER(C.c_int)]
        L.ptss_read_accumulator.argtypes = [vp, _u32p, C.c_size_t]
        L.ptss_read_float_accumulator.argtypes = [vp, _f32p, C.c_size_t]
        L.ptss_read_pixels.argtypes = [vp, vp, vp, C.c_size_t]
        L.ptss_read_rng_state.argtypes = [vp, C.c_size_t, _u32p]
        L.ptss_read_rng_state_lane.argtypes = [vp, C.c_size_t, C.c_uint, _u32p]
        L.ptss_synchronize.argtypes = [vp]
        L.ptss_last_pass_ms.argtypes = [vp, _f32p]
        L.ptss_samples_since_reset.argtypes = [vp, C.POINTER(C.c_int)]
        L.ptss_live_counts.argtypes = [vp, _u32p, C.c_int, C.POINTER(C.c_int)]
        L.ptss_total_ray_bounces.argtypes = [vp, C.POINTER(C.c_ulonglong)]
        L.ptss_frame_lanes.argtypes = [vp, C.POINTER(C.c_int)]
        L.ptss_one_launch_frames.argtypes = [vp, C.POINTER(C.c_int)]
        L.ptss_guard_timeouts.argtypes = [vp, C.POINTER(C.c_uint)]
        L.ptss_bounce_kernel_time.argtypes = [vp, C.POINTER(C.c_double), C.POINTER(C.c_ulonglong)]
        L.ptss_launched_kernels.argtypes = [vp, C.POINTER(C.c_ulonglong)]
        L.ptss_debug_counters.argtypes = [vp, C.POINTER(C.c_ulonglong)]
        L.ptss_triangle_leaves.argtypes = [vp, C.POINTER(C.c_int)]
        L.ptss_intersect.argtypes = [vp, vp, vp, C.c_size_t, vp]
        L.ptss_occluded.argtypes = [vp, vp, vp, C.c_size_t, vp]
        L.ptss_render_features.argtypes = [vp, vp, vp]
        L.ptss_default_denoise_params.argtypes = [C.POINTER(DenoiseParams)]
        L.ptss_denoise.argtypes = [vp, vp, C.POINTER(DenoiseParams), vp, vp]
        L.ptss_read_denoise_plane.argtypes = [vp, _f32p, C.c_size_t, C.POINTER(C.c_int)]
        L.ptss_error_string.argtypes = [C.c_int]
        L.ptss_error_string.restype = C.c_char_p
        L.ptss_last_error_detail.restype = C.c_char_p
        _dev = L
    return _dev


def _check(rc):
    if rc != 0:
        L = device_lib()
        raise PtssError(f"ptss error {rc} ({L.ptss_error_string(rc).decode()}): {L.ptss_last_error_detail().decode()}")


class Scene:

    def __init__(self, preset="default"):
        self._h = C.c_void_p()
        rc = host_lib().ptss_scene_create(preset.encode(), C.byref(self._h))
        if rc != 0:
            raise PtssError(f"unknown scene preset {preset!r}")
        self.preset = preset
        self.desc = SceneDesc()
        host_lib().ptss_scene_describe(self._h, C.byref(self.desc))
        self.desc._owner = self

    def add_obj(self, path, transform=None, material=0):
        m = None
        if transform is not None:
            t = np.ascontiguousarray(np.asarray(transform, dtype=np.float32).reshape(4, 4))
            m = t.ctypes.data_as(_f32p)
        added = C.c_size_t()
        rc = host_lib().ptss_scene_add_obj(self._h, os.fsencode(path), m, int(material), C.byref(added))
        if rc != 0:
            raise PtssError(f"add_obj({path!r}) failed: {'cannot read the file' if rc == -2 else 'malformed OBJ or bad argument'} ({rc})")
        owner = self
        self.desc = SceneDesc()
        host_lib().ptss_scene_describe(self._h, C.byref(self.desc))
        self.desc._owner = owner
        return added.value

    def __del__(self):
        if getattr(self, "_h", None) and self._h.value and host_lib is not None:
            host_lib().ptss_scene_destroy(self._h)
            self._h = C.c_void_p()

    def _arr(self, ptr, n):
        return [ptr[i] for i in range(n)]

    @property
    def spheres(self):
        return self._arr(self.desc.spheres, self.desc.numSpheres)

    @property
    def triangles(self):
        return self._arr(self.desc.triangles, self.desc.numTriangles)

    @property
    def materials(self):
        return self._arr(self.desc.materials, self.desc.numMaterials)

    @property
    def area_lights(self):
        return self._arr(self.desc.areaLights, self.desc.numAreaLights)

    @property
    def point_lights(self):
        return self._arr(self.desc.pointLights, self.desc.numPointLights)

    def table(self):
        return {
            "spheres": [struct_to_dict(s) for s in self.spheres],
            "triangles": [struct_to_dict(s) for s in self.triangles],
            "materials": [struct_to_dict(s) for s in self.materials],
            "pointLights": [struct_to_dict(s) for s in self.point_lights],
            "areaLights": [struct_to_dict(s) for s in self.area_lights],
        }


def probe_mesh_bound(tris, origins, directions, margin=1.0):
    t = np.ascontiguousarray(np.asarray(tris, dtype=np.float32).reshape(-1, 9))
    o = np.ascontiguousarray(np.asarray(origins, dtype=np.float32).reshape(-1, 3))
    d = np.ascontiguousarray(np.asarray(directions, dtype=np.float32).reshape(-1, 3))
    out = np.zeros(len(o), dtype=np.int32)
    bound = np.zeros(12, dtype=np.float32)
    rc = host_lib().ptss_probe_mesh_bound(t.ctypes.data_as(_f32p), len(t), o.ctypes.data_as(_f32p), d.ctypes.data_as(_f32p), len(o),
                                          float(margin), out.ctypes.data_as(C.POINTER(C.c_int)), bound.ctypes.data_as(_f32p))
    if rc != 0:
        raise PtssError(f"ptss_probe_mesh_bound: {rc}")
    return out, bound


def default_camera():
    cam = Camera()
    host_lib().ptss_camera_default(C.byref(cam))
    return cam


def move_camera(cam, key):
    moved = C.c_int(0)
    host_lib().ptss_camera_move(C.byref(cam), ord(key), C.byref(moved))
    return bool(moved.value)


RAY_DTYPE = np.dtype([("origin", np.float32, 3), ("tmax", np.float32), ("direction", np.float32, 3), ("pad", np.float32)])
HIT_DTYPE = np.dtype([("point", np.float32, 3), ("distance", np.float32), ("normal", np.float32, 3), ("materialIdx", np.int32),
                      ("kind", np.int32), ("primitive", np.int32), ("w1", np.float32), ("w2", np.float32)])
FEATURE_DTYPE = np.dtype([("normal", np.float32, 3), ("depth", np.float32), ("albedo", np.float32, 3), ("materialIdx", np.int32)])
assert RAY_DTYPE.itemsize == C.sizeof(RayQuery) and HIT_DTYPE.itemsize == C.sizeof(RayHit)
assert FEATURE_DTYPE.itemsize == C.sizeof(PixelFeature)


def default_denoise_params(**overrides):
    p = DenoiseParams()
    _check(device_lib().ptss_default_denoise_params(C.byref(p)))
    for k, v in overrides.items():
        if v is not None:
            setattr(p, k, v)
    return p


def probe_denoise(accum, inverse_ticks, features, width, height, params):
    a = np.ascontiguousarray(accum, dtype=np.uint32).reshape(-1, 3)
    f = np.ascontiguousarray(features, dtype=FEATURE_DTYPE).reshape(-1)
    if len(a) != width * height or len(f) != width * height:
        raise ValueError("accum and features must hold width * height pixels")
    rgba = np.empty((len(a), 4), dtype=np.uint8)
    flt = np.empty((len(a), 3), dtype=np.float32)
    rc = host_lib().ptss_probe_denoise(a.ctypes.data_as(_u32p), float(inverse_ticks), f.ctypes.data_as(C.c_void_p), width, height,
                                       C.byref(params), rgba.ctypes.data_as(C.c_void_p), flt.ctypes.data_as(_f32p))
    if rc != 0:
        raise PtssError(f"ptss_probe_denoise: {rc}")
    return rgba, flt


def make_rays(origins, directions, tmax=float("inf")):
    o = np.asarray(origins, dtype=np.float32).reshape(-1, 3)
    d = np.asarray(directions, dtype=np.float32).reshape(-1, 3)
    if o.shape != d.shape:
        raise ValueError("origins and directions differ in shape")
    out = np.zeros((o.shape[0], 8), dtype=np.float32)
    out[:, 0:3], out[:, 4:7] = o, d
    out[:, 3] = np.broadcast_to(np.asarray(tmax, dtype=np.float32), (o.shape[0],))
    return out


def camera_ray(cam, width, height, x, y, jitter=(0.5, 0.5)):
    q = RayQuery()
    rc = host_lib().ptss_camera_ray(C.byref(cam), width, height, x, y, jitter[0], jitter[1], C.byref(q))
    if rc != 0:
        raise PtssError(f"ptss_camera_ray: {rc}")
    return np.frombuffer(bytes(q), dtype=np.float32).copy()


def camera_rays(cam, width, height, jitter=(0.5, 0.5)):
    out = np.empty((width * height, 8), dtype=np.float32)
    q = RayQuery()
    fn, jx, jy, ref_cam, ref_q = host_lib().ptss_camera_ray, C.c_float(jitter[0]), C.c_float(jitter[1]), C.byref(cam), C.byref(q)
    buf = (C.c_float * 8).from_buffer(q)
    for y in range(height):
        for x in range(width):
            if fn(ref_cam, width, height, x, y, jx, jy, ref_q) != 0:
                raise PtssError("ptss_camera_ray failed")
            out[y * width + x] = buf
    return out


def tile_rows(height, band_rows, rank, world):
    n = host_lib().ptss_tile_rows(height, band_rows, rank, world, None, 0)
    if n < 0:
        raise PtssError("bad tile spec")
    rows = (C.c_int * max(n, 1))()
    host_lib().ptss_tile_rows(height, band_rows, rank, world, rows, n)
    return np.array(rows[:n], dtype=np.int64)


def write_tga(path, rgba_hw4):
    a = np.ascontiguousarray(rgba_hw4, dtype=np.uint8)
    h, w = a.shape[:2]
    rc = host_lib().ptss_write_tga(path.encode(), a.ctypes.data_as(C.c_void_p), w, h)
    if rc != 0:
        raise PtssError(f"write_tga failed ({rc})")


class Renderer:

    def __init__(self, scene, width, height, max_iterations=15, seed=0x5EED, device=0, tile_rank=0, tile_world=1,
                 band_rows=8, sync_each_frame=True, float_accumulator=False, time_kernels=False, samples_per_pass=1,
                 every_sphere_loop=False, frame_lanes=0, lanes_free_run=False, one_launch_frames=0):
        L = device_lib()
        cfg = RenderConfig()
        _check(L.ptss_default_config(C.byref(cfg)))
        cfg.width, cfg.height = width, height
        cfg.seed = seed
        cfg.maxIterations = max_iterations
        cfg.device = device
        cfg.tileRank, cfg.tileWorld, cfg.bandRows = tile_rank, tile_world, band_rows
        cfg.syncEachFrame = 1 if sync_each_frame else 0
        cfg.floatAccumulator = 1 if float_accumulator else 0
        cfg.timeKernels = 1 if time_kernels else 0
        cfg.samplesPerPass = samples_per_pass
        cfg.everySphereLoop = 1 if every_sphere_loop else 0
        cfg.frameLanes = frame_lanes
        cfg.lanesFreeRun = 1 if lanes_free_run else 0
        cfg.oneLaunchFrames = one_launch_frames
        self.cfg = cfg
        self._scene = scene
        self._ctx = C.c_void_p()
        _check(L.ptss_create(C.byref(scene.desc), C.byref(cfg), C.byref(self._ctx)))
        n = C.c_size_t()
        _check(L.ptss_local_pixels(self._ctx, C.byref(n)))
        self.local_pixels = n.value
        self.width, self.height = width, height
        self.local_rows = self.local_pixels // width
        self._own_pixels = None
        self._buffers = {}
        self._have_features = False
        self.ticks = 1

    def close(self):
        if self._ctx:
            L = device_lib()
            if self._own_pixels:
                L.ptss_free_pixels(self._ctx, self._own_pixels)
                self._own_pixels = None
            for p in self._buffers.values():
                _hip_lib().hipFree(p)
            self._buffers = {}
            L.ptss_destroy(self._ctx)
            self._ctx = C.c_void_p()

    def __del__(self):
        try:
            self.close()
        except Exception:
            pass

    def pixels_devptr(self):
        if self._own_pixels is None:
            p = C.c_void_p()
            _check(device_lib().ptss_alloc_pixels(self._ctx, C.byref(p)))
            self._own_pixels = p
        return self._own_pixels

    def set_stream(self, raw_stream):
        _check(device_lib().ptss_set_stream(self._ctx, C.c_void_p(raw_stream)))

    def bind_accumulator(self, devptr):
        _check(device_lib().ptss_bind_accumulator(self._ctx, C.c_void_p(devptr)))

    def rows(self):
        cnt = C.c_int()
        rows = (C.c_int * max(self.local_rows, 1))()
        _check(device_lib().ptss_local_rows(self._ctx, rows, self.local_rows, C.byref(cnt)))
        return np.array(rows[:cnt.value], dtype=np.int64)

    def generate_frame(self, dev_pixels=None, ticks=None):
        if ticks is None:
            ticks = self.ticks
            self.ticks += 1
        if dev_pixels is None:
            dev_pixels = self.pixels_devptr()
        elif isinstance(dev_pixels, int):
            dev_pixels = C.c_void_p(dev_pixels)
        _check(device_lib().ptss_generate_frame(self._ctx, dev_pixels, ticks))

    def set_camera(self, cam):
        _check(device_lib().ptss_set_camera(self._ctx, C.byref(cam)))
        self._have_features = False

    def get_camera(self):
        cam = Camera()
        _check(device_lib().ptss_get_camera(self._ctx, C.byref(cam)))
        return cam

    def request_reset(self):
        _check(device_lib().ptss_request_reset(self._ctx))

    def set_mode(self, use_path_tracer):
        _check(device_lib().ptss_set_mode(self._ctx, 1 if use_path_tracer else 0))

    def set_max_iterations(self, n):
        _check(device_lib().ptss_set_max_iterations(self._ctx, n))

    def synchronize(self):
        _check(device_lib().ptss_synchronize(self._ctx))

    def accumulator(self):
        out = np.empty((self.local_pixels, 3), dtype=np.uint32)
        _check(device_lib().ptss_read_accumulator(self._ctx, out.ctypes.data_as(_u32p), out.size))
        return out

    def float_accumulator(self):
        out = np.empty((self.local_pixels, 3), dtype=np.float32)
        _check(device_lib().ptss_read_float_accumulator(self._ctx, out.ctypes.data_as(_f32p), out.size))
        return out

    def pixels(self, dev_pixels=None):
        if dev_pixels is None:
            dev_pixels = self.pixels_devptr()
        elif isinstance(dev_pixels, int):
            dev_pixels = C.c_void_p(dev_pixels)
        out = np.empty((self.local_pixels, 4), dtype=np.uint8)
        _check(device_lib().ptss_read_pixels(self._ctx, dev_pixels, out.ctypes.data_as(C.c_void_p), self.local_pixels))
        return out

    def rng_state(self, local_pixel, lane=0):
        out = np.empty(6, dtype=np.uint32)
        _check(device_lib().ptss_read_rng_state_lane(self._ctx, local_pixel, lane, out.ctypes.data_as(_u32p)))
        return out

    def last_pass_ms(self):
        v = C.c_float()
        _check(device_lib().ptss_last_pass_ms(self._ctx, C.byref(v)))
        return v.value

    def live_counts(self):
        out = (C.c_uint32 * 65)()
        n = C.c_int()
        _check(device_lib().ptss_live_counts(self._ctx, out, 65, C.byref(n)))
        return np.array(out[:n.value], dtype=np.uint32)

    def total_ray_bounces(self):
        v = C.c_ulonglong()
        _check(device_lib().ptss_total_ray_bounces(self._ctx, C.byref(v)))
        return v.value

    @property
    def one_launch_frames(self):
        v = C.c_int()
        _check(device_lib().ptss_one_launch_frames(self._ctx, C.byref(v)))
        return bool(v.value)

    @property
    def frame_lanes(self):
        v = C.c_int()
        _check(device_lib().ptss_frame_lanes(self._ctx, C.byref(v)))
        return v.value

    def guard_timeouts(self):
        v = C.c_uint()
        _check(device_lib().ptss_guard_timeouts(self._ctx, C.byref(v)))
        return v.value

    def launched_kernels(self):
        v = C.c_ulonglong()
        _check(device_lib().ptss_launched_kernels(self._ctx, C.byref(v)))
        out = set()
        for i, name in enumerate(KERNEL_VARIANTS):
            for j in range(8):
                if v.value >> (i * 8 + j) & 1:
                    out.add(("bounce", name, bool(j & 4), bool(j & 2), bool(j & 1)))
            if v.value >> (32 + i) & 1:
                out.add(("frame", name))
        for j in range(8):
            if v.value >> (40 + j) & 1:
                out.add(("bounce", "mesh", bool(j & 4), bool(j & 2), bool(j & 1)))
        for j in range(4):
            if v.value >> (48 + j) & 1:
                out.add(("query", "any" if j & 2 else "closest", bool(j & 1)))
        for j in range(2):
            if v.value >> (52 + j) & 1:
                out.add(("features", bool(j)))
        if v.value >> 54 & 1:
            out.add(("denoise",))
        return out

    def intersect(self, rays):
        return self._query(rays, any_hit=False)

    def occluded(self, rays):
        return self._query(rays, any_hit=True)

    def _query(self, rays, any_hit):
        L = device_lib()
        fn = L.ptss_occluded if any_hit else L.ptss_intersect
        if type(rays).__module__.split(".")[0] == "torch":
            import sys
            torch = sys.modules["torch"]
            if rays.dtype != torch.float32 or rays.dim() != 2 or rays.shape[1] != 8 or not rays.is_contiguous() or not rays.is_cuda:
                raise ValueError("rays: a contiguous (N, 8) float32 device tensor")
            n = rays.shape[0]
            out = (torch.empty(n, dtype=torch.int32, device=rays.device) if any_hit
                   else torch.empty((n, 12), dtype=torch.float32, device=rays.device))
            stream = torch.cuda.current_stream(rays.device).cuda_stream
            _check(fn(self._ctx, C.c_void_p(rays.data_ptr()), C.c_void_p(out.data_ptr()), n, C.c_void_p(stream)))
            return out
        a = np.asarray(rays)
        if a.dtype == RAY_DTYPE:
            a = np.ascontiguousarray(a).view(np.float32).reshape(-1, 8)
        a = np.ascontiguousarray(a, dtype=np.float32)
        if a.ndim != 2 or a.shape[1] != 8:
            raise ValueError("rays: (N, 8) float32 or (N,) RAY_DTYPE")
        n = a.shape[0]
        out = np.empty(n, dtype=np.uint32) if any_hit else np.empty(n, dtype=HIT_DTYPE)
        if n == 0:
            return out
        H = _hip_lib()
        _hip_check(H.hipSetDevice(self.cfg.device), "hipSetDevice")
        d_rays, d_out = C.c_void_p(), C.c_void_p()
        _hip_check(H.hipMalloc(C.byref(d_rays), a.nbytes), "hipMalloc")
        try:
            _hip_check(H.hipMalloc(C.byref(d_out), out.nbytes), "hipMalloc")
            _hip_check(H.hipMemcpy(d_rays, a.ctypes.data, a.nbytes, 1), "hipMemcpy")
            _check(fn(self._ctx, d_rays, d_out, n, None))
            self.synchronize()
            _hip_check(H.hipMemcpy(out.ctypes.data, d_out, out.nbytes, 2), "hipMemcpy")
        finally:
            H.hipFree(d_rays)
            if d_out:
                H.hipFree(d_out)
        return out

    def _device_buffer(self, name, nbytes):
        bufs = self._buffers
        if name not in bufs:
            H = _hip_lib()
            _hip_check(H.hipSetDevice(self.cfg.device), "hipSetDevice")
            p = C.c_void_p()
            _hip_check(H.hipMalloc(C.byref(p), max(nbytes, 16)), "hipMalloc")
            bufs[name] = p
        return bufs[name]

    def features_devptr(self):
        return self._device_buffer("features", self.local_pixels * FEATURE_DTYPE.itemsize)

    def features(self, stream=None):
        d = self.features_devptr()
        _check(device_lib().ptss_render_features(self._ctx, d, C.c_void_p(stream) if stream else None))
        out = np.empty(self.local_pixels, dtype=FEATURE_DTYPE)
        if self.local_pixels:
            if stream:
                _hip_check(_hip_lib().hipDeviceSynchronize(), "hipDeviceSynchronize")
            self.synchronize()
            _hip_check(_hip_lib().hipMemcpy(out.ctypes.data, d, out.nbytes, 2), "hipMemcpy")
        self._have_features = True
        return out

    def denoise(self, features=None, levels=None, sigma_color=None, sigma_normal=None, sigma_depth=None, dev_out=None, stream=None):
        L = device_lib()
        if features is None:
            if not self._have_features:
                self.features()
            d_feat = self.features_devptr()
        elif isinstance(features, int):
            d_feat = C.c_void_p(features)
        else:
            f = np.ascontiguousarray(features, dtype=FEATURE_DTYPE).reshape(-1)
            if len(f) != self.local_pixels:
                raise ValueError("features: one entry per local pixel")
            d_feat = self._device_buffer("features_upload", f.nbytes)
            _hip_check(_hip_lib().hipMemcpy(d_feat, f.ctypes.data, f.nbytes, 1), "hipMemcpy")
        params = default_denoise_params(levels=levels, sigmaColor=sigma_color, sigmaNormal=sigma_normal, sigmaDepth=sigma_depth)
        if dev_out is None:
            dev_out = self._device_buffer("denoised", self.local_pixels * 4)
        elif isinstance(dev_out, int):
            dev_out = C.c_void_p(dev_out)
        _check(L.ptss_denoise(self._ctx, d_feat, C.byref(params), dev_out, C.c_void_p(stream) if stream else None))
        if stream:
            _hip_check(_hip_lib().hipDeviceSynchronize(), "hipDeviceSynchronize")
        return self.pixels(dev_out)

    def denoise_plane(self):
        out = np.empty((self.local_pixels, 3), dtype=np.float32)
        level = C.c_int(-1)
        _check(device_lib().ptss_read_denoise_plane(self._ctx, out.ctypes.data_as(_f32p), out.size, C.byref(level)))
        return out, level.value

    def triangle_leaves(self):
        v = C.c_int()
        _check(device_lib().ptss_triangle_leaves(self._ctx, C.byref(v)))
        return v.value

    def debug_counters(self):
        out = (C.c_ulonglong * 8)()
        _check(device_lib().ptss_debug_counters(self._ctx, out))
        return [int(x) for x in out]

    def bounce_kernel_time(self):
        ms = C.c_double()
        n = C.c_ulonglong()
        _check(device_lib().ptss_bounce_kernel_time(self._ctx, C.byref(ms), C.byref(n)))
        return ms.value, n.value
```

### include/ptss.h

```cpp
#ifndef PTSS_H
#define PTSS_H

#include "ptss_types.h"

#ifdef __cplusplus
extern "C" {
#endif

#define PTSS_OK 0
#define PTSS_EINVAL (-1)
#define PTSS_EHIP (-2)
#define PTSS_ENODEVICE (-3)
#define PTSS_ENOMEM (-4)
#define PTSS_ERANGE (-5)
#define PTSS_ETIMEOUT (-6)
#define PTSS_VERSION 300

typedef struct ptss_context ptss_context;

typedef struct ptss_render_config {
    unsigned int structSize;
    int width, height;
    unsigned long long seed;
    unsigned int maxIterations;
    int device;
    int tileRank, tileWorld, bandRows;
    int syncEachFrame;
    int floatAccumulator;
    int timeKernels;
    int samplesPerPass;
    int everySphereLoop;
    int frameLanes;
    int lanesFreeRun;
    int oneLaunchFrames;
} ptss_render_config;

int ptss_default_config(ptss_render_config* cfg);

int ptss_create(const ptss_scene_desc* scene, const ptss_render_config* cfg, ptss_context** out);

int ptss_destroy(ptss_context* ctx);

int ptss_generate_frame(ptss_context* ctx, ptss_uchar4* dev_pixels, int ticks);

int ptss_set_camera(ptss_context* ctx, const ptss_camera* camera);
int ptss_get_camera(const ptss_context* ctx, ptss_camera* out);
int ptss_request_reset(ptss_context* ctx);
int ptss_set_mode(ptss_context* ctx, int usePathTracer);
int ptss_set_max_iterations(ptss_context* ctx, unsigned int maxIterations);

int ptss_set_stream(ptss_context* ctx, void* hipStream);
int ptss_bind_accumulator(ptss_context* ctx, uint32_t* dev_uint3);
int ptss_accumulator_devptr(ptss_context* ctx, uint32_t** out);
int ptss_float_accumulator_devptr(ptss_context* ctx, float** out);
int ptss_alloc_pixels(ptss_context* ctx, ptss_uchar4** out_dev);
int ptss_free_pixels(ptss_context* ctx, ptss_uchar4* dev);
int ptss_local_pixels(const ptss_context* ctx, size_t* out);
int ptss_local_rows(const ptss_context* ctx, int* rows, int cap, int* count);

int ptss_read_accumulator(ptss_context* ctx, uint32_t* host_uint3, size_t count);
int ptss_read_float_accumulator(ptss_context* ctx, float* host_float3, size_t count);
int ptss_read_pixels(ptss_context* ctx, const ptss_uchar4* dev_pixels, ptss_uchar4* host, size_t count);
int ptss_read_rng_state(ptss_context* ctx, size_t local_pixel, uint32_t* out6);
int ptss_read_rng_state_lane(ptss_context* ctx, size_t local_pixel, unsigned int lane, uint32_t* out6);
int ptss_synchronize(ptss_context* ctx);

int ptss_last_pass_ms(ptss_context* ctx, float* out_ms);
int ptss_samples_since_reset(const ptss_context* ctx, int* out);
int ptss_live_counts(ptss_context* ctx, uint32_t* out, int cap, int* n);
int ptss_total_ray_bounces(ptss_context* ctx, unsigned long long* out);
int ptss_bounce_kernel_time(ptss_context* ctx, double* total_ms, unsigned long long* launches);

int ptss_one_launch_frames(const ptss_context* ctx, int* out);
int ptss_frame_lanes(const ptss_context* ctx, int* out);
int ptss_guard_timeouts(ptss_context* ctx, unsigned int* out);

int ptss_launched_kernels(const ptss_context* ctx, unsigned long long* out);

int ptss_intersect(ptss_context* ctx, const ptss_ray_query* dev_rays, ptss_ray_hit* dev_hits, size_t n, void* hipStream);
int ptss_occluded(ptss_context* ctx, const ptss_ray_query* dev_rays, uint32_t* dev_occluded, size_t n, void* hipStream);

int ptss_render_features(ptss_context* ctx, ptss_pixel_feature* dev_features, void* hipStream);

int ptss_default_denoise_params(ptss_denoise_params* p);

int ptss_denoise(ptss_context* ctx, const ptss_pixel_feature* dev_features, const ptss_denoise_params* params, ptss_uchar4* dev_out,
                 void* hipStream);

int ptss_read_denoise_plane(ptss_context* ctx, float* host_float3, size_t count, int* level);

int ptss_triangle_leaves(const ptss_context* ctx, int* out);

int ptss_debug_counters(ptss_context* ctx, unsigned long long* out8);

const char* ptss_error_string(int code);
const char* ptss_last_error_detail(void);
int ptss_version(void);

#ifdef __cplusplus
}
#endif
#endif
```

### include/ptss_host.h

```cpp
#ifndef PTSS_HOST_H
#define PTSS_HOST_H

#include "ptss_types.h"

#ifdef __cplusplus
extern "C" {
#endif

#define PTSS_HOST_OK 0
#define PTSS_HOST_EINVAL (-1)
#define PTSS_HOST_EIO (-2)

typedef struct ptss_scene ptss_scene;

int ptss_scene_create(const char* preset, ptss_scene** out);
void ptss_scene_destroy(ptss_scene* s);
int ptss_scene_describe(const ptss_scene* s, ptss_scene_desc* out);

int ptss_scene_add_obj(ptss_scene* s, const char* path, const float* mat4x4, int materialIdx, size_t* added);

int ptss_camera_default(ptss_camera* out);
int ptss_camera_move(ptss_camera* cam, unsigned char key, int* moved);
int ptss_camera_ray(const ptss_camera* cam, int width, int height, int x, int y, float jx, float jy, ptss_ray_query* out);

int ptss_write_tga(const char* filename, const ptss_uchar4* rgba, int width, int height);

int ptss_tile_rows(int height, int band_rows, int rank, int world, int* rows, int cap);

int ptss_probe_math(int op, const float* x, const float* y, float* out, size_t n);
int ptss_probe_quantize(const float* x, unsigned int* out, size_t n);
int ptss_probe_quant_table(float* out257);
int ptss_probe_triangle_forms(const float* tri9, const float* o3, const float* d3, const float* limit, int primary, size_t n, int* cls,
                              float* general6, float* classed6);
int ptss_probe_mesh_bound(const float* tri9, size_t ntri, const float* o3, const float* d3, size_t n, float margin, int* out, float* bound12);
int ptss_probe_denoise(const uint32_t* accum, float inverseTicks, const ptss_pixel_feature* features, int width, int height,
                       const ptss_denoise_params* params, unsigned char* out_rgba, float* out_float);
int ptss_probe_rng_init(unsigned long long seed, unsigned int subsequence, unsigned int* out6);
int ptss_probe_rng_draw(unsigned int* state6, unsigned int* raw, float* uni, size_t n);
int ptss_probe_rng_jump_table(unsigned int* out, size_t words);

#ifdef __cplusplus
}
#endif
#endif
```

Before: 18260 Mrays/s.

## Cull primary-ray primitives per 64-pixel strip with camera frustum masks

Adds a kernel that runs when the camera changes. For each 64-pixel strip it builds a conservative frustum pyramid and computes a bitmask of the spheres and triangles that could be hit. The first-bounce closest-hit path reads this wave-uniform mask and skips sphere groups and triangles outside the strip's frustum. This removes intersection work only for primary rays, which are one of eight bounces. In exchange it adds a small per-camera-change kernel, extra blob storage and a risk of wrongly culling a primitive if the margins are too tight.

```diff
diff --git a/cuda-path-tracer-ss_amd/csrc/ptss_api.hip b/cuda-path-tracer-ss_amd/csrc/ptss_api.hip
--- a/cuda-path-tracer-ss_amd/csrc/ptss_api.hip
+++ b/cuda-path-tracer-ss_amd/csrc/ptss_api.hip
@@ -649,6 +649,14 @@
     }
 }
 
+uint32_t stripCount(const ptss_context* c) { return c->capacity / 64u; }
+size_t stripBytes(const ptss_context* c) { return (((size_t)stripCount(c) * 8u + 15u) / 16u) * 16u; }
+bool stripMasksOn(const ptss_context* c) {
+    const ptss::SceneLayout& L = c->image().layout;
+    return L.sphereBounded && cameraInRange(c->camera) && !L.accelSpheres && !ptss::meshImage(L) && (L.triClassed || L.numTriangles == 0) &&
+           L.numSpheres <= 32 && L.numSpheres + L.numTriangles <= 64 && c->usePathTracer && !c->cfg.everySphereLoop;
+}
+
 ptss::EyeParams eyeParams(const ptss_context* c) {
     return {c->camera, -2 * ptm::tan(c->camera.fieldOfView * 0.5f), (float)c->tile.height / (float)c->tile.width, 1.0f / c->tile.width,
             1.0f / c->tile.height};
@@ -897,8 +905,9 @@
 #define CREATE_TRY(expr) do { if (int _rc = createCheck((expr), #expr)) return (ptss_destroy(c), _rc); } while (0)
 
     for (int i = 0; i < numImages; ++i) {
-        CREATE_TRY(hipMalloc(&c->images[i].dBlob, blob[i].size() * sizeof(float4)));
+        CREATE_TRY(hipMalloc(&c->images[i].dBlob, (size_t)ptss::stripMaskRow(c->images[i].layout) * sizeof(float4) + stripBytes(c)));
         CREATE_TRY(hipMemcpy(c->images[i].dBlob, blob[i].data(), blob[i].size() * sizeof(float4), hipMemcpyHostToDevice));
+        CREATE_TRY(hipMemset(c->images[i].dBlob + ptss::stripMaskRow(c->images[i].layout), 0xff, stripBytes(c)));
     }
     CREATE_TRY(hipMalloc(&c->dRngHome, (size_t)ptss::kHomeWords * c->capacity * c->samples * sizeof(uint32_t)));
     for (int k = 0; k < numLanes; ++k)
@@ -1018,6 +1027,7 @@
     if (c->cameraDirty) {
         forkNeeded = true;
         HIP_TRY(ptss::launchPrimaryPrep(st, c->image().dBlob, c->image().layout, c->camera.position));
+        HIP_TRY(ptss::launchStripMasks(st, c->image().dBlob, c->image().layout, c->tile, eye, c->numPixels, stripCount(c), stripMasksOn(c)));
         c->cameraDirty = false;
     }
     harvestHints(c);
@@ -1065,6 +1075,7 @@
 int ptss_set_mode(ptss_context* c, int usePathTracer) {
     if (!c) return fail(PTSS_EINVAL, "ctx is null");
     c->usePathTracer = usePathTracer != 0;
+    c->cameraDirty = true;
     c->resetTicksThisFrame = true;
     return PTSS_OK;
 }
@@ -1359,6 +1370,26 @@
     return PTSS_OK;
 }
 
+int ptss_read_strip_masks(ptss_context* c, unsigned long long* out, size_t count) {
+    if (!c || !out) return fail(PTSS_EINVAL, "null argument");
+    if (count != (size_t)stripCount(c)) return fail(PTSS_ERANGE, "count must be the number of strips, local pixels rounded up to 256, / 64");
+    HIP_TRY(hipSetDevice(c->cfg.device));
+    HIP_TRY(hipStreamSynchronize(c->stream));
+    const ptss::SceneLayout& L = c->image().layout;
+    HIP_TRY(hipMemcpy(out, c->image().dBlob + ptss::stripMaskRow(L), count * sizeof(unsigned long long), hipMemcpyDeviceToHost));
+    if (L.triClassed && L.numTriangles > 0 && L.numSpheres + L.numTriangles <= 64) {
+        std::vector<int> posOf((size_t)L.numTriangles);
+        HIP_TRY(hipMemcpy(posOf.data(), c->image().dBlob + L.offTriPos, posOf.size() * sizeof(int), hipMemcpyDeviceToHost));
+        const unsigned long long low = L.numSpheres ? (~0ull >> (64 - L.numSpheres)) : 0ull, all = ~0ull >> (64 - (L.numSpheres + L.numTriangles));
+        for (size_t k = 0; k < count; ++k) {
+            unsigned long long w = (out[k] & low) | (out[k] & ~all);
+            for (int t = 0; t < L.numTriangles; ++t) w |= ((out[k] >> (L.numSpheres + posOf[(size_t)t])) & 1ull) << (L.numSpheres + t);
+            out[k] = w;
+        }
+    }
+    return PTSS_OK;
+}
+
 int ptss_triangle_leaves(const ptss_context* c, int* out) {
     if (!c || !out) return fail(PTSS_EINVAL, "null argument");
     const ptss::SceneLayout& L = c->image().layout;
diff --git a/cuda-path-tracer-ss_amd/csrc/ptss_device.h b/cuda-path-tracer-ss_amd/csrc/ptss_device.h
--- a/cuda-path-tracer-ss_amd/csrc/ptss_device.h
+++ b/cuda-path-tracer-ss_amd/csrc/ptss_device.h
@@ -94,6 +94,7 @@
     int offTriPos;
 };
 
+__host__ __device__ inline int stripMaskRow(const SceneLayout& L) { return L.totalVec4 + 1; }
 constexpr int kMeshLeaf = 16;
 __host__ __device__ inline bool meshImage(const SceneLayout& L) { return !L.triClassed && L.mesh.numLeaves > 0; }
 
@@ -152,6 +153,8 @@
 hipError_t launchDisplay(hipStream_t st, const FrameBuffers& fb);
 hipError_t launchClear(hipStream_t st, const FrameBuffers& fb);
 hipError_t launchPrimaryPrep(hipStream_t st, float4* sceneBlob, const SceneLayout& layout, ptss_vec3 origin);
+hipError_t launchStripMasks(hipStream_t st, float4* sceneBlob, const SceneLayout& layout, TileMap tile, EyeParams eye, uint32_t numPixels, uint32_t strips,
+                            bool on);
 hipError_t launchBounce(hipStream_t st, const FrameBuffers& fb, const float4* sceneBlob, SceneLayout layout, int bounce,
                         bool isLast, bool sceneInLds, bool bounded, int gridBlocks, TileMap tile, EyeParams eye, unsigned long long* launched);
 size_t bounceLdsBytes(const SceneLayout& layout, bool sceneInLds);
diff --git a/cuda-path-tracer-ss_amd/csrc/ptss_kernels.hip b/cuda-path-tracer-ss_amd/csrc/ptss_kernels.hip
--- a/cuda-path-tracer-ss_amd/csrc/ptss_kernels.hip
+++ b/cuda-path-tracer-ss_amd/csrc/ptss_kernels.hip
@@ -1,6 +1,7 @@
 #include "ptss_device.h"
 #include "ptquant.h"
 #include "pttri.h"
+#include "ptstrip.h"
 
 #include <array>
 #include <utility>
@@ -363,11 +364,17 @@
         shiftInMayHit(rev, b * b, 4 * pv.w);
     }
 }
-template <bool kPrimary, bool kBounded>
-__device__ __forceinline__ uint32_t sphereCandidates(const float4* rows, int cnt, vec3 o, vec3 d) {
+template <bool kPrimary, bool kBounded, bool kStrip = false>
+__device__ __forceinline__ uint32_t sphereCandidates(const float4* rows, int cnt, vec3 o, vec3 d, uint32_t keep = 0xffffffffu) {
     const int trips = (cnt + 3) >> 2;
     uint32_t rev = 0;
     for (int g = 0; g < trips; ++g) {
+        if constexpr (kStrip) {
+            if (((keep >> (4 * g)) & 15u) == 0u) {
+                rev <<= 4;
+                continue;
+            }
+        }
         const float4 r0 = rows[4 * g], r1 = rows[4 * g + 1], r2 = rows[4 * g + 2], r3 = rows[4 * g + 3];
         if constexpr (kPrimary) {
             shiftInSpherePrimary<kBounded>(rev, r0, d);
@@ -855,8 +862,9 @@
     return blocked;
 }
 
-template <bool kPrimary, bool kAccel, bool kBounded, bool kMesh = false>
-__device__ __forceinline__ Hit closestHit(const float4* sc, const float4* cold, const SceneLayout& L, vec3 o, vec3 d, bool live, uint32_t* ws) {
+template <bool kPrimary, bool kAccel, bool kBounded, bool kMesh = false, bool kStrip = false>
+__device__ __forceinline__ Hit closestHit(const float4* sc, const float4* cold, const SceneLayout& L, vec3 o, vec3 d, bool live, uint32_t* ws,
+                                          unsigned long long stripBits = ~0ull) {
     Hit h;
     h.distance = ptm::inf();
     h.kind = 0;
@@ -865,8 +873,9 @@
     if constexpr (kAccel) closestSpheresRegrouped<kPrimary>(sc, cold, L, o, d, live, h, ws);
     for (int base = 0; base < (kAccel ? 0 : L.numSpheres); base += 32) {
         const int cnt = (L.numSpheres - base < 32) ? (L.numSpheres - base) : 32;
-        uint32_t mask = sphereCandidates<kPrimary, kBounded>(sc + (kPrimary ? L.offPrimSphere : L.offSphere) + base, cnt, o, d);
-        mask &= live ? lowBits(cnt) : 0u;
+        const uint32_t keep = (kStrip && base == 0) ? (uint32_t)stripBits : 0xffffffffu;
+        uint32_t mask = sphereCandidates<kPrimary, kBounded, kStrip>(sc + (kPrimary ? L.offPrimSphere : L.offSphere) + base, cnt, o, d, keep);
+        mask &= live ? (lowBits(cnt) & keep) : 0u;
         PTSS_DIAG_CANDIDATES(mask, live, 0);
         while (mask != 0) {
             const int j = __builtin_ctz(mask);
@@ -899,10 +908,19 @@
     } else if (L.triClassed) {
         if (classedQueryOk(o, d)) {
             TriBest best{h.distance, kNoTriangle, 0.0f, 0.0f};
+            if (kStrip && stripBits != ~0ull) {
+                const unsigned long long triBits = stripBits >> (L.numSpheres & 63);
+#define PTSS_CLOSEST_BODY(c1, c2, t)              \
+    if (((triBits >> t) & 1ull) == 0ull) continue; \
+    triangleClassed<kPrimary, c1, c2, true>(sc + L.offTri + 3 * t, sc + L.offPrimTri + 2 * t, 0u, o, d, liveMask, best);
+                PTSS_FOR_TRIANGLES_BY_CLASS(L, PTSS_CLOSEST_BODY);
+#undef PTSS_CLOSEST_BODY
+            } else {
 #define PTSS_CLOSEST_BODY(c1, c2, t) \
     triangleClassed<kPrimary, c1, c2, true>(sc + L.offTri + 3 * t, sc + L.offPrimTri + 2 * t, 0u, o, d, liveMask, best);
             PTSS_FOR_TRIANGLES_BY_CLASS(L, PTSS_CLOSEST_BODY);
 #undef PTSS_CLOSEST_BODY
+            }
             if (waveAny(best.key != kNoTriangle)) {
                 const int* posOf = reinterpret_cast<const int*>(sc + L.offTriPos);
                 int pos = 0;
@@ -1475,6 +1493,21 @@
     }
 }
 
+__global__ void stripMaskKernel(float4* __restrict__ blob, SceneLayout L, TileMap tile, EyeParams eye, uint32_t numPixels, uint32_t strips, int on) {
+    const uint32_t k = blockIdx.x * blockDim.x + threadIdx.x;
+    if (k >= strips) return;
+    unsigned long long bits = ptstrip::kAllBits;
+    if (on) {
+        const float q[4] = {eye.camera.rotation.x, eye.camera.rotation.y, eye.camera.rotation.z, eye.camera.rotation.w};
+        const float pos[3] = {eye.camera.position.x, eye.camera.position.y, eye.camera.position.z};
+        const ptstrip::View v = ptstrip::makeView(q, pos, eye.camera.zNear, eye.s, eye.aspect, eye.invW, eye.invH, tile.width, tile.bandRows, tile.rank,
+                                                  tile.world, numPixels);
+        bits = ptstrip::stripMask(v, k, reinterpret_cast<const float*>(blob + L.offSphere), L.numSpheres, reinterpret_cast<const float*>(blob + L.offTri),
+                                  L.numTriangles, 1.0);
+    }
+    reinterpret_cast<unsigned long long*>(blob + stripMaskRow(L))[k] = bits;
+}
+
 struct TileEnv {
     const float4* sc;
     const float4* sceneBlob;
@@ -1541,7 +1574,15 @@
         h.kind = 2; h.idx = (int)(pixOf(ray.pix) % (uint32_t)L.numTriangles); h.distance = 1.0f + ray.d.x;
         h.w0 = 0.3f; h.w1 = 0.3f; h.w2 = 0.4f;
 #else
-        const Hit h = closestHit<kFirst, kAccel, kBounded, kMesh>(sc, sceneBlob, L, ray.o, ray.d, valid, reinterpret_cast<uint32_t*>(wq));
+        constexpr bool kStrip = kFirst && !kCoherentIo && !kAccel && !kMesh;
+        unsigned long long stripBits = ~0ull;
+        if constexpr (kStrip) {
+            const uint32_t strip = __builtin_amdgcn_readfirstlane((firstPixel - threadIdx.x + (threadIdx.x & ~63u)) >> 6);
+            const uint32_t* words = reinterpret_cast<const uint32_t*>(sceneBlob + stripMaskRow(L)) + 2 * (size_t)strip;
+            const uint32_t lo = __builtin_amdgcn_readfirstlane(words[0]), hi = __builtin_amdgcn_readfirstlane(words[1]);
+            stripBits = ((unsigned long long)hi << 32) | lo;
+        }
+        const Hit h = closestHit<kFirst, kAccel, kBounded, kMesh, kStrip>(sc, sceneBlob, L, ray.o, ray.d, valid, reinterpret_cast<uint32_t*>(wq), stripBits);
 #endif
         const bool hit = valid && h.kind != 0;
         if constexpr (!kFirst) {
@@ -2231,6 +2272,13 @@
     return hipGetLastError();
 }
 
+hipError_t launchStripMasks(hipStream_t st, float4* sceneBlob, const SceneLayout& layout, TileMap tile, EyeParams eye, uint32_t numPixels, uint32_t strips,
+                            bool on) {
+    if (strips == 0) return hipSuccess;
+    hipLaunchKernelGGL(stripMaskKernel, dim3(blocksFor(strips, 64)), dim3(64), 0, st, sceneBlob, layout, tile, eye, numPixels, strips, on ? 1 : 0);
+    return hipGetLastError();
+}
+
 #if PTSS_DIAG
 hipError_t readDiagCounters(unsigned long long* out8) { return hipMemcpyFromSymbol(out8, HIP_SYMBOL(g_diag), 64); }
 #endif
diff --git a/cuda-path-tracer-ss_amd/csrc/ptstrip.h b/cuda-path-tracer-ss_amd/csrc/ptstrip.h
--- /dev/null
+++ b/cuda-path-tracer-ss_amd/csrc/ptstrip.h
@@ -0,0 +1,202 @@
+#pragma once
+#include <stdint.h>
+
+#include "ptmath.h"
+#include "ptmesh.h"
+
+namespace ptstrip {
+
+constexpr double kTanSlack = 1e-4;
+constexpr double kSphereRel = 1e-2;
+constexpr int kMaxSpheres = 32, kMaxPrimitives = 64;
+constexpr unsigned long long kAllBits = ~0ull;
+
+struct View {
+    double o[3];
+    double cof[9];
+    double m[9];
+    double sx, sy;
+    double invW, invH;
+    int width, bandRows, rank, world;
+    uint32_t numPixels;
+    double side;
+    int valid;
+};
+
+PTM_HD bool finiteD(double x) { return x - x == 0.0; }
+
+PTM_HD View makeView(const float q[4], const float pos[3], float zNear, float s, float aspect, float invW, float invH, int width, int bandRows, int rank,
+                     int world, uint32_t numPixels) {
+    View v;
+    const double x = q[0], y = q[1], z = q[2], w = q[3];
+    const double M[9] = {1 - 2 * (y * y + z * z), 2 * (x * y - w * z),     2 * (x * z + w * y),
+                         2 * (x * y + w * z),     1 - 2 * (x * x + z * z), 2 * (y * z - w * x),
+                         2 * (x * z - w * y),     2 * (y * z + w * x),     1 - 2 * (x * x + y * y)};
+    for (int k = 0; k < 9; ++k) v.m[k] = M[k];
+    const int a[3] = {1, 2, 0}, b[3] = {2, 0, 1};
+    for (int r = 0; r < 3; ++r) {
+        const double* p = M + 3 * a[r];
+        const double* t = M + 3 * b[r];
+        v.cof[3 * r] = p[1] * t[2] - p[2] * t[1];
+        v.cof[3 * r + 1] = p[2] * t[0] - p[0] * t[2];
+        v.cof[3 * r + 2] = p[0] * t[1] - p[1] * t[0];
+    }
+    const double det = M[0] * v.cof[0] + M[1] * v.cof[1] + M[2] * v.cof[2];
+    for (int k = 0; k < 3; ++k) v.o[k] = pos[k];
+    v.sx = s;
+    v.sy = (double)s * (double)aspect;
+    v.invW = invW;
+    v.invH = invH;
+    v.width = width;
+    v.bandRows = bandRows;
+    v.rank = rank;
+    v.world = world;
+    v.numPixels = numPixels;
+    v.side = zNear < 0 ? -1.0 : 1.0;
+    const float az = zNear < 0 ? -zNear : zNear;
+    bool ok = det > 0.5 && det < 2.0 && az >= 1e-6f && az <= 1e6f && width > 0 && bandRows > 0 && world > 0 && rank >= 0;
+    ok = ok && finiteD(v.sx) && finiteD(v.sy) && finiteD(v.invW) && finiteD(v.invH);
+    ok = ok && (v.sx < 0 ? -v.sx : v.sx) <= 1e3 && (v.sy < 0 ? -v.sy : v.sy) <= 1e3 && v.invW > 0 && v.invW <= 1 && v.invH > 0 && v.invH <= 1;
+    for (int k = 0; k < 3; ++k) ok = ok && finiteD(v.o[k]);
+    v.valid = ok ? 1 : 0;
+    return v;
+}
+
+struct Pyramid {
+    double n[5][3];
+    double c[4][3];
+    int valid;
+};
+
+PTM_HD void mulUnit(const double A[9], double x, double y, double z, double out[3], int& ok) {
+    const double r0 = A[0] * x + A[1] * y + A[2] * z, r1 = A[3] * x + A[4] * y + A[5] * z, r2 = A[6] * x + A[7] * y + A[8] * z;
+    const double len = __builtin_sqrt(r0 * r0 + r1 * r1 + r2 * r2);
+    if (!(len > 1e-12) || !finiteD(len)) ok = 0;
+    out[0] = r0 / len;
+    out[1] = r1 / len;
+    out[2] = r2 / len;
+}
+
+PTM_HD Pyramid pyramidOf(const View& v, uint32_t strip, double margin) {
+    Pyramid p;
+    p.valid = 0;
+    const uint32_t p0 = strip * 64u;
+    if (!v.valid || p0 >= v.numPixels) return p;
+    const uint32_t p1 = (p0 + 63u < v.numPixels) ? p0 + 63u : v.numPixels - 1u;
+    const uint32_t W = (uint32_t)v.width;
+    const uint32_t ly0 = p0 / W, ly1 = p1 / W;
+    double xa, xb;
+    if (ly0 == ly1) {
+        xa = (double)(p0 % W);
+        xb = (double)(p1 % W);
+    } else {
+        xa = 0.0;
+        xb = (double)(W - 1u);
+    }
+    auto globalRow = [&](uint32_t ly) {
+        const uint32_t band = ly / (uint32_t)v.bandRows, within = ly % (uint32_t)v.bandRows;
+        return (double)((band * (uint32_t)v.world + (uint32_t)v.rank) * (uint32_t)v.bandRows + within);
+    };
+    const double ya = globalRow(ly0), yb = globalRow(ly1);
+    const double X0 = ((xa - margin) * v.invW - 0.5) * v.sx, X1 = ((xb + 2.0 * margin) * v.invW - 0.5) * v.sx;
+    const double Y0 = ((ya - margin) * v.invH - 0.5) * v.sy, Y1 = ((yb + 2.0 * margin) * v.invH - 0.5) * v.sy;
+    double Xmin = X0 < X1 ? X0 : X1, Xmax = X0 < X1 ? X1 : X0, Ymin = Y0 < Y1 ? Y0 : Y1, Ymax = Y0 < Y1 ? Y1 : Y0;
+    double big = -Xmin > Xmax ? -Xmin : Xmax;
+    big = -Ymin > big ? -Ymin : big;
+    big = Ymax > big ? Ymax : big;
+    const double slack = margin * kTanSlack * (1.0 + big);
+    Xmin -= slack;
+    Xmax += slack;
+    Ymin -= slack;
+    Ymax += slack;
+    int ok = (finiteD(Xmin) && finiteD(Xmax) && finiteD(Ymin) && finiteD(Ymax)) ? 1 : 0;
+    const double g = v.side;
+    mulUnit(v.cof, g, 0, -g * Xmin, p.n[0], ok);
+    mulUnit(v.cof, -g, 0, g * Xmax, p.n[1], ok);
+    mulUnit(v.cof, 0, g, -g * Ymin, p.n[2], ok);
+    mulUnit(v.cof, 0, -g, g * Ymax, p.n[3], ok);
+    mulUnit(v.cof, 0, 0, g, p.n[4], ok);
+    mulUnit(v.m, Xmin, Ymin, 1, p.c[0], ok);
+    mulUnit(v.m, Xmax, Ymin, 1, p.c[1], ok);
+    mulUnit(v.m, Xmin, Ymax, 1, p.c[2], ok);
+    mulUnit(v.m, Xmax, Ymax, 1, p.c[3], ok);
+    p.valid = ok;
+    return p;
+}
+
+PTM_HD bool sphereOutside(const View& v, const Pyramid& p, const float* row, double margin) {
+    const double w[3] = {(double)row[0] - v.o[0], (double)row[1] - v.o[1], (double)row[2] - v.o[2]};
+    const double r = __builtin_sqrt((double)row[3]);
+    const double len = __builtin_sqrt(w[0] * w[0] + w[1] * w[1] + w[2] * w[2]);
+    const double reach = r + margin * kSphereRel * (r + len);
+    if (!finiteD(reach)) return false;
+    for (int i = 0; i < 5; ++i)
+        if (p.n[i][0] * w[0] + p.n[i][1] * w[1] + p.n[i][2] * w[2] < -reach) return true;
+    return false;
+}
+
+PTM_HD bool triangleOutside(const View& v, const Pyramid& p, const float* v0, const float* e1, const float* e2, double margin) {
+    double vert[3][3], E[3][3];
+    for (int k = 0; k < 3; ++k) {
+        E[0][k] = e1[k];
+        E[1][k] = e2[k];
+        E[2][k] = (double)e2[k] - (double)e1[k];
+        vert[0][k] = (double)v0[k] - v.o[k];
+        vert[1][k] = vert[0][k] + E[0][k];
+        vert[2][k] = vert[0][k] + E[1][k];
+    }
+    double lmax = 0, sigma = 0;
+    for (int j = 0; j < 3; ++j) {
+        const double l = __builtin_sqrt(E[j][0] * E[j][0] + E[j][1] * E[j][1] + E[j][2] * E[j][2]);
+        const double d = __builtin_sqrt(vert[j][0] * vert[j][0] + vert[j][1] * vert[j][1] + vert[j][2] * vert[j][2]);
+        lmax = l > lmax ? l : lmax;
+        sigma = d > sigma ? d : sigma;
+    }
+    const double N[3] = {E[0][1] * E[1][2] - E[0][2] * E[1][1], E[0][2] * E[1][0] - E[0][0] * E[1][2], E[0][0] * E[1][1] - E[0][1] * E[1][0]};
+    double dmin = __builtin_inf();
+    int pos = 0, neg = 0;
+    for (int j = 0; j < 4; ++j) {
+        const double t = p.c[j][0] * N[0] + p.c[j][1] * N[1] + p.c[j][2] * N[2];
+        pos += t > 0;
+        neg += t < 0;
+        const double a = t < 0 ? -t : t;
+        dmin = a < dmin ? a : dmin;
+    }
+    const double coneD = (pos == 4 || neg == 4) ? dmin * (1.0 - 1e-5) : 0.0;
+    const double B = ptmesh::kBPerL2 * lmax * lmax * margin;
+    const double eta = (double)ptmesh::kEtaOfB * B;
+    const double floorD = (double)ptmesh::kDetFloor - eta;
+    const double D = coneD > floorD ? coneD : floorD;
+    if (!(D >= 4.0 * eta) || !(D > 0.0)) return false;
+    const double infl = (double)ptmesh::kInflRel * (lmax * (4.0 * (double)ptmesh::kU * margin + 1.02 * eta / D) + B * (sigma * (1.0 + 1e-6)) / D + 1e-30 * margin);
+    if (!finiteD(infl) || !finiteD(sigma)) return false;
+    for (int i = 0; i < 5; ++i) {
+        bool out = true;
+        for (int j = 0; j < 3; ++j) out = out && (p.n[i][0] * vert[j][0] + p.n[i][1] * vert[j][1] + p.n[i][2] * vert[j][2] < -infl);
+        if (out) return true;
+    }
+    return false;
+}
+
+PTM_HD bool geometryInDomain(const float* spheres, int numSpheres, const float* triRows, int numTriangles) {
+    bool ok = true;
+    for (int i = 0; i < 4 * numSpheres; ++i) ok = ok && (i % 4 == 3 ? spheres[i] <= 1e30f && spheres[i] >= 1e-24f : (spheres[i] <= 1e15f && spheres[i] >= -1e15f));
+    for (int i = 0; i < 12 * numTriangles; ++i) ok = ok && (i % 4 == 3 || (triRows[i] <= 2e15f && triRows[i] >= -2e15f));
+    return ok;
+}
+
+PTM_HD unsigned long long stripMask(const View& v, uint32_t strip, const float* spheres, int numSpheres, const float* triRows, int numTriangles, double margin) {
+    if (numSpheres < 0 || numTriangles < 0 || numSpheres > kMaxSpheres || numSpheres + numTriangles > kMaxPrimitives) return kAllBits;
+    const Pyramid p = pyramidOf(v, strip, margin);
+    if (!p.valid) return kAllBits;
+    unsigned long long bits = kAllBits;
+    for (int i = 0; i < numSpheres; ++i)
+        if (sphereOutside(v, p, spheres + 4 * i, margin)) bits &= ~(1ull << i);
+    for (int t = 0; t < numTriangles; ++t) {
+        const float* r = triRows + 12 * t;
+        if (triangleOutside(v, p, r, r + 4, r + 8, margin)) bits &= ~(1ull << (numSpheres + t));
+    }
+    return bits;
+}
+
+}
diff --git a/cuda-path-tracer-ss_amd/host/host_capi.cpp b/cuda-path-tracer-ss_amd/host/host_capi.cpp
--- a/cuda-path-tracer-ss_amd/host/host_capi.cpp
+++ b/cuda-path-tracer-ss_amd/host/host_capi.cpp
@@ -1,5 +1,6 @@
 #include "ptss_host.h"
 
+#include <cmath>
 #include <cstdio>
 #include <cstring>
 #include <new>
@@ -10,6 +11,7 @@
 #include "ptdenoise.h"
 #include "ptquant.h"
 #include "ptmesh.h"
+#include "ptstrip.h"
 #include "pttri.h"
 #include "xorwow.h"
 
@@ -85,6 +87,13 @@
 int ptss_camera_ray(const ptss_camera* cam, int width, int height, int x, int y, float jx, float jy, ptss_ray_query* out) {
     if (!cam || !out || width <= 0 || height <= 0) return PTSS_HOST_EINVAL;
     *out = cameraRay(*cam, width, height, x, y, jx, jy);
+    return PTSS_HOST_OK;
+}
+
+int ptss_camera_rays(const ptss_camera* cam, int width, int height, const int* x, const int* y, const float* jx, const float* jy, size_t n,
+                     ptss_ray_query* out) {
+    if (!cam || width <= 0 || height <= 0 || (n && (!x || !y || !jx || !jy || !out))) return PTSS_HOST_EINVAL;
+    for (size_t i = 0; i < n; ++i) out[i] = cameraRay(*cam, width, height, x[i], y[i], jx[i], jy[i]);
     return PTSS_HOST_OK;
 }
 
@@ -188,6 +197,69 @@
     for (size_t i = 0; i < n; ++i) {
         const vec3 o = v3(o3[3 * i], o3[3 * i + 1], o3[3 * i + 2]), d = v3(d3[3 * i], d3[3 * i + 1], d3[3 * i + 2]);
         out[i] = ptmesh::mayTouch(v3(b[0], b[1], b[2]), b[3], v3(b[4], b[5], b[6]), b[7], b[8], b[9], b[10], b[11], o, d, margin) ? 1 : 0;
+    }
+    return PTSS_HOST_OK;
+}
+
+int ptss_probe_strip_masks(const ptss_camera* cam, int width, int height, int band_rows, int rank, int world, const float* spheres4, size_t numSpheres,
+                           const float* tri9, size_t numTriangles, double margin, unsigned long long* out, size_t cap) {
+    if (!cam || width <= 0 || height <= 0 || band_rows <= 0 || world <= 0 || rank < 0 || rank >= world || (numSpheres && !spheres4) ||
+        (numTriangles && !tri9) || (cap && !out) || numSpheres > (1u << 20) || numTriangles > (1u << 20))
+        return PTSS_HOST_EINVAL;
+    const int rows = ptss_tile_rows(height, band_rows, rank, world, nullptr, 0);
+    const uint32_t numPixels = (uint32_t)rows * (uint32_t)width;
+    const float s = -2 * ptm::tan(cam->fieldOfView * 0.5f);
+    const float q[4] = {cam->rotation.x, cam->rotation.y, cam->rotation.z, cam->rotation.w};
+    const float pos[3] = {cam->position.x, cam->position.y, cam->position.z};
+    const ptstrip::View v = ptstrip::makeView(q, pos, cam->zNear, s, (float)height / (float)width, 1.0f / width, 1.0f / height, width, band_rows, rank, world, numPixels);
+    std::vector<float> sph(4 * numSpheres), tri(12 * numTriangles);
+    for (size_t i = 0; i < numSpheres; ++i) {
+        for (int k = 0; k < 3; ++k) sph[4 * i + k] = spheres4[4 * i + k];
+        sph[4 * i + 3] = spheres4[4 * i + 3] * spheres4[4 * i + 3];
+    }
+    for (size_t i = 0; i < numTriangles; ++i)
+        for (int r = 0; r < 3; ++r) {
+            for (int k = 0; k < 3; ++k) tri[12 * i + 4 * r + k] = tri9[9 * i + 3 * r + k];
+            tri[12 * i + 4 * r + 3] = 0.0f;
+        }
+    const uint32_t strips = (numPixels + 63u) / 64u;
+    const bool inDomain = ptstrip::geometryInDomain(sph.data(), (int)numSpheres, tri.data(), (int)numTriangles) && std::fabs(pos[0]) <= 1e15f &&
+                          std::fabs(pos[1]) <= 1e15f && std::fabs(pos[2]) <= 1e15f;
+    for (uint32_t k = 0; k < strips && k < cap; ++k)
+        out[k] = !inDomain ? ptstrip::kAllBits : ptstrip::stripMask(v, k, sph.data(), (int)numSpheres, tri.data(), (int)numTriangles, margin);
+    return (int)strips;
+}
+
+static bool sphereAcceptsPrimary(const float* sp4, vec3 o, vec3 d) {
+    const vec3 v = o - v3(sp4[0], sp4[1], sp4[2]);
+    const float c = dot(v, v) - sp4[3] * sp4[3];
+    const float b = dot(d, v) * 2;
+    float disc = (b * b) - 4 * c;
+    if (disc < 0) return false;
+    disc = ptm::sqrt(disc);
+    const float t0 = (-b + disc) * 0.5f, t1 = (-b - disc) * 0.5f;
+    if (t0 < 0 && t1 < 0) return false;
+    const float lo = t0 > t1 ? t1 : t0, hi = t0 > t1 ? t0 : t1;
+    const float cand = (lo < 0) ? hi : lo;
+    return !(cand > ptm::inf());
+}
+
+int ptss_probe_primary_hits(const float* spheres4, size_t numSpheres, const float* tri9, size_t numTriangles, const float* o3, const float* d3, size_t n,
+                            unsigned long long* out) {
+    if (numSpheres + numTriangles > 64 || (numSpheres && !spheres4) || (numTriangles && !tri9) || (n && (!o3 || !d3 || !out))) return PTSS_HOST_EINVAL;
+    const float inf = ptm::inf();
+    for (size_t i = 0; i < n; ++i) {
+        const vec3 o = v3(o3[3 * i], o3[3 * i + 1], o3[3 * i + 2]), d = v3(d3[3 * i], d3[3 * i + 1], d3[3 * i + 2]);
+        unsigned long long bits = 0;
+        for (size_t k = 0; k < numSpheres; ++k)
+            if (sphereAcceptsPrimary(spheres4 + 4 * k, o, d)) bits |= 1ull << k;
+        for (size_t t = 0; t < numTriangles; ++t) {
+            float g[6], c[6];
+            int cl;
+            ptss_probe_triangle_forms(tri9 + 9 * t, o3 + 3 * i, d3 + 3 * i, &inf, 1, 1, &cl, g, c);
+            if (g[0] != 0.0f || c[0] != 0.0f) bits |= 1ull << (numSpheres + t);
+        }
+        out[i] = bits;
     }
     return PTSS_HOST_OK;
 }
diff --git a/cuda-path-tracer-ss_amd/ptss.py b/cuda-path-tracer-ss_amd/ptss.py
--- a/cuda-path-tracer-ss_amd/ptss.py
+++ b/cuda-path-tracer-ss_amd/ptss.py
@@ -98,6 +98,10 @@
         L.ptss_probe_rng_jump_table.argtypes = [_u32p, C.c_size_t]
         L.ptss_camera_ray.argtypes = [C.POINTER(Camera), C.c_int, C.c_int, C.c_int, C.c_int, C.c_float, C.c_float, C.POINTER(RayQuery)]
         L.ptss_probe_denoise.argtypes = [_u32p, C.c_float, C.c_void_p, C.c_int, C.c_int, C.POINTER(DenoiseParams), C.c_void_p, _f32p]
+        L.ptss_camera_rays.argtypes = [C.POINTER(Camera), C.c_int, C.c_int, C.POINTER(C.c_int), C.POINTER(C.c_int), _f32p, _f32p, C.c_size_t, C.c_void_p]
+        L.ptss_probe_strip_masks.argtypes = [C.POINTER(Camera), C.c_int, C.c_int, C.c_int, C.c_int, C.c_int, _f32p, C.c_size_t, _f32p, C.c_size_t,
+                                             C.c_double, C.POINTER(C.c_ulonglong), C.c_size_t]
+        L.ptss_probe_primary_hits.argtypes = [_f32p, C.c_size_t, _f32p, C.c_size_t, _f32p, _f32p, C.c_size_t, C.POINTER(C.c_ulonglong)]
         _host = L
     return _host
 
@@ -157,6 +161,8 @@
         L.ptss_launched_kernels.argtypes = [vp, C.POINTER(C.c_ulonglong)]
         L.ptss_debug_counters.argtypes = [vp, C.POINTER(C.c_ulonglong)]
         L.ptss_triangle_leaves.argtypes = [vp, C.POINTER(C.c_int)]
+        if hasattr(L, "ptss_read_strip_masks"):
+            L.ptss_read_strip_masks.argtypes = [vp, C.POINTER(C.c_ulonglong), C.c_size_t]
         L.ptss_intersect.argtypes = [vp, vp, vp, C.c_size_t, vp]
         L.ptss_occluded.argtypes = [vp, vp, vp, C.c_size_t, vp]
         L.ptss_render_features.argtypes = [vp, vp, vp]
@@ -254,6 +260,38 @@
     return out, bound
 
 
+def scene_primitives(scene):
+    sp = np.array([[q.position.x, q.position.y, q.position.z, q.radius] for q in scene.spheres], dtype=np.float32).reshape(-1, 4)
+    v = np.array([[[p.x, p.y, p.z] for p in (t.vertex0, t.vertex1, t.vertex2)] for t in scene.triangles], dtype=np.float32).reshape(-1, 3, 3)
+    tri = np.concatenate([v[:, 0], v[:, 1] - v[:, 0], v[:, 2] - v[:, 0]], axis=1).astype(np.float32) if len(v) else np.zeros((0, 9), np.float32)
+    return np.ascontiguousarray(sp), np.ascontiguousarray(tri)
+
+
+def probe_strip_masks(cam, width, height, spheres4, tri9, band_rows=1, rank=0, world=1, margin=1.0):
+    sp = np.ascontiguousarray(np.asarray(spheres4, dtype=np.float32).reshape(-1, 4))
+    tr = np.ascontiguousarray(np.asarray(tri9, dtype=np.float32).reshape(-1, 9))
+    args = (C.byref(cam), width, height, band_rows, rank, world, sp.ctypes.data_as(_f32p), len(sp), tr.ctypes.data_as(_f32p), len(tr), float(margin))
+    n = host_lib().ptss_probe_strip_masks(*args, None, 0)
+    if n < 0:
+        raise PtssError(f"ptss_probe_strip_masks: {n}")
+    out = np.zeros(n, dtype=np.uint64)
+    host_lib().ptss_probe_strip_masks(*args, out.ctypes.data_as(C.POINTER(C.c_ulonglong)), n)
+    return out
+
+
+def probe_primary_hits(spheres4, tri9, origins, directions):
+    sp = np.ascontiguousarray(np.asarray(spheres4, dtype=np.float32).reshape(-1, 4))
+    tr = np.ascontiguousarray(np.asarray(tri9, dtype=np.float32).reshape(-1, 9))
+    o = np.ascontiguousarray(np.asarray(origins, dtype=np.float32).reshape(-1, 3))
+    d = np.ascontiguousarray(np.asarray(directions, dtype=np.float32).reshape(-1, 3))
+    out = np.zeros(len(o), dtype=np.uint64)
+    rc = host_lib().ptss_probe_primary_hits(sp.ctypes.data_as(_f32p), len(sp), tr.ctypes.data_as(_f32p), len(tr), o.ctypes.data_as(_f32p),
+                                            d.ctypes.data_as(_f32p), len(o), out.ctypes.data_as(C.POINTER(C.c_ulonglong)))
+    if rc != 0:
+        raise PtssError(f"ptss_probe_primary_hits: {rc}")
+    return out
+
+
 def default_camera():
     cam = Camera()
     host_lib().ptss_camera_default(C.byref(cam))
@@ -326,6 +364,20 @@
             if fn(ref_cam, width, height, x, y, jx, jy, ref_q) != 0:
                 raise PtssError("ptss_camera_ray failed")
             out[y * width + x] = buf
+    return out
+
+
+def camera_rays_at(cam, width, height, x, y, jx, jy):
+    x = np.ascontiguousarray(x, dtype=np.int32)
+    y = np.ascontiguousarray(y, dtype=np.int32)
+    jx = np.ascontiguousarray(jx, dtype=np.float32)
+    jy = np.ascontiguousarray(jy, dtype=np.float32)
+    out = np.empty((len(x), 8), dtype=np.float32)
+    ip = C.POINTER(C.c_int)
+    rc = host_lib().ptss_camera_rays(C.byref(cam), width, height, x.ctypes.data_as(ip), y.ctypes.data_as(ip), jx.ctypes.data_as(_f32p),
+                                     jy.ctypes.data_as(_f32p), len(x), out.ctypes.data_as(C.c_void_p))
+    if rc != 0:
+        raise PtssError(f"ptss_camera_rays: {rc}")
     return out
 
 
@@ -630,6 +682,13 @@
         _check(device_lib().ptss_read_denoise_plane(self._ctx, out.ctypes.data_as(_f32p), out.size, C.byref(level)))
         return out, level.value
 
+    def strip_masks(self):
+        L = device_lib()
+        n = ((self.local_pixels + 255) // 256) * 256 // 64 if self.local_pixels else 4
+        out = np.zeros(n, dtype=np.uint64)
+        _check(L.ptss_read_strip_masks(self._ctx, out.ctypes.data_as(C.POINTER(C.c_ulonglong)), n))
+        return out
+
     def triangle_leaves(self):
         v = C.c_int()
         _check(device_lib().ptss_triangle_leaves(self._ctx, C.byref(v)))
diff --git a/include/ptss.h b/include/ptss.h
--- a/include/ptss.h
+++ b/include/ptss.h
@@ -89,6 +89,8 @@
 
 int ptss_read_denoise_plane(ptss_context* ctx, float* host_float3, size_t count, int* level);
 
+int ptss_read_strip_masks(ptss_context* ctx, unsigned long long* out, size_t count);
+
 int ptss_triangle_leaves(const ptss_context* ctx, int* out);
 
 int ptss_debug_counters(ptss_context* ctx, unsigned long long* out8);
diff --git a/include/ptss_host.h b/include/ptss_host.h
--- a/include/ptss_host.h
+++ b/include/ptss_host.h
@@ -22,6 +22,8 @@
 int ptss_camera_default(ptss_camera* out);
 int ptss_camera_move(ptss_camera* cam, unsigned char key, int* moved);
 int ptss_camera_ray(const ptss_camera* cam, int width, int height, int x, int y, float jx, float jy, ptss_ray_query* out);
+int ptss_camera_rays(const ptss_camera* cam, int width, int height, const int* x, const int* y, const float* jx, const float* jy, size_t n,
+                     ptss_ray_query* out);
 
 int ptss_write_tga(const char* filename, const ptss_uchar4* rgba, int width, int height);
 
@@ -33,6 +35,10 @@
 int ptss_probe_triangle_forms(const float* tri9, const float* o3, const float* d3, const float* limit, int primary, size_t n, int* cls,
                               float* general6, float* classed6);
 int ptss_probe_mesh_bound(const float* tri9, size_t ntri, const float* o3, const float* d3, size_t n, float margin, int* out, float* bound12);
+int ptss_probe_strip_masks(const ptss_camera* cam, int width, int height, int band_rows, int rank, int world, const float* spheres4, size_t numSpheres,
+                           const float* tri9, size_t numTriangles, double margin, unsigned long long* out, size_t cap);
+int ptss_probe_primary_hits(const float* spheres4, size_t numSpheres, const float* tri9, size_t numTriangles, const float* o3, const float* d3, size_t n,
+                            unsigned long long* out);
 int ptss_probe_denoise(const uint32_t* accum, float inverseTicks, const ptss_pixel_feature* features, int width, int height,
                        const ptss_denoise_params* params, unsigned char* out_rgba, float* out_float);
 int ptss_probe_rng_init(unsigned long long seed, unsigned int subsequence, unsigned int* out6);
```

Measured after the change: 18690 Mrays/s, median of 6. 1.02x the previous value.
